# yukiteruono/pbsim3

Measured on AMD Instinct MI355X. Metric: simulated bases/sec, higher is better.
Workload: dtype u8

## Files before the change

pbsim3_amd/csrc/ctx.h:

```cpp
#pragma once
#include <hip/hip_runtime.h>
#include <limits.h>
#include <stdio.h>
#include <stdlib.h>
#include <stdint.h>

#include <algorithm>
#include <condition_variable>
#include <functional>
#include <memory>
#include <mutex>
#include <string>
#include <vector>

#include "../../include/pbsim3_amd.h"
#include "host_tables.h"
#include "kernels.h"

namespace pbsim {
extern thread_local std::string g_err;
int fail(const std::string &m);
}


#define NEED_DEVICE(c)                                                                      \
  do {                                                                                      \
    if ((c)->device < 0 || !(c)->stream)                                                    \
      return fail("this context has no HIP device: the gfx950 product path has no CPU fallback"); \
  } while (0)

#define HIP_OK(expr)                                                                        \
  do {                                                                                      \
    hipError_t e_ = (expr);                                                                 \
    if (e_ != hipSuccess)                                                                   \
      return fail(std::string("HIP error: ") + hipGetErrorString(e_) + " at " #expr);       \
  } while (0)

struct DevBuf {
  void *p = nullptr;
  size_t bytes = 0;
  ~DevBuf() { release(); }
  void release() {
    if (p) (void)hipFree(p);
    p = nullptr;
    bytes = 0;
  }
  hipError_t ensure(size_t n, bool exact = false) {
    if (n <= bytes) return hipSuccess;
    release();
    size_t want = exact ? n : std::max<size_t>(n + n / 8 + 256, 64u << 10);
    hipError_t e = hipMalloc(&p, want);
    if (e != hipSuccess) {
      p = nullptr;
      return e;
    }
    bytes = want;
    return hipSuccess;
  }
  template <class T>
  T *as() const {
    return reinterpret_cast<T *>(p);
  }
};

struct HostBuf {
  void *p = nullptr;
  size_t bytes = 0;
  ~HostBuf() {
    if (p) (void)hipHostFree(p);
  }
  hipError_t ensure(size_t n) {
    if (n <= bytes) return hipSuccess;
    if (p) (void)hipHostFree(p);
    p = nullptr;
    bytes = 0;
    size_t want = std::max<size_t>(n + n / 8 + 4096, 1u << 20);
    hipError_t e = hipHostMalloc(&p, want, hipHostMallocDefault);
    if (e != hipSuccess) {
      p = nullptr;
      return e;
    }
    bytes = want;
    return hipSuccess;
  }
};

using namespace pbsim;

constexpr int kMaxSlots = 6;
constexpr int kPipelineDepth = 2;
static_assert(kPipelineDepth >= 1 && kPipelineDepth <= kMaxSlots, "the pipeline's slots are the first of kMaxSlots");

constexpr size_t kScratchSlack = 64u << 10;
constexpr double kSinkBatchBases = 5.0e9;

constexpr int kDfBuffers = 5;
struct DfLane {
  DevBuf d_df_status, d_df_ctl;
  uint32_t epoch = 0;
  DevBuf d_df_dense[kDfBuffers];
  DevBuf d_df_code;
  HostBuf h_df_total, h_df_out[kDfBuffers];
  hipStream_t stream = nullptr;
  hipStream_t copy_stream = nullptr;
  bool own_streams = false;
  hipStream_t own[2] = {nullptr, nullptr};
  bool pre_valid = false, pre_own_staging = false, pre_elsewhere = false;
  const uint8_t *pre_text = nullptr;
  int64_t pre_n = 0;
  int pre_count = 0;
  hipStream_t lane_stream = nullptr;
  hipEvent_t ev_pre = nullptr;
  hipEvent_t ev_df[kDfBuffers] = {}, ev_cp[kDfBuffers] = {};
  hipEvent_t ev_k0[kDfBuffers] = {}, ev_k1[kDfBuffers] = {};
  std::vector<std::unique_ptr<HostBuf>> arena_blocks;
  std::vector<size_t> arena_fill;
  std::vector<char> arena_touched;
  std::vector<int> arena_idle;
  std::vector<std::pair<const char *, int64_t>> arena_segs;
  size_t arena_bytes() const {
    size_t n = 0;
    for (const auto &b : arena_blocks) n += b->bytes;
    return n;
  }
  void arena_reset() {
    std::fill(arena_fill.begin(), arena_fill.end(), 0);
    arena_segs.clear();
  }
  char *arena_reserve(int64_t n, size_t max_bytes) {
    static const size_t kBlock = getenv("PBSIM_PINNED_BLOCK_KB") && atoll(getenv("PBSIM_PINNED_BLOCK_KB")) > 0
                                     ? (size_t)atoll(getenv("PBSIM_PINNED_BLOCK_KB")) << 10 : (size_t)256u << 20;
    const size_t need = ((size_t)n + 63) & ~(size_t)63;
    for (size_t i = 0; i < arena_blocks.size(); i++) {
      HostBuf &b = *arena_blocks[i];
      if (arena_fill[i] + need <= b.bytes) {
        char *p = (char *)b.p + arena_fill[i];
        arena_fill[i] += need;
        arena_touched[i] = 1;
        arena_segs.emplace_back(p, n);
        return p;
      }
    }
    const size_t want = std::max(kBlock, need);
    if (max_bytes && arena_bytes() + want > max_bytes) return nullptr;
    if (getenv("PBSIM_TRACE")) fprintf(stderr, "[pbsim arena] new block of %zu MB (lane holds %zu MB in %zu blocks)\n", want >> 20, arena_bytes() >> 20, arena_blocks.size());
    arena_blocks.emplace_back(new HostBuf);
    arena_fill.push_back(0);
    arena_touched.push_back(1);
    arena_idle.push_back(0);
    if (arena_blocks.back()->ensure(want) != hipSuccess) {
      arena_blocks.pop_back();
      arena_fill.pop_back();
      arena_touched.pop_back();
      arena_idle.pop_back();
      return nullptr;
    }
    arena_fill.back() = need;
    arena_segs.emplace_back((char *)arena_blocks.back()->p, n);
    return (char *)arena_blocks.back()->p;
  }
  static constexpr int kArenaIdleJobs = 16;
  void arena_release() {
    arena_blocks.clear();
    arena_fill.clear();
    arena_touched.clear();
    arena_idle.clear();
    arena_segs.clear();
  }
  void arena_trim() {
    size_t k = 0;
    for (size_t i = 0; i < arena_blocks.size(); i++) arena_idle[i] = arena_touched[i] ? 0 : arena_idle[i] + 1;
    if (getenv("PBSIM_TRACE")) {
      size_t drop = 0;
      for (size_t i = 0; i < arena_blocks.size(); i++) drop += arena_idle[i] >= kArenaIdleJobs ? 1 : 0;
      if (drop) fprintf(stderr, "[pbsim arena] trim: %zu of %zu blocks go back\n", drop, arena_blocks.size());
    }
    for (size_t i = 0; i < arena_blocks.size(); i++)
      if (arena_idle[i] < kArenaIdleJobs) {
        if (k != i) {
          arena_blocks[k] = std::move(arena_blocks[i]);
          arena_idle[k] = arena_idle[i];
        }
        k++;
      }
    arena_blocks.resize(k);
    arena_idle.resize(k);
    arena_fill.assign(k, 0);
    arena_touched.assign(k, 0);
    arena_segs.clear();
  }
};

struct RefDesc {
  const uint8_t *seq = nullptr;
  const uint8_t *hp = nullptr;
  int64_t len = 0;
  int64_t unit = 0;
  bool hp_flag = false;
  bool hp11 = false;
};

struct StatsAcc {
  int64_t res_num = 0, res_len_total = 0, res_len_min = LONG_MAX, res_len_max = 0;
  int64_t res_sub = 0, res_ins = 0, res_del = 0;
  double accuracy_total = 0.0;
  std::vector<int64_t> freq_len, freq_acc;
  bool keep_values = false;
  struct Block {
    int64_t first_task;
    std::vector<double> values;
  };
  std::vector<Block> blocks;
  void reset() {
    res_num = res_len_total = res_len_max = 0;
    res_len_min = LONG_MAX;
    res_sub = res_ins = res_del = 0;
    accuracy_total = 0.0;
    std::fill(freq_len.begin(), freq_len.end(), 0);
    std::fill(freq_acc.begin(), freq_acc.end(), 0);
    blocks.clear();
  }
};

struct Slot {
  RefDesc ref;
  hipStream_t stream = nullptr;
  hipEvent_t ev0 = nullptr, ev1 = nullptr, ev2 = nullptr, ev3 = nullptr;
  DevBuf d_flags;
  DevBuf d_rawlen, d_len, d_off, d_acc;
  DevBuf d_hist, d_bin_start, d_bin_cursor, d_class_start;
  DevBuf d_task_of_slot, d_slot_of_task, d_wave_cap, d_wave_off, d_wg_tmp, d_wg_order;
  DevBuf d_out_len, d_maf_len, d_nsub, d_nins, d_ndel, d_qsum;
  DevBuf d_cum, d_scan_tmp, d_rt_len, d_mt_len, d_row_dst;
  DevBuf d_chain, d_chain_mask;
  DevBuf d_scratch, d_read_text, d_maf_text;
  HostBuf h_read_text, h_maf_text, h_stats, h_flags;
  DfLane df[2];
  hipStream_t walk_stream = nullptr;
  hipEvent_t ev_sq_walk = nullptr, ev_sq_done = nullptr;
  bool sq_pending = false;
  hipEvent_t ev_prep = nullptr;
  hipStream_t coop_stream = nullptr;
  hipEvent_t ev_coop = nullptr;
  bool stats_fetched = false;
  hipEvent_t ev_t0 = nullptr, ev_t1 = nullptr;
  bool text_timed = false;
  int64_t text_in = 0, text_out = 0;
  hipEvent_t ev_text = nullptr;
  int64_t b_first = 0, b_n = 0, b_slots_max = 0;
  bool b_truncated = false, b_enqueued = false, b_walked = false, b_finalized = false;
  bool b_chain = false;
  bool b_exported = false;
  int64_t b_trunc = -1;
  double b_factor = 2.0;
  int64_t b_pass0 = 0;
  int64_t b_max_raw = 0;
  pbsim_batch_info b_info;
};

struct JobRecord {
  DevBuf seq, hp, tiles, flags;
  int64_t len = 0;
  RefDesc ref;
  hipEvent_t ready = nullptr;
  DeviceFlags *h_flags = nullptr;
  ~JobRecord() {
    if (ready) (void)hipEventDestroy(ready);
    if (h_flags) (void)hipHostFree(h_flags);
  }
};

struct pbsim_ctx {
  pbsim_params p;
  int device = 0;
  hipStream_t stream = nullptr;
  Slot slots[kMaxSlots];
  int cur = 0;
  Slot &s() { return slots[cur]; }

  std::unique_ptr<ErrModel> err;
  std::unique_ptr<QsModel> qs;
  HeaderTables hdr;
  HpBias bias;
  ErrClassTables ect;
  QsClassTables qct;
  bool class_tables_dirty = true;
  int coop_wg_errhmm[2] = {0, 0};
  bool header_uploaded = false;

  DevBuf d_prob2len, d_prob2acc, d_cls;
  DevBuf d_qs_tabs_v[2];
  bool qs_tabs_ready[2] = {false, false};
  DevBuf d_seq_own, d_hp, d_tiles, d_ref_flags;
  DevBuf d_seq_next, d_hp_next, d_tiles_next, d_ref_flags_next;
  hipStream_t prefetch_stream = nullptr;
  DevBuf d_lines, d_lines_tmp;
  hipStream_t sq_stream = nullptr;
  const void *pf_src = nullptr;
  int64_t pf_len = 0;
  bool seq_hp_flag = false;
  const uint8_t *d_seq = nullptr;
  int64_t ref_len = 0;
  int64_t unit = 0;
  int64_t census[kHpSlots] = {0};
  bool census_done = false;
  bool census_from_job = false;
  bool hp11_explicit = false;
  bool hp11_before_job = false;
  int64_t n_units = 0, trans_reads = 0;
  DevBuf d_read_unit, d_read_minus, d_read_base, d_unit_len, d_unit_rank, d_unit_names, d_off_table, d_ssp, d_ssp_rv;
  DevBuf d_sq, d_sq_line_len, d_sq_line_qoff, d_sq_vbase;
  std::vector<int32_t> sq_len;
  std::vector<int64_t> sq_off;
  int64_t sq_total = 0;
  int64_t sp_chunk_bytes = 0;
  int64_t scratch_budget = 0;
  double scratch_factor = 2.0, need_seen = 0.0;
  bool scratch_factor_fixed = false;
  int64_t rewalked_batches = 0;
  bool scratch_auto = true;
  hipStream_t df_streams[2][2] = {{nullptr, nullptr}, {nullptr, nullptr}};
  bool defer_text_sync = false;
  bool defer_account = false;
  int walk_lds_kb = 27;
  bool bam_output = false;
  int deflate = 0;
  bool deflate_parallel = false;
  DevBuf d_df_tables;
  DevBuf d_df_prof;

  StatsAcc st;
  std::vector<std::unique_ptr<JobRecord>> job_records;
  std::mutex job_mu;
  std::condition_variable job_cv;
  std::vector<int64_t> job_expect_len;
  std::vector<std::unique_ptr<JobRecord>> job_spare;
  bool job_feed_failed = false;
  std::string job_feed_err;
  int64_t job_counters[8] = {0};
  int64_t job_progress[8] = {0};
  double job_breakdown[16] = {0};
  int job_interleave = 1;
  int64_t job_first_unit = 1;

  double prof_walk_ms = 0, prof_total_ms = 0, prof_tail_ms = 0;
  int64_t prof_walk_launches = 0, prof_tail_launches = 0;
  int64_t prof_wave_launches = 0;
  hipEvent_t ev_prof_base = nullptr;
  std::vector<std::pair<float, float>> prof_intervals;
  double prof_text_ms = 0, prof_deflate_ms = 0;
  int64_t prof_text_launches = 0, prof_text_in = 0, prof_text_out = 0;
  int64_t prof_deflate_launches = 0, prof_deflate_in = 0, prof_deflate_out = 0;
  std::mutex prof_mu;
};

namespace pbsim {
RefDesc current_ref(const pbsim_ctx *c);
int64_t quota_of(const pbsim_ctx *c, int64_t ref_len);
int walk_begin(pbsim_ctx *c, const RefDesc &ref, int64_t first_read, int64_t n_reads, int64_t truncate_remaining, bool chain = false,
               double factor = 0.0 );
double scratch_factor_of(const pbsim_ctx *c);
int chain_end_finalize(pbsim_ctx *c, int64_t len_total_before, pbsim_batch_info *out);
int chain_reads_for(const pbsim_ctx *c, int64_t ref_len, int64_t remaining);
constexpr int kChainReads = 6;
int64_t batch_capacity_for(const pbsim_ctx *c, int64_t ref_len);
int finalize_cut(pbsim_ctx *c, int64_t len_total_before, pbsim_batch_info *out);
int finalize_text(pbsim_ctx *c, pbsim_batch_info *info);
int finalize_uncut(pbsim_ctx *c, pbsim_batch_info *out);
std::string sam_header_text(const pbsim_ctx *c, int64_t unit);
int account_slot(pbsim_ctx *c, StatsAcc *st);
int account_of(pbsim_ctx *c, Slot &sl, StatsAcc *st);
void stats_add_task(StatsAcc *st, int64_t len_max, bool quality, long len, long nsub, long nins, long ndel, double qsum,
                    std::vector<double> *values);
void stats_finish(const StatsAcc &st, const pbsim_params &p, int64_t ref_len, pbsim_stats *o);
int stats_merge(StatsAcc *st, const pbsim_params &p, const pbsim_comm *comm, int64_t *extra, int n_extra);
int deflate_prelaunch(pbsim_ctx *c, Slot &sl, bool want_read, bool want_maf);
int deflate_pieces(pbsim_ctx *c, DfLane &lane, const uint8_t *d_text, int64_t n,
                   const std::function<int(const char *, int64_t)> &consume,
                   const std::function<char *(int64_t)> *place = nullptr);
int ensure_deflate_ready(pbsim_ctx *c);
int ensure_crc_tables(pbsim_ctx *c);
int prepare_enqueue(pbsim_ctx *c, uint8_t *d_seq, DevBuf &hp, DevBuf &tiles, DevBuf &flags, int64_t len, hipStream_t stream);
int ensure_tables(pbsim_ctx *c, bool hp11);
inline bool has_quality(const pbsim_ctx *c) { return c->p.method == PBSIM_METHOD_QS || c->p.method == PBSIM_METHOD_SAMPLE; }
}
```

pbsim3_amd/csrc/deflate.hip:

```cpp
#include <hip/hip_runtime.h>
#include <stdint.h>
#include <stdlib.h>

#include "kernels.h"

namespace pbsim {

namespace {

constexpr int kChunk = DF_CHUNK;
constexpr int kThreads = 256;
constexpr int kSeg = kChunk / kThreads;
constexpr int kSegDw = kSeg / 4;
constexpr int kInDw = kChunk / 4 + kChunk / 128;
constexpr int kOutBytes = 33024;
constexpr int kOutDw = kOutBytes / 4;
constexpr int kSyms = 288;
constexpr uint32_t kPoly = 0xEDB88320u;
constexpr int kHeadBits = 18 * 8;
constexpr int kPrefixBits = 3 + 5 + 5 + 4 + 19 * 3;

constexpr int kClLenTab[19] = {3, 5, 4, 4, 4, 5, 5, 5, 5, 5, 5, 5, 4, 5, 5, 5, 5, 3, 3};
constexpr int kClOrderTab[19] = {16, 17, 18, 0, 8, 7, 9, 6, 10, 5, 11, 4, 12, 3, 13, 2, 14, 1, 15};
constexpr uint64_t pack_cl_len() {
  uint64_t v = 0;
  for (int s = 0; s < 19; ++s) v |= (uint64_t)kClLenTab[s] << (3 * s);
  return v;
}
constexpr uint64_t kClLenPacked = pack_cl_len();
__device__ __forceinline__ uint32_t cl_len(uint32_t s) { return (uint32_t)(kClLenPacked >> (3 * s)) & 7u; }
constexpr unsigned __int128 pack_prefix() {
  unsigned __int128 v = 1u | (2u << 1) | ((unsigned __int128)15 << 13);
  for (int i = 0; i < 19; ++i) v |= (unsigned __int128)kClLenTab[kClOrderTab[i]] << (17 + 3 * i);
  return v;
}
constexpr uint64_t kPrefixLo = (uint64_t)pack_prefix();
constexpr uint32_t kPrefixHi = (uint32_t)(pack_prefix() >> 64);

__device__ __forceinline__ uint32_t rev_bits(uint32_t code, uint32_t len) { return __brev(code) >> (32 - len); }

__device__ __forceinline__ uint32_t cl_code(uint32_t s) {
  uint32_t c, l = cl_len(s);
  if (l == 3) c = s == 0 ? 0 : s - 16;
  else if (l == 4) c = s == 12 ? 9 : 4 + s;
  else c = s == 1 ? 20 : s <= 11 ? 16 + s : 15 + s;
  return rev_bits(c, l);
}

__device__ __forceinline__ uint32_t gf2_mul(uint32_t a, uint32_t b) {
  uint32_t p = 0;
#pragma unroll
  for (int i = 0; i < 32; ++i) {
    p ^= b & (0u - ((a >> (31 - i)) & 1u));
    b = (b >> 1) ^ (kPoly & (0u - (b & 1u)));
  }
  return p;
}

struct BitWriter {
  uint32_t *out;
  uint32_t word, nb;
  uint64_t acc;
  __device__ __forceinline__ void init(uint32_t *o, uint32_t bitpos) {
    out = o;
    word = bitpos >> 5;
    nb = bitpos & 31;
    acc = 0;
  }
  __device__ __forceinline__ void put(uint32_t v, uint32_t k) {
    acc |= (uint64_t)v << nb;
    nb += k;
    if (nb >= 32) {
      atomicOr(&out[word++], (uint32_t)acc);
      acc >>= 32;
      nb -= 32;
    }
  }
  __device__ __forceinline__ void put64(uint64_t v, uint32_t k) {
    if (k > 32) {
      put((uint32_t)v, 32);
      put((uint32_t)(v >> 32), k - 32);
    } else {
      put((uint32_t)v, k);
    }
  }
  __device__ __forceinline__ void flush() {
    if (nb) atomicOr(&out[word], (uint32_t)acc);
  }
};

__device__ __forceinline__ void length_symbol(uint32_t L, uint32_t *sym, uint32_t *eb, uint32_t *ev) {
  const uint32_t v = L - 3;
  if (v < 8) {
    *sym = 257 + v;
    *eb = 0;
    *ev = 0;
  } else if (L == 258) {
    *sym = 285;
    *eb = 0;
    *ev = 0;
  } else {
    const uint32_t e = (31 - __clz(v)) - 2;
    *sym = 261 + 4 * e + ((v >> e) & 3);
    *eb = e;
    *ev = v & ((1u << e) - 1);
  }
}

__device__ __forceinline__ uint32_t block_scan_excl(uint32_t v, uint32_t *s_wave, uint32_t *total) {
  const int lane = threadIdx.x & 63, wave = threadIdx.x >> 6;
  uint32_t inc = v;
#pragma unroll
  for (int d = 1; d < 64; d <<= 1) {
    const uint32_t o = __shfl_up(inc, d, 64);
    if (lane >= d) inc += o;
  }
  __syncthreads();
  if (lane == 63) s_wave[wave] = inc;
  __syncthreads();
  uint32_t base = 0, tot = 0;
#pragma unroll
  for (int w = 0; w < kThreads / 64; ++w) {
    const uint32_t x = s_wave[w];
    if (w < wave) base += x;
    tot += x;
  }
  *total = tot;
  return base + inc - v;
}

struct Mask128 {
  uint64_t lo, hi;
};
__device__ __forceinline__ Mask128 m_and(Mask128 a, Mask128 b) { return {a.lo & b.lo, a.hi & b.hi}; }
__device__ __forceinline__ Mask128 m_or(Mask128 a, Mask128 b) { return {a.lo | b.lo, a.hi | b.hi}; }
__device__ __forceinline__ Mask128 m_not(Mask128 a) { return {~a.lo, ~a.hi}; }
template <int K>
__device__ __forceinline__ Mask128 m_shl(Mask128 a) { return {a.lo << K, (a.hi << K) | (a.lo >> (64 - K))}; }
template <int K>
__device__ __forceinline__ Mask128 m_shr(Mask128 a) { return {(a.lo >> K) | (a.hi << (64 - K)), a.hi >> K}; }
__device__ __forceinline__ uint32_t m_nibble(Mask128 a, int j) {
  return (uint32_t)((j < 16 ? a.lo >> (4 * j) : a.hi >> (4 * j - 64)) & 15u);
}
__device__ __forceinline__ int m_first(Mask128 a) { return a.lo ? __builtin_ctzll(a.lo) : 64 + __builtin_ctzll(a.hi); }
__device__ __forceinline__ Mask128 m_clear(Mask128 a, int pos) {
  if (pos < 64) a.lo &= ~(1ull << pos);
  else a.hi &= ~(1ull << (pos - 64));
  return a;
}
__device__ __forceinline__ int m_run(Mask128 m, int pos) {
  uint64_t lo, hi;
  if (pos == 0) {
    lo = m.lo;
    hi = m.hi;
  } else if (pos < 64) {
    lo = (m.lo >> pos) | (m.hi << (64 - pos));
    hi = m.hi >> pos;
  } else {
    lo = m.hi >> (pos - 64);
    hi = 0;
  }
  if (~lo) return __builtin_ctzll(~lo);
  return ~hi ? 64 + __builtin_ctzll(~hi) : 128;
}

struct SegTokens {
  Mask128 lit;
  Mask128 start;
  Mask128 cover;
};

__device__ __forceinline__ SegTokens seg_tokens(const uint32_t (&seg)[kSegDw], int seg_n, uint32_t prev_dword,
                                                bool chunk_start) {
  uint64_t e[2] = {0, 0};
  uint32_t pw = prev_dword;
#pragma unroll
  for (int j = 0; j < kSegDw; ++j) {
    const uint32_t w = seg[j];
    const uint32_t d = w ^ ((w << 8) | (pw >> 24));
    const uint32_t z = ~(((d & 0x7F7F7F7Fu) + 0x7F7F7F7Fu) | d | 0x7F7F7F7Fu);
    const uint32_t nib = (((z >> 7) * 0x00204081u) >> 21) & 15u;
    e[j >> 4] |= (uint64_t)nib << (4 * (j & 15));
    pw = w;
  }
  Mask128 valid;
  valid.lo = seg_n >= 64 ? ~0ull : (1ull << seg_n) - 1;
  valid.hi = seg_n >= 128 ? ~0ull : seg_n > 64 ? (1ull << (seg_n - 64)) - 1 : 0ull;
  Mask128 eq = {e[0] & valid.lo, e[1] & valid.hi};
  if (chunk_start) eq.lo &= ~1ull;
  const Mask128 r3 = m_and(eq, m_and(m_shr<1>(eq), m_shr<2>(eq)));
  SegTokens t;
  t.cover = m_or(r3, m_or(m_shl<1>(r3), m_shl<2>(r3)));
  t.start = m_and(t.cover, m_not(m_shl<1>(t.cover)));
  t.lit = m_and(valid, m_not(t.cover));
  return t;
}

constexpr int kSampleChunks = DF_SAMPLE_CHUNKS;
constexpr int kHdrDw = DF_TABLE_HDR_DW;

struct DfTable {
  uint32_t code[kSyms];
  uint32_t hdr_end_bits;
  uint32_t pad[3];
  uint32_t hdr[kHdrDw];
};
static_assert(sizeof(DfTable) <= DF_TABLE_BYTES, "DF_TABLE_BYTES too small");

__device__ __forceinline__ void load_chunk(const uint8_t *__restrict__ text, int64_t n_bytes, int64_t chunk, uint32_t *s_in,
                                           uint32_t (&seg)[kSegDw], int *n_out, int *seg_n_out, uint32_t *prev_dw) {
  const int tid = threadIdx.x;
  const int64_t base = chunk * (int64_t)kChunk;
  const int n = (int)((n_bytes - base) < (int64_t)kChunk ? (n_bytes - base) : (int64_t)kChunk);
  const uint4 *src4 = reinterpret_cast<const uint4 *>(text + base);
  for (int q = tid; q < kChunk / 16; q += kThreads) {
    uint4 v = make_uint4(0, 0, 0, 0);
    if (q * 16 < n) v = src4[q];
    const int d = q * 4;
    uint32_t *dst = &s_in[d + (d >> 5)];
    dst[0] = v.x;
    dst[1] = v.y;
    dst[2] = v.z;
    dst[3] = v.w;
  }
  __syncthreads();
  const int beg = tid * kSeg;
  *n_out = n;
  *seg_n_out = n - beg < 0 ? 0 : (n - beg < kSeg ? n - beg : kSeg);
#pragma unroll
  for (int j = 0; j < kSegDw; ++j) seg[j] = s_in[tid * (kSegDw + 1) + j];
  *prev_dw = tid ? s_in[tid * (kSegDw + 1) - 2] : 0u;
  __syncthreads();
}

__global__ __launch_bounds__(kThreads) void k_deflate_hist(const uint8_t *__restrict__ text, int64_t n_bytes,
                                                            uint32_t *__restrict__ hist) {
  __shared__ uint32_t s_in[kInDw];
  __shared__ uint32_t s_hist[3 * kSyms + 64];
  const int tid = threadIdx.x, lane = tid & 63;
  for (int i = tid; i < 3 * kSyms + 64; i += kThreads) s_hist[i] = 0;
  uint32_t seg[kSegDw], prev_dw;
  int n, seg_n;
  load_chunk(text, n_bytes, blockIdx.x, s_in, seg, &n, &seg_n, &prev_dw);
  const SegTokens tk = seg_tokens(seg, seg_n, prev_dw, tid == 0);
  const uint32_t copy = (uint32_t)(lane % 3) * kSyms, dummy = 3 * kSyms + lane;
#pragma unroll
  for (int j = 0; j < kSegDw; ++j) {
    const uint32_t nl = m_nibble(tk.lit, j);
    if (nl == 0) continue;
    const uint32_t w = seg[j];
#pragma unroll
    for (int k = 0; k < 4; ++k) atomicAdd(&s_hist[((nl >> k) & 1u) ? copy + ((w >> (8 * k)) & 255u) : dummy], 1u);
  }
  Mask128 st = tk.start;
  while (st.lo | st.hi) {
    const int pos = m_first(st);
    st = m_clear(st, pos);
    uint32_t sy, eb, ev;
    length_symbol((uint32_t)m_run(tk.cover, pos), &sy, &eb, &ev);
    atomicAdd(&s_hist[copy + sy], 1u);
  }
  __syncthreads();
  for (int i = tid; i < 286; i += kThreads) {
    const uint32_t f = s_hist[i] + s_hist[kSyms + i] + s_hist[2 * kSyms + i] + (i == 256 ? 1u : 0u);
    if (f) atomicAdd(&hist[i], f);
  }
}

__global__ __launch_bounds__(kThreads) void k_deflate_build(const uint32_t *__restrict__ hist, DfTable *__restrict__ tbl) {
  __shared__ uint32_t s_freq[kSyms], s_sfreq[kSyms], s_w[kSyms], s_code[kSyms];
  __shared__ uint16_t s_sorted[kSyms], s_par[kSyms], s_leafpar[kSyms], s_dep[kSyms];
  __shared__ uint8_t s_len[kSyms];
  __shared__ uint32_t s_cnt[16], s_first[16];
  __shared__ uint32_t s_img[4 + kHdrDw];
  const int tid = threadIdx.x;
  constexpr int m = 286;
  for (int i = tid; i < kSyms; i += kThreads) {
    s_freq[i] = i < m ? hist[i] + 1u : 0u;
    s_code[i] = 0;
    s_len[i] = 0;
  }
  for (int i = tid; i < 4 + kHdrDw; i += kThreads) s_img[i] = 0;
  if (tid < 16) s_cnt[tid] = 0;
  __syncthreads();
  for (int i = tid; i < m; i += kThreads) {
    const uint32_t fi = s_freq[i];
    uint32_t rank = 0;
    for (int u = 0; u < m; ++u) {
      const uint32_t g = s_freq[u];
      rank += (g < fi) | ((g == fi) & (u < i));
    }
    s_sorted[rank] = (uint16_t)i;
    s_sfreq[rank] = fi;
  }
  __syncthreads();
  if (tid == 0) {
    int leaf = 0, root = 0;
    for (int nxt = 0; nxt < m - 1; ++nxt) {
      uint32_t tot = 0;
      for (int k = 0; k < 2; ++k) {
        const bool take_leaf = leaf < m && (root >= nxt || s_sfreq[leaf] <= s_w[root]);
        if (take_leaf) {
          tot += s_sfreq[leaf];
          s_leafpar[leaf] = (uint16_t)nxt;
          ++leaf;
        } else {
          tot += s_w[root];
          s_par[root] = (uint16_t)nxt;
          ++root;
        }
      }
      s_w[nxt] = tot;
    }
    s_dep[m - 2] = 0;
    for (int i = m - 3; i >= 0; --i) s_dep[i] = s_dep[s_par[i]] + 1;
    for (int i = 0; i < m; ++i) {
      int d = s_dep[s_leafpar[i]] + 1;
      if (d > 15) d = 15;
      s_cnt[d] += 1;
    }
    uint32_t total = 0;
    for (int l = 1; l <= 15; ++l) total += s_cnt[l] << (15 - l);
    while (total > (1u << 15)) {
      s_cnt[15] -= 1;
      for (int l = 14; l >= 1; --l)
        if (s_cnt[l]) {
          s_cnt[l] -= 1;
          s_cnt[l + 1] += 2;
          break;
        }
      total -= 1;
    }
    int i = 0;
    for (int l = 15; l >= 1; --l)
      for (uint32_t k = 0; k < s_cnt[l]; ++k) s_len[s_sorted[i++]] = (uint8_t)l;
    uint32_t code = 0;
    s_cnt[0] = 0;
    for (int l = 1; l <= 15; ++l) {
      code = (code + s_cnt[l - 1]) << 1;
      s_first[l] = code;
    }
  }
  __syncthreads();
  for (int i = tid; i < m; i += kThreads) {
    const uint32_t l = s_len[i];
    uint32_t idx = 0;
    for (int u = 0; u < i; ++u) idx += s_len[u] == l;
    s_code[i] = rev_bits(s_first[l] + idx, l) | (l << 16);
  }
  __syncthreads();
  if (tid == 0) {
    BitWriter bw;
    bw.init(s_img, kHeadBits);
    bw.put64(kPrefixLo | ((uint64_t)(m - 257) << 3), 64);
    bw.put(kPrefixHi, kPrefixBits - 64);
    uint32_t bits = kHeadBits + kPrefixBits;
    int p = 0;
    const int npos = m + 1;
    while (p < npos) {
      const uint32_t v = p < m ? s_len[p] : 1u;
      bw.put(cl_code(v), cl_len(v));
      bits += cl_len(v);
      ++p;
      int r = 0;
      while (p + r < npos && (p + r < m ? s_len[p + r] : 1u) == v) ++r;
      while (r >= 3) {
        const int t = r < 6 ? r : 6;
        bw.put(cl_code(16) | ((uint32_t)(t - 3) << cl_len(16)), cl_len(16) + 2);
        bits += cl_len(16) + 2;
        r -= t;
        p += t;
      }
    }
    bw.flush();
    tbl->hdr_end_bits = bits;
  }
  __syncthreads();
  for (int i = tid; i < kSyms; i += kThreads) tbl->code[i] = s_code[i];
  for (int i = tid; i < kHdrDw; i += kThreads) tbl->hdr[i] = s_img[4 + i];
}

struct DfCtl {
  uint32_t ticket;
  uint32_t error;
  int64_t total;
};
static_assert(sizeof(DfCtl) == DF_CTL_BYTES, "DF_CTL_BYTES");

constexpr uint64_t kStSize = 1ull << 32, kStPrefix = 2ull << 32;
__device__ __forceinline__ uint64_t st_word(uint32_t epoch, uint64_t flag, uint32_t v) { return ((uint64_t)epoch << 34) | flag | v; }

__device__ __forceinline__ uint32_t look_back(const uint64_t *status, int64_t c, uint32_t epoch, int lane, uint32_t *error) {
  uint32_t sum = 0;
  int64_t hi = c - 1;
  for (uint32_t spins = 0;; spins++) {
    if (spins > (1u << 24)) {
      if (lane == 0) atomicOr(error, 1u);
      return sum;
    }
    const int64_t i = hi - lane;
    uint64_t w = 0;
    if (i >= 0) w = __hip_atomic_load(&status[i], __ATOMIC_RELAXED, __HIP_MEMORY_SCOPE_AGENT);
    const bool mine = i >= 0 && (uint32_t)(w >> 34) == epoch && ((w >> 32) & 3u) != 0;
    const uint64_t ready = __ballot(mine || i < 0);
    const uint64_t pref = __ballot(mine && ((w >> 32) & 3u) == 2u);
    const int k = ~ready ? __builtin_ctzll(~ready) : 64;
    const uint64_t usable = k >= 64 ? ~0ull : ((1ull << k) - 1);
    const uint64_t stop = pref & usable;
    if (stop) {
      const int e = __builtin_ctzll(stop);
      uint32_t v = (lane <= e && i >= 0) ? (uint32_t)w : 0u;
#pragma unroll
      for (int d = 32; d >= 1; d >>= 1) v += __shfl_xor(v, d, 64);
      return sum + v;
    }
    if (k == 0) {
      __builtin_amdgcn_s_sleep(2);
      continue;
    }
    uint32_t v = (lane < k && i >= 0) ? (uint32_t)w : 0u;
#pragma unroll
    for (int d = 32; d >= 1; d >>= 1) v += __shfl_xor(v, d, 64);
    sum += v;
    hi -= k;
    if (hi < 0) return sum;
  }
}

typedef uint32_t u32x4 __attribute__((ext_vector_type(4)));
__device__ __forceinline__ void store_member(uint8_t *dst, const uint32_t *s_img, uint32_t bytes, int tid) {
  const uint32_t head = min((uint32_t)((16u - ((uintptr_t)dst & 15u)) & 15u), bytes);
  const uint8_t *s8 = reinterpret_cast<const uint8_t *>(s_img);
  if ((uint32_t)tid < head) dst[tid] = s8[tid];
  const uint32_t nvec = (bytes - head) >> 4;
  const uint32_t sh = head & 3u, dw0 = head >> 2;
  u32x4 *d4 = reinterpret_cast<u32x4 *>(dst + head);
  for (uint32_t v = tid; v < nvec; v += kThreads) {
    const uint32_t *p = s_img + dw0 + 4u * v;
    const uint32_t a = p[0], b = p[1], c = p[2], d = p[3], e = p[4];
    u32x4 o;
    o.x = __builtin_amdgcn_alignbyte(b, a, sh);
    o.y = __builtin_amdgcn_alignbyte(c, b, sh);
    o.z = __builtin_amdgcn_alignbyte(d, c, sh);
    o.w = __builtin_amdgcn_alignbyte(e, d, sh);
    __builtin_nontemporal_store(o, &d4[v]);
  }
  const uint32_t done = head + 16u * nvec;
  if ((uint32_t)tid < bytes - done) dst[done + tid] = s8[done + tid];
}

__global__ __launch_bounds__(kThreads) void k_deflate_chunks(const uint8_t *__restrict__ text, int64_t n_bytes,
                                                              uint8_t *__restrict__ dense, uint64_t *__restrict__ status,
                                                              DfCtl *__restrict__ ctl, uint32_t epoch,
                                                              const uint32_t *__restrict__ crc_table,
                                                              const uint32_t *__restrict__ pow128, uint32_t x8rem,
                                                              const DfTable *__restrict__ tbl,
                                                              unsigned long long *__restrict__ prof) {
  __shared__ uint32_t s_in[kInDw];
  static_assert(kOutDw <= kInDw, "the output image must fit the input image");
  uint32_t *const s_out = s_in;
  __shared__ uint32_t s_code[kSyms];
  uint32_t *const s_crc = s_in;
  __shared__ uint32_t s_wave[kThreads / 64];
  __shared__ uint32_t s_misc[4];

  const int tid = threadIdx.x, lane = tid & 63;
  unsigned long long t_prev = prof ? wall_clock64() : 0;
  int phase = 0;
  auto mark = [&]() {
    if (prof && tid == 0) {
      const unsigned long long t = wall_clock64();
      atomicAdd(&prof[phase], t - t_prev);
      t_prev = t;
    }
    ++phase;
  };
  for (int i = tid; i < kSyms; i += kThreads) s_code[i] = i < 286 ? tbl->code[i] : 0u;
  if (tid < 4) s_misc[tid] = tid == 0 ? atomicAdd(&ctl->ticket, 1u) : 0u;
  __syncthreads();
  const int64_t chunk = s_misc[0];
  const int64_t n_chunks = (n_bytes + kChunk - 1) / kChunk;
  uint32_t seg[kSegDw], prev_dw;
  int n, seg_n;
  load_chunk(text, n_bytes, chunk, s_in, seg, &n, &seg_n, &prev_dw);
  const int beg = tid * kSeg;
  mark();
  for (int i = tid; i < kInDw; i += kThreads) s_in[i] = (i < 1024) ? crc_table[i] : 0u;
  __syncthreads();
  const SegTokens tk = seg_tokens(seg, seg_n, prev_dw, tid == 0);

  uint32_t tok_bits = 0;
  {
    uint32_t c = tid == 0 ? 0xFFFFFFFFu : 0u;
    const int full = seg_n >> 2;
#pragma unroll
    for (int j = 0; j < kSegDw; ++j) {
      if (j < full) {
        const uint32_t x = c ^ seg[j];
        c = s_crc[768 + (x & 255u)] ^ s_crc[512 + ((x >> 8) & 255u)] ^ s_crc[256 + ((x >> 16) & 255u)] ^ s_crc[x >> 24];
      } else if (j == full) {
        for (int k = 0; k < (seg_n & 3); ++k) c = s_crc[(c ^ (seg[j] >> (8 * k))) & 255u] ^ (c >> 8);
      }
    }
    const int q = n >> 7, r = n & 127;
    if (seg_n == kSeg && tid < q) {
      c = gf2_mul(c, pow128[q - tid - 1]);
      if (r) c = gf2_mul(c, x8rem);
    }
    if (seg_n == 0) c = 0;
#pragma unroll
    for (int d = 32; d >= 1; d >>= 1) c ^= __shfl_xor(c, d, 64);
    if (lane == 0) atomicXor(&s_misc[3], c);
  }
  mark();
  {
#pragma unroll
    for (int j = 0; j < kSegDw; ++j) {
      const uint32_t nl = m_nibble(tk.lit, j);
      if (nl == 0) continue;
      const uint32_t w = seg[j];
#pragma unroll
      for (int k = 0; k < 4; ++k)
        tok_bits += s_code[((nl >> k) & 1u) ? (w >> (8 * k)) & 255u : 287u] >> 16;
    }
    Mask128 st = tk.start;
    while (st.lo | st.hi) {
      const int pos = m_first(st);
      st = m_clear(st, pos);
      uint32_t sy, eb, ev;
      length_symbol((uint32_t)m_run(tk.cover, pos), &sy, &eb, &ev);
      tok_bits += (s_code[sy] >> 16) + eb + 1;
    }
  }
  uint32_t tok_total;
  const uint32_t tok_off = block_scan_excl(tok_bits, s_wave, &tok_total);
  const uint32_t hdr_end = tbl->hdr_end_bits;
  const uint32_t eob_len = s_code[256] >> 16;
  const uint32_t payload_bits = hdr_end - kHeadBits + tok_total + eob_len;
  const uint32_t payload_bytes = (payload_bits + 7) >> 3;
  const bool huff = (18 + payload_bytes + 8 <= (uint32_t)kOutBytes) && (payload_bytes < (uint32_t)n + 5);
  const uint32_t crc = s_misc[3] ^ 0xFFFFFFFFu;
  const uint32_t member = huff ? 18 + payload_bytes + 8 : 18 + 5 + (uint32_t)n + 8;
  if (tid == 0)
    __hip_atomic_store(&status[chunk], st_word(epoch, chunk == 0 ? kStPrefix : kStSize, member), __ATOMIC_RELAXED, __HIP_MEMORY_SCOPE_AGENT);
  mark();

  if (huff) {
    __syncthreads();
    for (int i = tid; i < 1024; i += kThreads) s_in[i] = 0;
    __syncthreads();
    if (tid < kHdrDw) s_out[4 + tid] = tbl->hdr[tid];
    if (tid == 0) {
      s_out[0] = 0x04088b1fu;
      s_out[1] = 0;
      s_out[2] = 0x0006ff00u;
      s_out[3] = 0x00024342u;
    }
    __syncthreads();
    if (tid == 0) atomicOr(&s_out[4], member - 1);
    mark();
    {
      BitWriter bw;
      bw.init(s_out, hdr_end + tok_off);
#pragma unroll
      for (int j = 0; j < kSegDw; ++j) {
        const uint32_t nl = m_nibble(tk.lit, j), ns = m_nibble(tk.start, j);
        if ((nl | ns) == 0) continue;
        const uint32_t w = seg[j];
        uint32_t c[4];
#pragma unroll
        for (int k = 0; k < 4; ++k) c[k] = s_code[((nl >> k) & 1u) ? (w >> (8 * k)) & 255u : 287u];
        uint32_t mv = 0, ml = 0, ks = 4;
        if (ns) {
          ks = (uint32_t)__builtin_ctz(ns);
          uint32_t sy, eb, ev;
          length_symbol((uint32_t)m_run(tk.cover, 4 * j + (int)ks), &sy, &eb, &ev);
          const uint32_t cm = s_code[sy];
          mv = (cm & 0xFFFFu) | (ev << (cm >> 16));
          ml = (cm >> 16) + eb + 1;
        }
        bw.put(ks == 0 ? mv : 0u, ks == 0 ? ml : 0u);
        {
          const uint32_t l0 = c[0] >> 16;
          bw.put((c[0] & 0xFFFFu) | ((c[1] & 0xFFFFu) << l0), l0 + (c[1] >> 16));
        }
        const bool mid = ks == 1 || ks == 2;
        bw.put(mid ? mv : 0u, mid ? ml : 0u);
        {
          const uint32_t l2 = c[2] >> 16;
          bw.put((c[2] & 0xFFFFu) | ((c[3] & 0xFFFFu) << l2), l2 + (c[3] >> 16));
        }
        bw.put(ks == 3 ? mv : 0u, ks == 3 ? ml : 0u);
      }
      bw.flush();
    }
    mark();
    if (tid == 0) {
      BitWriter bw;
      bw.init(s_out, hdr_end + tok_total);
      bw.put(s_code[256] & 0xFFFFu, eob_len);
      bw.flush();
      bw.init(s_out, (18 + payload_bytes) * 8);
      bw.put(crc, 32);
      bw.put((uint32_t)n, 32);
      bw.flush();
    }
    if (tid < 64 && chunk > 0) {
      const uint32_t excl = look_back(status, chunk, epoch, tid, &ctl->error);
      if (tid == 0) {
        s_misc[1] = excl;
        __hip_atomic_store(&status[chunk], st_word(epoch, kStPrefix, excl + member), __ATOMIC_RELAXED, __HIP_MEMORY_SCOPE_AGENT);
      }
    }
    __syncthreads();
    mark();
    const uint32_t off = s_misc[1];
    store_member(dense + off, s_out, member, tid);
    if (tid == 0 && chunk == n_chunks - 1) ctl->total = (int64_t)off + member;
    mark();
  } else {
    if (tid < 64 && chunk > 0) {
      const uint32_t excl = look_back(status, chunk, epoch, tid, &ctl->error);
      if (tid == 0) {
        s_misc[1] = excl;
        __hip_atomic_store(&status[chunk], st_word(epoch, kStPrefix, excl + member), __ATOMIC_RELAXED, __HIP_MEMORY_SCOPE_AGENT);
      }
    }
    __syncthreads();
    uint8_t *slot = dense + s_misc[1];
    if (tid == 0 && chunk == n_chunks - 1) ctl->total = (int64_t)s_misc[1] + member;
    if (tid == 0) {
      const uint8_t head[23] = {0x1f, 0x8b, 8,   4,   0,   0,
                                0,    0,    0,   0xff, 6,  0,
                                'B',  'C',  2,   0,   (uint8_t)((member - 1) & 255), (uint8_t)((member - 1) >> 8),
                                1,    (uint8_t)(n & 255), (uint8_t)(n >> 8), (uint8_t)(~n & 255), (uint8_t)((~n >> 8) & 255)};
      for (int i = 0; i < 23; ++i) slot[i] = head[i];
      uint8_t *t = slot + 23 + n;
      for (int i = 0; i < 4; ++i) t[i] = (uint8_t)(crc >> (8 * i));
      for (int i = 0; i < 4; ++i) t[4 + i] = (uint8_t)((uint32_t)n >> (8 * i));
    }
#pragma unroll
    for (int j = 0; j < kSegDw; ++j)
#pragma unroll
      for (int k = 0; k < 4; ++k)
        if (4 * j + k < seg_n) slot[23 + beg + 4 * j + k] = (uint8_t)(seg[j] >> (8 * k));
  }
}

uint32_t host_gf2_mul(uint32_t a, uint32_t b) {
  uint32_t p = 0;
  for (int i = 0; i < 32; ++i) {
    if (a & (0x80000000u >> i)) p ^= b;
    b = (b >> 1) ^ ((b & 1u) ? kPoly : 0u);
  }
  return p;
}

uint32_t host_xpow8(uint64_t nbytes) {
  uint32_t r = 0x80000000u, b = 0x00800000u;
  while (nbytes) {
    if (nbytes & 1) r = host_gf2_mul(r, b);
    b = host_gf2_mul(b, b);
    nbytes >>= 1;
  }
  return r;
}

}

void deflate_host_tables(uint32_t *crc_table, uint32_t *pow128) {
  for (uint32_t i = 0; i < 256; ++i) {
    uint32_t c = i;
    for (int k = 0; k < 8; ++k) c = (c >> 1) ^ ((c & 1u) ? kPoly : 0u);
    crc_table[i] = c;
  }
  for (int t = 1; t < 4; ++t)
    for (uint32_t i = 0; i < 256; ++i) {
      const uint32_t c = crc_table[(t - 1) * 256 + i];
      crc_table[t * 256 + i] = (c >> 8) ^ crc_table[c & 255u];
    }
  const uint32_t step = host_xpow8(128);
  uint32_t v = 0x80000000u;
  for (int k = 0; k < 256; ++k) {
    pow128[k] = v;
    v = host_gf2_mul(v, step);
  }
}

void launch_deflate_table(const uint8_t *text, int64_t n_bytes, uint32_t *hist, void *table, hipStream_t s) {
  if (n_bytes <= 0) return;
  const int64_t nch = (n_bytes + DF_CHUNK - 1) / DF_CHUNK;
  const int64_t ns = nch < kSampleChunks ? nch : kSampleChunks;
  const int64_t sample_bytes = ns * (int64_t)DF_CHUNK < n_bytes ? ns * (int64_t)DF_CHUNK : n_bytes;
  (void)hipMemsetAsync(hist, 0, 288 * sizeof(uint32_t), s);
  hipLaunchKernelGGL(k_deflate_hist, dim3((unsigned)ns), dim3(kThreads), 0, s, text, sample_bytes, hist);
  hipLaunchKernelGGL(k_deflate_build, dim3(1), dim3(kThreads), 0, s, (const uint32_t *)hist, reinterpret_cast<DfTable *>(table));
}

void launch_deflate(const uint8_t *text, int64_t n_bytes, uint64_t *status, void *ctl, uint32_t epoch, uint8_t *dense,
                    const uint32_t *d_crc_table, const uint32_t *d_pow128, const void *table, hipStream_t s,
                    unsigned long long *d_prof, hipEvent_t ev_begin, hipEvent_t ev_chunks_done) {
  if (n_bytes <= 0) return;
  const int64_t nch = (n_bytes + DF_CHUNK - 1) / DF_CHUNK;
  const uint32_t x8rem = host_xpow8((uint64_t)(n_bytes % DF_CHUNK) & 127u);
  (void)hipMemsetAsync(ctl, 0, DF_CTL_BYTES, s);
  if (ev_begin) (void)hipEventRecord(ev_begin, s);
  hipLaunchKernelGGL(k_deflate_chunks, dim3((unsigned)nch), dim3(kThreads), 0, s, text, n_bytes, dense, status,
                     reinterpret_cast<DfCtl *>(ctl), epoch & 0x3fffffffu, d_crc_table, d_pow128, x8rem,
                     reinterpret_cast<const DfTable *>(table), d_prof);
  if (ev_chunks_done) (void)hipEventRecord(ev_chunks_done, s);
}

}
```

pbsim3_amd/csrc/deflate_host.cpp:

```cpp
#include <hip/hip_runtime.h>
#include <limits.h>
#include <math.h>
#include <stdio.h>
#include <stdlib.h>
#include <string.h>

#include <algorithm>
#include <chrono>
#include <functional>
#include <memory>
#include <string>
#include <thread>
#include <vector>

#include "ctx.h"
#include "engine_internal.h"
#include "unit_io.h"

extern "C" {

extern "C++" {
namespace {

int ensure_deflate_tables(pbsim_ctx *c) {
  if (c->d_df_tables.p) return PBSIM_SUCCEEDED;
  std::vector<uint32_t> t(1024 + 256);
  deflate_host_tables(t.data(), t.data() + 1024);
  if (!upload(c->d_df_tables, t.data(), t.size() * 4, c->stream)) return PBSIM_FAILED;
  HIP_OK(hipStreamSynchronize(c->stream));
  return PBSIM_SUCCEEDED;
}

struct DfGeom {
  int64_t piece, max_ch, n_pieces;
  int ahead, nbuf;
  int64_t off(int64_t j) const { return j * piece; }
  int64_t len(int64_t j, int64_t n) const { return std::min(piece, n - off(j)); }
};
DfGeom df_geom(int64_t n) {
  constexpr int64_t piece_chunks = DF_PIECE_CHUNKS;
  constexpr int kDfAhead = 4;
  static_assert(kDfAhead >= 1 && kDfAhead <= kDfBuffers - 1, "ahead + 1 dense buffers are in use");
  DfGeom g;
  g.piece = piece_chunks * DF_CHUNK;
  g.max_ch = std::min<int64_t>(piece_chunks, (n + DF_CHUNK - 1) / DF_CHUNK);
  g.n_pieces = (n + g.piece - 1) / g.piece;
  g.ahead = kDfAhead;
  g.nbuf = g.ahead + 1;
  return g;
}

int df_launch_piece(pbsim_ctx *c, DfLane &sl, const DfGeom &g, const uint8_t *d_text, int64_t n, int64_t j, bool wait_buffer,
                    bool own_staging, unsigned long long *d_prof) {
  const int b = (int)(j % g.nbuf);
  const int64_t off = g.off(j), len = g.len(j, n);
  const uint32_t *tab = c->d_df_tables.as<uint32_t>();
  int64_t *h_total = reinterpret_cast<int64_t *>(sl.h_df_total.p);
  HIP_OK(sl.d_df_dense[b].ensure((size_t)g.max_ch * DF_SLOT + 64, true));
  if (own_staging) HIP_OK(sl.h_df_out[b].ensure((size_t)g.max_ch * DF_SLOT + 64));
  if (wait_buffer) HIP_OK(hipStreamWaitEvent(sl.stream, sl.ev_cp[b], 0));
  uint8_t *dense = sl.d_df_dense[b].as<uint8_t>();
  if (((sl.epoch + 1) & 0x3fffffffu) == 0) {
    HIP_OK(hipMemsetAsync(sl.d_df_status.p, 0, sl.d_df_status.bytes, sl.stream));
    sl.epoch++;
  }
  launch_deflate(d_text + off, len, sl.d_df_status.as<uint64_t>(), sl.d_df_ctl.p, ++sl.epoch, dense, tab, tab + 1024,
                 sl.d_df_code.p, sl.stream, d_prof, sl.ev_k0[b], sl.ev_k1[b]);
  HIP_OK(hipGetLastError());
  HIP_OK(hipMemcpyAsync(&h_total[2 * b], sl.d_df_ctl.p, DF_CTL_BYTES, hipMemcpyDeviceToHost, sl.stream));
  HIP_OK(hipEventRecord(sl.ev_df[b], sl.stream));
  return PBSIM_SUCCEEDED;
}

int df_begin(pbsim_ctx *c, DfLane &sl, const uint8_t *d_text, int64_t n, bool own_staging, hipStream_t launch_stream) {
  if (!ensure_deflate_tables(c)) return PBSIM_FAILED;
  const DfGeom g = df_geom(n);
  const size_t status_bytes_was = sl.d_df_status.bytes;
  HIP_OK(sl.d_df_status.ensure((size_t)(g.piece / DF_CHUNK) * 8));
  HIP_OK(sl.d_df_ctl.ensure(DF_CTL_BYTES));
  HIP_OK(sl.h_df_total.ensure(DF_CTL_BYTES * kDfBuffers));
  HIP_OK(sl.d_df_code.ensure(DF_TABLE_BYTES + 288 * 4));
  int lane_index = 0;
  for (Slot &slot : c->slots)
    if (&slot.df[1] == &sl) lane_index = 1;
  hipStream_t lane_streams[2];
  if (sl.own_streams) {
    for (int i = 0; i < 2; i++)
      if (!sl.own[i]) HIP_OK(hipStreamCreateWithFlags(&sl.own[i], hipStreamNonBlocking));
    lane_streams[0] = sl.own[0];
    lane_streams[1] = sl.own[1];
  } else {
    for (int i = 0; i < 2; i++)
      if (!c->df_streams[lane_index][i]) HIP_OK(hipStreamCreateWithFlags(&c->df_streams[lane_index][i], hipStreamNonBlocking));
    lane_streams[0] = c->df_streams[lane_index][0];
    lane_streams[1] = c->df_streams[lane_index][1];
  }
  sl.lane_stream = lane_streams[0];
  sl.stream = launch_stream ? launch_stream : lane_streams[0];
  sl.copy_stream = lane_streams[1];
  if (sl.d_df_status.bytes != status_bytes_was) HIP_OK(hipMemsetAsync(sl.d_df_status.p, 0, sl.d_df_status.bytes, sl.stream));
  launch_deflate_table(d_text, n, reinterpret_cast<uint32_t *>(sl.d_df_code.as<uint8_t>() + DF_TABLE_BYTES), sl.d_df_code.p, sl.stream);
  if (!sl.ev_df[0]) {
    for (int i = 0; i < kDfBuffers; i++) {
      HIP_OK(hipEventCreateWithFlags(&sl.ev_df[i], hipEventDisableTiming));
      HIP_OK(hipEventCreateWithFlags(&sl.ev_cp[i], hipEventDisableTiming));
      HIP_OK(hipEventCreate(&sl.ev_k0[i]));
      HIP_OK(hipEventCreate(&sl.ev_k1[i]));
    }
  }
  unsigned long long *d_prof = nullptr;
  if (getenv("PBSIM_DEFLATE_PROF")) {
    HIP_OK(c->d_df_prof.ensure(128));
    HIP_OK(hipMemsetAsync(c->d_df_prof.p, 0, 128, sl.stream));
    d_prof = c->d_df_prof.as<unsigned long long>();
  }
  const int64_t first = std::min<int64_t>(launch_stream ? 1 : g.ahead, g.n_pieces);
  for (int64_t j = 0; j < first; j++)
    if (!df_launch_piece(c, sl, g, d_text, n, j, false, own_staging, d_prof)) return PBSIM_FAILED;
  sl.pre_count = (int)first;
  sl.pre_text = d_text;
  sl.pre_n = n;
  sl.pre_own_staging = own_staging;
  sl.pre_valid = true;
  sl.pre_elsewhere = launch_stream != nullptr;
  if (launch_stream) {
    if (!sl.ev_pre) HIP_OK(hipEventCreateWithFlags(&sl.ev_pre, hipEventDisableTiming));
    HIP_OK(hipEventRecord(sl.ev_pre, launch_stream));
  }
  return PBSIM_SUCCEEDED;
}

template <class F>
int deflate_stream(pbsim_ctx *c, DfLane &sl, const uint8_t *d_text, int64_t n, F &&consume,
                   const std::function<char *(int64_t)> *place = nullptr) {
  if (n <= 0) return PBSIM_SUCCEEDED;
  const bool prelaunched = sl.pre_valid && sl.pre_text == d_text && sl.pre_n == n && sl.pre_own_staging == (place == nullptr);
  sl.pre_valid = false;
  if (!prelaunched && !df_begin(c, sl, d_text, n, place == nullptr, nullptr)) return PBSIM_FAILED;
  sl.pre_valid = false;
  if (sl.pre_elsewhere) {
    sl.stream = sl.lane_stream;
    HIP_OK(hipStreamWaitEvent(sl.stream, sl.ev_pre, 0));
    sl.pre_elsewhere = false;
  }
  const DfGeom g = df_geom(n);
  const int64_t n_pieces = g.n_pieces;
  const int ahead = g.ahead, nbuf = g.nbuf;
  unsigned long long *d_prof = getenv("PBSIM_DEFLATE_PROF") ? c->d_df_prof.as<unsigned long long>() : nullptr;
  const bool trace = getenv("PBSIM_DEFLATE_TRACE") != nullptr;
  const auto now = []() { return std::chrono::duration<double, std::milli>(std::chrono::steady_clock::now().time_since_epoch()).count(); };
  double t_kernel = 0, t_copy = 0, t_consume = 0, t_begin = now();
  int64_t out_bytes = 0;
  std::vector<std::pair<hipEvent_t, hipEvent_t>> tev;
  bool used[kDfBuffers] = {false};
  int64_t *h_total = reinterpret_cast<int64_t *>(sl.h_df_total.p);
  auto launch = [&](int64_t j) -> int {
    return df_launch_piece(c, sl, g, d_text, n, j, used[(int)(j % nbuf)], place == nullptr, d_prof);
  };
  for (int64_t j = sl.pre_count; j < std::min<int64_t>(ahead, n_pieces); j++)
    if (!launch(j)) return PBSIM_FAILED;
  const char *prev_ptr = nullptr;
  int64_t prev_bytes = 0;
  int prev_buf = 0;
  for (int64_t k = 0; k < n_pieces; k++) {
    const int b = (int)(k % nbuf);
    const double t0 = now();
    HIP_OK(hipEventSynchronize(sl.ev_df[b]));
    t_kernel += now() - t0;
    const int64_t total = h_total[2 * b + 1];
    if ((uint64_t)h_total[2 * b] >> 32) return fail("deflate: a workgroup's look-back gave up waiting for its predecessors");
    out_bytes += total;
    {
      float ms = 0;
      if (hipEventElapsedTime(&ms, sl.ev_k0[b], sl.ev_k1[b]) == hipSuccess) {
        std::lock_guard<std::mutex> lk(c->prof_mu);
        c->prof_deflate_ms += ms;
        c->prof_deflate_launches++;
        c->prof_deflate_in += g.len(k, n);
        c->prof_deflate_out += total;
      }
    }
    char *dst = place ? (*place)(total) : (char *)sl.h_df_out[b].p;
    if (!dst) return fail("deflate: no room for a compressed piece");
    HIP_OK(hipStreamWaitEvent(sl.copy_stream, sl.ev_df[b], 0));
    if (trace) {
      hipEvent_t e0 = nullptr, e1 = nullptr;
      HIP_OK(hipEventCreate(&e0));
      HIP_OK(hipEventCreate(&e1));
      tev.emplace_back(e0, e1);
      HIP_OK(hipEventRecord(e0, sl.copy_stream));
    }
    HIP_OK(hipMemcpyAsync(dst, sl.d_df_dense[b].p, (size_t)total, hipMemcpyDeviceToHost, sl.copy_stream));
    if (trace) HIP_OK(hipEventRecord(tev.back().second, sl.copy_stream));
    HIP_OK(hipEventRecord(sl.ev_cp[b], sl.copy_stream));
    used[b] = true;
    if (prev_bytes) {
      const double t1 = now();
      HIP_OK(hipEventSynchronize(sl.ev_cp[prev_buf]));
      const double t2 = now();
      if (!consume(prev_ptr, prev_bytes)) return PBSIM_FAILED;
      t_copy += t2 - t1;
      t_consume += now() - t2;
    }
    prev_ptr = dst;
    prev_bytes = total;
    prev_buf = b;
    if (k + ahead < n_pieces && !launch(k + ahead)) return PBSIM_FAILED;
  }
  if (prev_bytes) {
    const double t1 = now();
    HIP_OK(hipEventSynchronize(sl.ev_cp[prev_buf]));
    const double t2 = now();
    if (!consume(prev_ptr, prev_bytes)) return PBSIM_FAILED;
    t_copy += t2 - t1;
    t_consume += now() - t2;
  }
  if (trace) {
    double t_link = 0, t_span = 0;
    float ms = 0;
    for (auto &e : tev) {
      if (hipEventElapsedTime(&ms, e.first, e.second) == hipSuccess) t_link += ms;
    }
    if (!tev.empty() && hipEventElapsedTime(&ms, tev.front().first, tev.back().second) == hipSuccess) t_span = ms;
    for (auto &e : tev) {
      (void)hipEventDestroy(e.first);
      (void)hipEventDestroy(e.second);
    }
    fprintf(stderr,
            "[deflate] %.1f MB -> %.1f MB in %.1f ms: waited %.1f ms for kernels, %.1f ms for copies, %.1f ms in the consumer; copies: "
            "%.1f ms on the engine within a span of %.1f ms (%.1f GB/s while copying)\n",
            n / 1e6, out_bytes / 1e6, now() - t_begin, t_kernel, t_copy, t_consume, t_link, t_span, t_link > 0 ? out_bytes / t_link / 1e6 : 0.0);
  }
  if (d_prof) {
    unsigned long long t[16];
    HIP_OK(hipMemcpy(t, d_prof, 128, hipMemcpyDeviceToHost));
    const double nch = (double)((n + DF_CHUNK - 1) / DF_CHUNK);
    static const char *names[7] = {"stage", "crc", "sizes+scan", "header", "tokens", "trailer", "store"};
    fprintf(stderr, "[deflate prof] %.0f chunks; us per chunk (lane 0):", nch);
    for (int i = 0; i < 7; ++i) fprintf(stderr, " %s %.1f", names[i], t[i] / nch / 100);
    fprintf(stderr, "\n");
  }
  return PBSIM_SUCCEEDED;
}

int deflate_to_host(pbsim_ctx *c, DfLane &sl, const uint8_t *d_text, int64_t n, char *host_dst, int64_t cap,
                    int64_t *out_bytes) {
  int64_t written = 0;
  const int ok = deflate_stream(c, sl, d_text, n, [&](const char *z, int64_t k) {
    if (written + k > cap) return fail("deflate: output buffer too small");
    memcpy(host_dst + written, z, (size_t)k);
    written += k;
    return PBSIM_SUCCEEDED;
  });
  *out_bytes = written;
  return ok;
}

}
}

extern "C++" int pbsim::deflate_pieces(pbsim_ctx *c, DfLane &lane, const uint8_t *d_text, int64_t n,
                                       const std::function<int(const char *, int64_t)> &consume,
                                       const std::function<char *(int64_t)> *place) {
  return deflate_stream(c, lane, d_text, n, consume, place);
}
extern "C++" int pbsim::ensure_deflate_ready(pbsim_ctx *c) {
  for (auto &lane : c->df_streams)
    for (hipStream_t &st : lane)
      if (!st) HIP_OK(hipStreamCreateWithFlags(&st, hipStreamNonBlocking));
  return ensure_deflate_tables(c);
}
extern "C++" int pbsim::ensure_crc_tables(pbsim_ctx *c) { return ensure_deflate_tables(c); }
extern "C++" int pbsim::deflate_prelaunch(pbsim_ctx *c, Slot &sl, bool want_read, bool want_maf) {
  const pbsim_batch_info &bi = sl.b_info;
  if (want_read && bi.read_text_bytes > 0 && !df_begin(c, sl.df[0], sl.d_read_text.as<uint8_t>(), bi.read_text_bytes, true, sl.stream))
    return PBSIM_FAILED;
  if (want_maf && bi.maf_text_bytes > 0 && !df_begin(c, sl.df[1], sl.d_maf_text.as<uint8_t>(), bi.maf_text_bytes, true, sl.stream))
    return PBSIM_FAILED;
  return PBSIM_SUCCEEDED;
}

int pbsim_set_deflate(pbsim_ctx *c, int on) {
  if (!c) return fail("bad argument");
  c->deflate = on & 3;
  c->deflate_parallel = (on & 4) != 0;
  return PBSIM_SUCCEEDED;
}

int64_t pbsim_deflate_bound(int64_t n) {
  if (n <= 0) return 0;
  return n + ((n + DF_CHUNK - 1) / DF_CHUNK) * 31;
}

int pbsim_batch_fetch_deflated(pbsim_ctx *c, char *read_gz, int64_t read_cap, char *maf_gz, int64_t maf_cap,
                               int64_t *read_gz_bytes, int64_t *maf_gz_bytes) {
  if (!c || !c->s().b_finalized) return fail("pbsim_batch_fetch_deflated: no finalized batch");
  NEED_DEVICE(c);
  HIP_OK(hipSetDevice(c->device));
  int64_t nr = 0, nm = 0;
  if (read_gz && !deflate_to_host(c, c->s().df[0], c->s().d_read_text.as<uint8_t>(), c->s().b_info.read_text_bytes, read_gz,
                                  read_cap, &nr))
    return PBSIM_FAILED;
  if (maf_gz && !deflate_to_host(c, c->s().df[0], c->s().d_maf_text.as<uint8_t>(), c->s().b_info.maf_text_bytes, maf_gz,
                                 maf_cap, &nm))
    return PBSIM_FAILED;
  if (read_gz_bytes) *read_gz_bytes = nr;
  if (maf_gz_bytes) *maf_gz_bytes = nm;
  return PBSIM_SUCCEEDED;
}

int pbsim_deflate_buffer(pbsim_ctx *c, const void *src, int64_t n, void *dst, int64_t cap, int64_t *out_bytes) {
  if (!c || !out_bytes || n < 0 || (n > 0 && (!src || !dst))) return fail("pbsim_deflate_buffer: bad argument");
  NEED_DEVICE(c);
  HIP_OK(hipSetDevice(c->device));
  *out_bytes = 0;
  if (n == 0) return PBSIM_SUCCEEDED;
  Slot &sl = c->slots[0];
  DevBuf d_in;
  HIP_OK(d_in.ensure((size_t)n + 16));
  HIP_OK(hipMemcpyAsync(d_in.p, src, (size_t)n, hipMemcpyHostToDevice, sl.stream));
  HIP_OK(hipStreamSynchronize(sl.stream));
  return deflate_to_host(c, sl.df[0], d_in.as<uint8_t>(), n, (char *)dst, cap, out_bytes);
}

extern "C++" int pbsim::deliver(pbsim_ctx *c, const pbsim_sink *sink) {
  const pbsim_batch_info &bi = c->s().b_info;
  if (sink && c->defer_text_sync) {
    NEED_DEVICE(c);
    HIP_OK(hipEventSynchronize(c->s().ev_text));
  }
  if (sink && c->deflate) {
    const bool zr = c->deflate & 1, zm = c->deflate & 2;
    NEED_DEVICE(c);
    HIP_OK(hipSetDevice(c->device));
    if (!zr) HIP_OK(c->s().h_read_text.ensure((size_t)bi.read_text_bytes + 16));
    if (!zm) HIP_OK(c->s().h_maf_text.ensure((size_t)bi.maf_text_bytes + 16));
    if ((!zr || !zm) &&
        !pbsim_batch_fetch(c, zr ? nullptr : (char *)c->s().h_read_text.p, zm ? nullptr : (char *)c->s().h_maf_text.p))
      return PBSIM_FAILED;
    Slot &sl = c->s();
    auto send_read = [&]() -> int {
      if (!(sink->on_read_text && bi.read_text_bytes)) return PBSIM_SUCCEEDED;
      if (!zr)
        return sink->on_read_text(sink->user, (const char *)sl.h_read_text.p, bi.read_text_bytes) ? PBSIM_SUCCEEDED
                                                                                                 : fail("sink aborted (read text)");
      return deflate_stream(c, sl.df[0], sl.d_read_text.as<uint8_t>(), bi.read_text_bytes, [&](const char *z, int64_t k) {
        return sink->on_read_text(sink->user, z, k) ? PBSIM_SUCCEEDED : fail("sink aborted (read text)");
      });
    };
    auto send_maf = [&]() -> int {
      if (!(sink->on_maf_text && bi.maf_text_bytes)) return PBSIM_SUCCEEDED;
      if (!zm)
        return sink->on_maf_text(sink->user, (const char *)sl.h_maf_text.p, bi.maf_text_bytes) ? PBSIM_SUCCEEDED
                                                                                              : fail("sink aborted (MAF text)");
      return deflate_stream(c, sl.df[1], sl.d_maf_text.as<uint8_t>(), bi.maf_text_bytes, [&](const char *z, int64_t k) {
        return sink->on_maf_text(sink->user, z, k) ? PBSIM_SUCCEEDED : fail("sink aborted (MAF text)");
      });
    };
    if (c->deflate_parallel && zr && zm && bi.read_text_bytes && bi.maf_text_bytes) {
      if (!ensure_deflate_tables(c)) return PBSIM_FAILED;
      int ok_read = PBSIM_SUCCEEDED;
      std::string err_read;
      std::thread t([&]() {
        (void)hipSetDevice(c->device);
        ok_read = send_read();
        if (!ok_read) err_read = g_err;
      });
      const int ok_maf = send_maf();
      t.join();
      if (!ok_read) return fail(err_read);
      if (!ok_maf) return PBSIM_FAILED;
    } else {
      if (!send_read()) return PBSIM_FAILED;
      if (!send_maf()) return PBSIM_FAILED;
    }
  } else if (sink) {
    HIP_OK(c->s().h_read_text.ensure((size_t)bi.read_text_bytes + 16));
    HIP_OK(c->s().h_maf_text.ensure((size_t)bi.maf_text_bytes + 16));
    if (!pbsim_batch_fetch(c, (char *)c->s().h_read_text.p, (char *)c->s().h_maf_text.p)) return PBSIM_FAILED;
    if (sink->on_read_text && bi.read_text_bytes &&
        !sink->on_read_text(sink->user, (const char *)c->s().h_read_text.p, bi.read_text_bytes))
      return fail("sink aborted (read text)");
    if (sink->on_maf_text && bi.maf_text_bytes &&
        !sink->on_maf_text(sink->user, (const char *)c->s().h_maf_text.p, bi.maf_text_bytes))
      return fail("sink aborted (MAF text)");
  }
  return c->defer_account ? PBSIM_SUCCEEDED : pbsim_batch_account(c);
}
}
```

pbsim3_amd/csrc/engine.cpp:

```cpp
#include <hip/hip_runtime.h>
#include <limits.h>
#include <math.h>
#include <stdio.h>
#include <stdlib.h>
#include <string.h>

#include <algorithm>
#include <chrono>
#include <functional>
#include <memory>
#include <string>
#include <thread>
#include <vector>

#include "ctx.h"
#include "engine_internal.h"
#include "unit_io.h"
#include "philox.h"

namespace pbsim {
thread_local std::string g_err;
int fail(const std::string &m) {
  g_err = m;
  return PBSIM_FAILED;
// ... 753 lines not shown
      hipStream_t cs = (ws == c->s().walk_stream && c->s().coop_stream) ? c->s().coop_stream : ws;
      if (cs != ws) HIP_OK(hipStreamWaitEvent(cs, c->s().ev_prep, 0));
      launch_walk_qshmm_coop(w, n_wg, c->qct.stride + 512 + 1024, cs);
      launch_qshmm_coop_qsum(w, slots_max, cs);
      c->prof_wave_launches++;
      if (cs != ws) HIP_OK(hipEventRecord(c->s().ev_coop, cs));
      lanes_idle = coop_len == 0 && s.coop_classes == (ncls >= 64 ? ~0ull : (1ull << ncls) - 1);
      if (!lanes_idle)
        launch_walk_qshmm(w, slots_max, c->qct.stride + 1536 + 96 * 8 + 94 * 48 + 94 * 8 + 94 * 32, c->qct.all_rv_100,
                          ref.hp_flag, ws, c->walk_lds_kb);
      if (cs != ws) HIP_OK(hipStreamWaitEvent(ws, c->s().ev_coop, 0));
    } else {
      launch_walk_qshmm(w, slots_max, c->qct.stride + 1536 + 96 * 8 + 94 * 48 + 94 * 8 + 94 * 32, c->qct.all_rv_100,
                        ref.hp_flag, ws, c->walk_lds_kb);
    }
    (void)lanes_idle;
  }
  if (chain) launch_chain_update(step, P, w.out_len, d_chain, ws);
  }
  HIP_OK(hipEventRecord(c->s().ev2, ws));
  HIP_OK(hipStreamWaitEvent(c->s().stream, c->s().ev2, 0));
  launch_gather_pass0_scan(w.out_len, n_reads, P, c->s().d_cum.as<int64_t>(), c->s().d_scan_tmp.as<int64_t>(),
                           &flags->sums[0], c->s().stream);
  HIP_OK(hipEventRecord(c->s().ev3, c->s().stream));
  HIP_OK(hipGetLastError());
  c->s().b_first = first_read;
  c->s().b_n = n_reads;
  c->s().b_slots_max = slots_max;
  c->s().b_chain = chain;
  c->s().b_trunc = truncate_remaining;
  c->s().b_factor = factor;
  c->s().b_truncated = truncate_remaining >= 0 || trans;
  c->s().b_enqueued = true;
  c->s().b_walked = false;
  c->s().b_finalized = false;
  c->s().stats_fetched = false;
  return PBSIM_SUCCEEDED;
}

int pbsim_batch_walk_end(pbsim_ctx *c, int64_t *pass0_bases) {
  if (!c) return fail("pbsim_batch_walk_end: bad argument");
  NEED_DEVICE(c);
  if (!c->s().b_enqueued) return fail("pbsim_batch_walk_end: no batch was begun on this slot");
  HIP_OK(hipSetDevice(c->device));
  c->s().b_enqueued = false;
  DeviceFlags f;
  if (!read_flags(c, &f)) return PBSIM_FAILED;
  float ms = 0;
  const bool bulk = c->s().b_n > 1 && !c->s().b_chain;
  if (hipEventElapsedTime(&ms, c->s().ev1, c->s().ev2) == hipSuccess) (bulk ? c->prof_walk_ms : c->prof_tail_ms) += ms;
  if (!bulk) c->prof_tail_launches++;
  if (bulk && c->ev_prof_base) {
    float a = 0, b = 0;
    if (hipEventElapsedTime(&a, c->ev_prof_base, c->s().ev1) == hipSuccess &&
        hipEventElapsedTime(&b, c->ev_prof_base, c->s().ev2) == hipSuccess)
      c->prof_intervals.emplace_back(a, b);
  }
  if (hipEventElapsedTime(&ms, c->s().ev0, c->s().ev3) == hipSuccess) c->prof_total_ms += ms;
  if (bulk) c->prof_walk_launches++;
  if (f.error & kErrScratchBudget) {
    char buf[160];
    snprintf(buf, sizeof buf, "scratch budget exceeded: batch needs %lld bytes, pool holds %lld",
             (long long)f.scratch_need, (long long)c->scratch_budget);
    return fail(buf);
  }
  if (f.need_q10) {
    c->need_seen = std::max(c->need_seen, (double)f.need_q10 / 1024.0);
    if (!c->scratch_factor_fixed) c->scratch_factor = std::min(2.0, std::max(1.0, c->need_seen + 0.08));
  }
  if (f.error & kErrScratchOverflow) {
    if (c->s().b_factor < 2.0) {
      c->rewalked_batches++;
      if (!c->scratch_factor_fixed) c->scratch_factor = std::min(2.0, c->scratch_factor + 0.25);
      Slot &sl = c->s();
      if (!walk_begin(c, sl.ref, sl.b_first, sl.b_n, sl.b_trunc, sl.b_chain, 2.0)) return PBSIM_FAILED;
      return pbsim_batch_walk_end(c, pass0_bases);
    }
    return fail("a read produced more MAF columns than 2*len+64 (the reference's buffers are 2*len_max+1)");
  }
  c->s().b_walked = true;
  c->s().b_pass0 = f.sums[0];
  c->s().b_max_raw = (int64_t)f.max_rawlen;
  if (pass0_bases) *pass0_bases = f.sums[0];
  return PBSIM_SUCCEEDED;
}

int pbsim_batch_fetch_lengths(pbsim_ctx *c, int32_t *rawlen, int32_t *len, int32_t *out_len_pass0) {
  if (!c || !c->s().b_walked) return fail("pbsim_batch_fetch_lengths: no walked batch on this slot");
  NEED_DEVICE(c);
  HIP_OK(hipSetDevice(c->device));
  Slot &sl = c->s();
  const size_t n = (size_t)sl.b_n;
  if (rawlen) HIP_OK(hipMemcpyAsync(rawlen, sl.d_rawlen.p, n * 4, hipMemcpyDeviceToHost, sl.stream));
  if (len) HIP_OK(hipMemcpyAsync(len, sl.d_len.p, n * 4, hipMemcpyDeviceToHost, sl.stream));
  if (out_len_pass0)
    HIP_OK(hipMemcpy2DAsync(out_len_pass0, 4, sl.d_out_len.p, (size_t)c->p.pass_num * 4, 4, n, hipMemcpyDeviceToHost, sl.stream));
  HIP_OK(hipStreamSynchronize(sl.stream));
  return PBSIM_SUCCEEDED;
}

extern "C++" int pbsim::chain_reads_for(const pbsim_ctx *c, int64_t ref_len, int64_t remaining) {
  const double lub = (double)std::min<int64_t>(std::min<int64_t>(c->p.len_max, std::max<int64_t>(ref_len, 1)),
                                               std::max<int64_t>(remaining, c->p.len_min));
  const double per_block = (double)regions_of(c) * 64.0 * (scratch_factor_of(c) * lub + kScratchPad + 64.0);
  const int64_t fit = (int64_t)((double)c->scratch_budget / (1.05 * per_block));
  return (int)std::max<int64_t>(1, std::min<int64_t>(kChainReads, fit));
}

extern "C++" int pbsim::chain_end_finalize(pbsim_ctx *c, int64_t len_total_before, pbsim_batch_info *out) {
  if (!c || !c->s().b_enqueued || !c->s().b_chain) return fail("internal: no chain of truncated reads on this slot");
  if (!pbsim_batch_walk_end(c, nullptr)) return PBSIM_FAILED;
  Slot &sl = c->s();
  ChainState *pin = reinterpret_cast<ChainState *>((char *)sl.h_flags.p + sizeof(DeviceFlags) + 16);
  HIP_OK(hipMemcpyAsync(pin, sl.d_chain.p, sizeof(ChainState), hipMemcpyDeviceToHost, sl.stream));
  HIP_OK(hipStreamSynchronize(sl.stream));
  const ChainState cs = *pin;
  pbsim_batch_info bi;
  memset(&bi, 0, sizeof bi);
  bi.first_read = sl.b_first;
  bi.n_reads = sl.b_n;
  bi.n_final = cs.made;
  bi.len_total_after = len_total_before + cs.total;
  bi.quota_reached = cs.done != 0;
  bi.need_truncated_read = !cs.done;
  sl.b_info = bi;
  if (!finalize_text(c, &bi)) return PBSIM_FAILED;
  *out = bi;
  return PBSIM_SUCCEEDED;
}

static void fill_text_args(pbsim_ctx *c, TextArgs *t, int64_t n_emit) {
  memset(t, 0, sizeof *t);
  t->first_read = c->s().b_first;
  t->n_reads = n_emit;
  t->pass_num = c->p.pass_num;
  t->is_wgs = c->p.strategy == PBSIM_STRATEGY_WGS;
  t->is_qs = has_quality_row(c);
  t->unit = (uint32_t)c->s().ref.unit;
  t->ref_len = c->s().ref.len;
  t->len = c->s().d_len.as<int32_t>();
  t->off = c->s().d_off.as<int32_t>();
  t->out_len = c->s().d_out_len.as<int32_t>();
  t->maf_len = c->s().d_maf_len.as<int32_t>();
  t->slot_of_task = c->s().d_slot_of_task.as<int32_t>();
  t->task_of_slot = c->s().d_task_of_slot.as<int32_t>();
  t->row_dst = c->s().d_row_dst.as<int64_t>();
  t->wave_cap = c->s().d_wave_cap.as<int32_t>();
  t->wave_off = c->s().d_wave_off.as<int64_t>();
  t->scratch = c->s().d_scratch.as<uint8_t>();
  t->read_text_len = c->s().d_rt_len.as<int64_t>();
  t->maf_text_len = c->s().d_mt_len.as<int64_t>();
  t->read_text_off = t->read_text_len;
  t->maf_text_off = t->maf_text_len;
  t->id_prefix_len = (int)strlen(c->p.id_prefix);
  memcpy(t->id_prefix, c->p.id_prefix, sizeof t->id_prefix);
  t->rq_len = snprintf(t->rq_text, sizeof t->rq_text, "%f", c->p.accuracy_mean);
  t->bam = c->bam_output && c->p.pass_num > 1;
  {
    const float f = strtof(t->rq_text, nullptr);
    memcpy(&t->rq_bits, &f, 4);
  }
  if (c->p.strategy != PBSIM_STRATEGY_WGS) {
    t->name_pad3 = c->p.strategy == PBSIM_STRATEGY_TEMPL;
    t->read_unit = c->d_read_unit.as<int32_t>() + (c->s().b_first - 1);
    t->read_minus = c->d_read_minus.as<uint8_t>() + (c->s().b_first - 1);
    t->unit_len = c->d_unit_len.as<int64_t>();
    t->unit_names = c->d_unit_names.as<char>();
  }
}

extern "C++" int pbsim::finalize_cut(pbsim_ctx *c, int64_t len_total_before, pbsim_batch_info *out) {
  if (!c || !c->s().b_walked) return fail("pbsim_batch_finalize: no walked batch");
  NEED_DEVICE(c);
  HIP_OK(hipSetDevice(c->device));
  DeviceFlags *flags = c->s().d_flags.as<DeviceFlags>();
  const int64_t quota = quota_of(c, c->s().ref.len);
  launch_quota_cut(c->s().d_cum.as<int64_t>(),
                   c->p.method == PBSIM_METHOD_SAMPLE ? nullptr : c->s().d_rawlen.as<int32_t>(), c->s().b_n, len_total_before, quota,
                   c->s().b_truncated ? 1 : 0, flags, c->s().stream);
  DeviceFlags f;
  if (!read_flags(c, &f)) return PBSIM_FAILED;
  const int64_t n_final = f.n_final;
  int64_t cum_final = c->s().b_pass0;
  if (n_final < c->s().b_n) {
    int64_t *pin = reinterpret_cast<int64_t *>((char *)c->s().h_flags.p + sizeof(DeviceFlags));
    HIP_OK(hipMemcpyAsync(pin, c->s().d_cum.as<int64_t>() + n_final, 8, hipMemcpyDeviceToHost, c->s().stream));
    HIP_OK(hipStreamSynchronize(c->s().stream));
    cum_final = *pin;
  }
  pbsim_batch_info bi;
  memset(&bi, 0, sizeof bi);
  bi.first_read = c->s().b_first;
  bi.n_reads = c->s().b_n;
  bi.n_final = n_final;
  bi.len_total_after = len_total_before + cum_final;
  if (c->p.strategy != PBSIM_STRATEGY_WGS) {
    bi.quota_reached = 0;
    bi.need_truncated_read = 0;
  } else if (c->s().b_truncated) {
    bi.quota_reached = bi.len_total_after >= quota;
    bi.need_truncated_read = !bi.quota_reached;
  } else {
    bi.quota_reached = (n_final < c->s().b_n) || (bi.len_total_after >= quota);
    bi.need_truncated_read = (n_final < c->s().b_n) && (bi.len_total_after < quota);
  }
  c->s().b_info = bi;
  *out = bi;
  return PBSIM_SUCCEEDED;
}

extern "C++" int pbsim::finalize_uncut(pbsim_ctx *c, pbsim_batch_info *out) {
  if (!c || !c->s().b_walked) return fail("pbsim_batch_finalize: no walked batch");
  NEED_DEVICE(c);
  pbsim_batch_info bi;
  memset(&bi, 0, sizeof bi);
  bi.first_read = c->s().b_first;
  bi.n_reads = c->s().b_n;
  bi.n_final = c->s().b_n;
  bi.len_total_after = c->s().b_pass0;
  c->s().b_info = bi;
  *out = bi;
  return PBSIM_SUCCEEDED;
}

static int fetch_stats(pbsim_ctx *c, Slot &sl, int64_t n_tasks);
static void collect_text_timing(pbsim_ctx *c, Slot &sl) {
  if (!sl.text_timed || hipEventQuery(sl.ev_t1) != hipSuccess) return;
  float ms = 0;
  if (hipEventElapsedTime(&ms, sl.ev_t0, sl.ev_t1) == hipSuccess) {
    std::lock_guard<std::mutex> lk(c->prof_mu);
    c->prof_text_ms += ms;
    c->prof_text_launches++;
    c->prof_text_in += sl.text_in;
    c->prof_text_out += sl.text_out;
  }
  sl.text_timed = false;
}
extern "C++" int pbsim::finalize_text(pbsim_ctx *c, pbsim_batch_info *info) {
  DeviceFlags *flags = c->s().d_flags.as<DeviceFlags>();
  DeviceFlags f;
  pbsim_batch_info bi = c->s().b_info;
  const int P = c->p.pass_num;
  const int64_t n_final = bi.n_final;
  const int64_t n_tasks = n_final * P;
  for (DfLane &L : c->s().df) L.pre_valid = false;
  if (n_tasks > 0) {
    HIP_OK(c->s().d_rt_len.ensure(n_tasks * 8));
    HIP_OK(c->s().d_mt_len.ensure(n_tasks * 8));
    HIP_OK(c->s().d_row_dst.ensure(n_tasks * 6 * 8));
    c->s().stats_fetched = c->defer_text_sync;
    if (c->defer_text_sync && !fetch_stats(c, c->s(), n_tasks)) return PBSIM_FAILED;
    HIP_OK(hipMemsetAsync(&flags->sums[1], 0, 5 * sizeof(int64_t), c->s().stream));
    TextArgs t;
    fill_text_args(c, &t, n_final);
    launch_text_sizes(t, flags, c->s().stream);
    launch_exclusive_scan_i64(t.read_text_len, t.read_text_len, n_tasks, c->s().d_scan_tmp.as<int64_t>(), &flags->sums[1],
                              c->s().stream);
    launch_exclusive_scan_i64(t.maf_text_len, t.maf_text_len, n_tasks, c->s().d_scan_tmp.as<int64_t>(), &flags->sums[2],
                              c->s().stream);
    if (!read_flags(c, &f)) return PBSIM_FAILED;
    bi.read_text_bytes = f.sums[1];
    bi.maf_text_bytes = f.sums[2];
    bi.bases = f.sums[3];
    bi.ref_bases = f.sums[4];
    bi.maf_columns = f.sums[5];
    HIP_OK(c->s().d_read_text.ensure(std::max<size_t>((size_t)bi.read_text_bytes + 16, 8u << 20)));
    HIP_OK(c->s().d_maf_text.ensure(std::max<size_t>((size_t)bi.maf_text_bytes + 16, 8u << 20)));
    t.read_text = c->s().d_read_text.as<char>();
    t.maf_text = c->s().d_maf_text.as<char>();
    collect_text_timing(c, c->s());
    HIP_OK(hipEventRecord(c->s().ev_t0, c->s().stream));
    launch_text_emit(t, c->s().b_slots_max, flags, c->s().stream);
    HIP_OK(hipEventRecord(c->s().ev_t1, c->s().stream));
    c->s().text_timed = true;
    c->s().text_in = (int64_t)regions_of(c) * bi.maf_columns;
    c->s().text_out = bi.read_text_bytes + bi.maf_text_bytes;
    HIP_OK(hipGetLastError());
    HIP_OK(hipEventRecord(c->s().ev_text, c->s().stream));
    if (!c->defer_text_sync) HIP_OK(hipStreamSynchronize(c->s().stream));
  }
  c->s().b_info = bi;
  c->s().b_finalized = true;
  if (info) *info = bi;
  return PBSIM_SUCCEEDED;
}

extern "C++" int pbsim::emit_batch(pbsim_ctx *c, const BatchOutput &o, pbsim_batch_info *info) {
  return o.arrays ? export_batch(c, o.arrays, info) : finalize_text(c, info);
}
extern "C++" int pbsim::deliver_batch(pbsim_ctx *c, const BatchOutput &o) {
  return o.arrays ? deliver_arrays(c, o.arrays) : deliver(c, o.sink);
}

int pbsim_batch_finalize(pbsim_ctx *c, int64_t len_total_before, pbsim_batch_info *info) {
  pbsim_batch_info bi;
  if (!finalize_cut(c, len_total_before, &bi)) return PBSIM_FAILED;
  return finalize_text(c, info);
}

int pbsim_batch_fetch(pbsim_ctx *c, char *read_text, char *maf_text) {
  if (!c || !c->s().b_finalized) return fail("pbsim_batch_fetch: no finalized batch");
  NEED_DEVICE(c);
  HIP_OK(hipSetDevice(c->device));
  if (read_text && c->s().b_info.read_text_bytes)
    HIP_OK(hipMemcpyAsync(read_text, c->s().d_read_text.p, (size_t)c->s().b_info.read_text_bytes, hipMemcpyDeviceToHost,
                          c->s().stream));
  if (maf_text && c->s().b_info.maf_text_bytes)
    HIP_OK(hipMemcpyAsync(maf_text, c->s().d_maf_text.p, (size_t)c->s().b_info.maf_text_bytes, hipMemcpyDeviceToHost,
                          c->s().stream));
  HIP_OK(hipStreamSynchronize(c->s().stream));
  return PBSIM_SUCCEEDED;
}

static int fetch_stats(pbsim_ctx *c, Slot &sl, int64_t n_tasks) {
  HIP_OK(sl.h_stats.ensure((size_t)n_tasks * 24));
  int32_t *ol = reinterpret_cast<int32_t *>(sl.h_stats.p);
  int32_t *ns = ol + n_tasks, *ni = ns + n_tasks, *nd = ni + n_tasks;
  double *qs = reinterpret_cast<double *>(nd + n_tasks);
  if (sl.sq_pending) {
    HIP_OK(hipStreamWaitEvent(sl.stream, sl.ev_sq_done, 0));
    sl.sq_pending = false;
  }
  HIP_OK(hipMemcpyAsync(ol, sl.d_out_len.p, n_tasks * 4, hipMemcpyDeviceToHost, sl.stream));
  HIP_OK(hipMemcpyAsync(ns, sl.d_nsub.p, n_tasks * 4, hipMemcpyDeviceToHost, sl.stream));
  HIP_OK(hipMemcpyAsync(ni, sl.d_nins.p, n_tasks * 4, hipMemcpyDeviceToHost, sl.stream));
  HIP_OK(hipMemcpyAsync(nd, sl.d_ndel.p, n_tasks * 4, hipMemcpyDeviceToHost, sl.stream));
  if (has_quality_row(c)) HIP_OK(hipMemcpyAsync(qs, sl.d_qsum.p, n_tasks * 8, hipMemcpyDeviceToHost, sl.stream));
  return PBSIM_SUCCEEDED;
}

extern "C++" int pbsim::account_of(pbsim_ctx *c, Slot &sl, StatsAcc *st) {
  if (!c || !sl.b_finalized) return fail("pbsim_batch_account: no finalized batch");
  NEED_DEVICE(c);
  HIP_OK(hipSetDevice(c->device));
  const int P = c->p.pass_num;
  const int64_t n_tasks = sl.b_info.n_final * P;
  if (n_tasks == 0) return PBSIM_SUCCEEDED;
  if (!sl.stats_fetched) {
    if (!fetch_stats(c, sl, n_tasks)) return PBSIM_FAILED;
    HIP_OK(hipStreamSynchronize(sl.stream));
  }
  const int32_t *ol = reinterpret_cast<const int32_t *>(sl.h_stats.p);
  const int32_t *ns = ol + n_tasks, *ni = ns + n_tasks, *nd = ni + n_tasks;
  const double *qs = reinterpret_cast<const double *>(nd + n_tasks);
  const bool quality = has_quality_row(c);
  st->res_num += sl.b_info.n_final;
  std::vector<double> *values = nullptr;
  if (st->keep_values) {
    st->blocks.emplace_back();
    st->blocks.back().first_task = (sl.b_first - 1) * P;
    values = &st->blocks.back().values;
    values->reserve((size_t)n_tasks);
  }
  for (int64_t t = 0; t < n_tasks; t++) stats_add_task(st, c->p.len_max, quality, ol[t], ns[t], ni[t], nd[t], quality ? qs[t] : 0.0, values);
  return PBSIM_SUCCEEDED;
}

extern "C++" int pbsim::account_slot(pbsim_ctx *c, StatsAcc *st) {
  if (!c) return fail("pbsim_batch_account: bad argument");
  return account_of(c, c->s(), st);
}

int pbsim_batch_account(pbsim_ctx *c) { return c ? account_slot(c, &c->st) : fail("pbsim_batch_account: bad argument"); }

int pbsim_get_stats(pbsim_ctx *c, pbsim_stats *o) {
  if (!c || !o) return fail("pbsim_get_stats: bad argument");
  stats_finish(c->st, c->p, c->p.strategy == PBSIM_STRATEGY_WGS ? c->ref_len : 0, o);
  return PBSIM_SUCCEEDED;
}

extern "C++" std::string pbsim::sam_header_text(const pbsim_ctx *c, int64_t unit) {
  std::string h = "@HD\tVN:1.5\tSO:unknown\tpb:3.0.7\n";
  h += "@RG\tID:ffffffff\tPL:PACBIO\tDS:READTYPE=SUBREAD;Ipd:CodecV1=ip;PulseWidth:CodecV1=pw;"
       "BINDINGKIT=101-789-500;SEQUENCINGKIT=101-826-100;BASECALLERVERSION=5.0.0;FRAMERATEHZ=100.000000\tPU:";
  h += c->p.id_prefix;
  if (c->p.strategy == PBSIM_STRATEGY_WGS) h += std::to_string((long)unit);
  h += "\tPM:SEQUELII\n";
  return h;
}
int64_t pbsim_sam_header(pbsim_ctx *c, char *buf, int64_t cap) {
  if (!c) return -1;
  const std::string h = sam_header_text(c, c->unit);
  if (buf && cap > (int64_t)h.size()) memcpy(buf, h.c_str(), h.size() + 1);
  return (int64_t)h.size();
}

int pbsim_set_bam_output(pbsim_ctx *c, int on) {
  if (!c) return fail("bad argument");
  if (on && c->p.pass_num < 2) return fail("BAM output applies to --pass-num >= 2 (single pass writes FASTQ, pbsim.cpp:707)");
  c->bam_output = on != 0;
  return PBSIM_SUCCEEDED;
}

int64_t pbsim_bam_header(pbsim_ctx *c, char *buf, int64_t cap) {
  if (!c) return -1;
  const int64_t lt = pbsim_sam_header(c, nullptr, 0);
  const int64_t n = 4 + 4 + lt + 4;
  if (buf && cap >= n) {
    std::vector<char> text((size_t)lt + 1);
    pbsim_sam_header(c, text.data(), lt + 1);
    memcpy(buf, "BAM\1", 4);
    const uint32_t l = (uint32_t)lt, zero = 0;
    memcpy(buf + 4, &l, 4);
    memcpy(buf + 8, text.data(), (size_t)lt);
    memcpy(buf + 8 + lt, &zero, 4);
  }
  return n;
}

extern "C++" int pbsim::prepare_enqueue(pbsim_ctx *c, uint8_t *d_seq, DevBuf &hp, DevBuf &tiles, DevBuf &flags, int64_t len,
                                        hipStream_t stream) {
  return enqueue_prepare(c, d_seq, hp, tiles, flags, len, 0, stream);
}
extern "C++" int pbsim::ensure_tables(pbsim_ctx *c, bool hp11) {
  if (!ensure_header_tables(c) || !ensure_class_tables(c)) return PBSIM_FAILED;
  if (c->p.method == PBSIM_METHOD_QS && !ensure_qs_tabs(c, hp11)) return PBSIM_FAILED;
  return PBSIM_SUCCEEDED;
}


int pbsim_simulate_wgs(pbsim_ctx *c, const pbsim_sink *sink) {
  if (!c) return fail("bad argument");
  return simulate_wgs(c, BatchOutput{sink, nullptr});
}
extern "C++" int pbsim::simulate_wgs(pbsim_ctx *c, const BatchOutput &out) {
  NEED_DEVICE(c);
  if (c->p.strategy != PBSIM_STRATEGY_WGS) return fail("pbsim_simulate_wgs: strategy is not wgs");
  if (!c->d_seq) return fail("no reference set (pbsim_set_reference)");
  pbsim_reset_stats(c);
  const int64_t quota = pbsim_unit_quota(c);
  double mean = 0.97 * std::min<double>(c->hdr.mean_len, (double)c->ref_len);
  constexpr int n_slots = kPipelineDepth;
  if (c->scratch_auto) {
    size_t free_b = 0, total_b = 0;
// ... 260 lines not shown
```

pbsim3_amd/csrc/job.cpp:

```cpp
#include <math.h>
#include <stdio.h>
#include <stdlib.h>
#include <string.h>

#include <algorithm>
#include <atomic>
#include <chrono>
#include <condition_variable>
#include <deque>
#include <future>
#include <mutex>
#include <thread>

#include "ctx.h"

using namespace pbsim;

namespace {

double now_us() {
  return std::chrono::duration<double, std::micro>(std::chrono::steady_clock::now().time_since_epoch()).count();
}

constexpr double kMinBatchBases = 2.0e9;
// ... 241 lines not shown
    return fail(werr);
  }

  void progress(int phase, int rec, int64_t first = 0, int64_t n_per = 0) {
    int64_t *g = c->job_progress;
    g[0] = phase;
    g[1] = rec;
    g[2] = first;
    g[3] = n_per;
    g[4] = W;
    g[5] = rec >= 0 ? recs[(size_t)rec].len_total : 0;
    g[6] = rec >= 0 ? recs[(size_t)rec].quota : 0;
    g[7] = rec >= 0 ? recs[(size_t)rec].next_read : 0;
  }
  int gather(const int64_t *send, int64_t n, std::vector<int64_t> *recv) {
    recv->assign((size_t)W * n, 0);
    if (!multi) {
      memcpy(recv->data(), send, (size_t)n * 8);
      return PBSIM_SUCCEEDED;
    }
    const double t0 = now_us();
    const int ok = comm->all_gather_i64(comm->user, send, n, recv->data());
    comm_us += now_us() - t0;
    n_exchanges++;
    return ok ? PBSIM_SUCCEEDED : fail("pbsim_comm.all_gather_i64 failed");
  }

  bool slot_busy(int s) const {
    if (delivering[s]) return true;
    for (const Round &r : fifo)
      if (r.slot == s) return true;
    for (const Rec &r : recs)
      if (r.tail_slot == s) return true;
    return false;
  }
  static constexpr int kTailSlot = kMaxSlots - 2;
  int free_slot() const {
    for (int s = 0; s < kTailSlot; s++)
      if (!slot_busy(s)) return s;
    return -1;
  }
  int free_tail_slot() const {
    for (int s = kTailSlot; s < kMaxSlots; s++)
      if (!slot_busy(s)) return s;
    return -1;
  }
  int bulk_in_flight() const { return (int)fifo.size(); }
  int acquire_slot() {
    const double t0 = now_us();
    for (;;) {
      const int s = free_slot();
      if (s >= 0) {
        bd_slot_wait += now_us() - t0;
        return s;
      }
      std::unique_lock<std::mutex> lk(worker.mu);
      worker.cv_idle.wait_for(lk, std::chrono::milliseconds(2));
    }
  }

  void drop_round(const Round &r) {
    c->cur = r.slot;
    (void)hipStreamSynchronize(c->s().stream);
    c->s().b_enqueued = false;
  }
  void drop_rounds_of(int rec) {
    for (auto it = fifo.begin(); it != fifo.end();) {
      if (it->rec == rec) {
        drop_round(*it);
        it = fifo.erase(it);
      } else {
        ++it;
      }
    }
  }
  void drop_everything(bool failing = true) {
    if (failing) {
      giving_up = true;
      { std::lock_guard<std::mutex> lk(out_mu); }
      out_cv.notify_all();
    }
    worker.drain();
    tail_worker.drain();
    for (const Round &r : fifo) drop_round(r);
    fifo.clear();
    for (Rec &r : recs)
      if (r.tail_slot >= 0) {
        c->cur = r.tail_slot;
        (void)hipStreamSynchronize(c->s().stream);
        c->s().b_enqueued = false;
        r.tail_slot = -1;
      }
  }

  size_t arena_max = 0;
  bool wants_text() const { return sink && (sink->on_read_text || sink->on_maf_text); }
  bool deflated() const { return wants_text() && c->deflate == 3; }

  int fetch_plain(Slot &sl) {
    const pbsim_batch_info &bi = sl.b_info;
    const bool want_r = sink->on_read_text && bi.read_text_bytes, want_m = sink->on_maf_text && bi.maf_text_bytes;
    if (want_r) {
      HIP_OK(sl.h_read_text.ensure((size_t)bi.read_text_bytes + 16));
      HIP_OK(hipMemcpyAsync(sl.h_read_text.p, sl.d_read_text.p, (size_t)bi.read_text_bytes, hipMemcpyDeviceToHost, sl.stream));
    }
    if (want_m) {
      HIP_OK(sl.h_maf_text.ensure((size_t)bi.maf_text_bytes + 16));
      HIP_OK(hipMemcpyAsync(sl.h_maf_text.p, sl.d_maf_text.p, (size_t)bi.maf_text_bytes, hipMemcpyDeviceToHost, sl.stream));
    }
    HIP_OK(hipStreamSynchronize(sl.stream));
    return PBSIM_SUCCEEDED;
  }
  int call_sink(int which, int64_t unit, const char *text, int64_t bytes, int64_t at) {
    std::lock_guard<std::mutex> lk(sink_mu[which]);
    return (which == 0 ? sink->on_read_text : sink->on_maf_text)(sink->user, unit, text, bytes, at);
  }
  int sink_plain(Slot &sl, int64_t unit, int64_t read_at, int64_t maf_at) {
    const pbsim_batch_info &bi = sl.b_info;
    if (sink->on_read_text && bi.read_text_bytes && !call_sink(0, unit, (const char *)sl.h_read_text.p, bi.read_text_bytes, read_at))
      return fail("sink aborted (read text)");
    if (sink->on_maf_text && bi.maf_text_bytes && !call_sink(1, unit, (const char *)sl.h_maf_text.p, bi.maf_text_bytes, maf_at))
      return fail("sink aborted (MAF text)");
    return PBSIM_SUCCEEDED;
  }
  template <class F>
  int both_lanes(Slot &sl, F &&lane) {
    const pbsim_batch_info &bi = sl.b_info;
    if (c->deflate_parallel && bi.read_text_bytes && bi.maf_text_bytes && sink->on_read_text && sink->on_maf_text) {
      int ok_read = PBSIM_SUCCEEDED;
      std::string err_read;
      std::thread t([&]() {
        (void)hipSetDevice(c->device);
        ok_read = lane(0);
        if (!ok_read) err_read = g_err;
      });
      const int ok_maf = lane(1);
      t.join();
      if (!ok_read) return fail(err_read);
      return ok_maf;
    }
    return lane(0) && lane(1);
  }
  int stream_deflated(Slot &sl, int64_t unit, int64_t read_at, int64_t maf_at, int64_t *read_gz, int64_t *maf_gz) {
    const pbsim_batch_info &bi = sl.b_info;
    *read_gz = *maf_gz = 0;
    return both_lanes(sl, [&](int which) -> int {
      const bool is_read = which == 0;
      const int64_t n = is_read ? bi.read_text_bytes : bi.maf_text_bytes;
      auto cb = is_read ? sink->on_read_text : sink->on_maf_text;
      int64_t *sent = is_read ? read_gz : maf_gz;
      const int64_t base = is_read ? read_at : maf_at;
      const uint8_t *d = is_read ? sl.d_read_text.as<uint8_t>() : sl.d_maf_text.as<uint8_t>();
      if (!cb || n == 0) return PBSIM_SUCCEEDED;
      return deflate_pieces(c, sl.df[which], d, n, [&](const char *z, int64_t k) {
        if (!call_sink(which, unit, z, k, base + *sent)) return fail(is_read ? "sink aborted (read text)" : "sink aborted (MAF text)");
        *sent += k;
        return PBSIM_SUCCEEDED;
      });
    });
  }
  int arena_fill(Slot &sl, int64_t *read_gz, int64_t *maf_gz) {
    const pbsim_batch_info &bi = sl.b_info;
    *read_gz = *maf_gz = 0;
    return both_lanes(sl, [&](int which) -> int {
      DfLane &L = sl.df[which];
      L.arena_reset();
      const int64_t n = which == 0 ? bi.read_text_bytes : bi.maf_text_bytes;
      auto cb = which == 0 ? sink->on_read_text : sink->on_maf_text;
      if (!cb || n == 0) return PBSIM_SUCCEEDED;
      const uint8_t *d = which == 0 ? sl.d_read_text.as<uint8_t>() : sl.d_maf_text.as<uint8_t>();
      bool oom = false;
      const std::function<char *(int64_t)> place = [&](int64_t k) -> char * {
        char *p = L.arena_reserve(k, arena_max);
        if (!p) oom = true;
        return p;
      };
      if (!deflate_pieces(c, L, d, n, [](const char *, int64_t) { return PBSIM_SUCCEEDED; }, &place))
        return oom ? fail("out of pinned host memory for a compressed batch (PBSIM_PINNED_ARENA_MB bounds a lane's arena)") : PBSIM_FAILED;
      int64_t tot = 0;
      for (const auto &sg : L.arena_segs) tot += sg.second;
      (which == 0 ? *read_gz : *maf_gz) = tot;
      return PBSIM_SUCCEEDED;
    });
  }
  int arena_flush(Slot &sl, int64_t unit, int64_t read_at, int64_t maf_at) {
    return both_lanes(sl, [&](int which) -> int {
      int64_t at = which == 0 ? read_at : maf_at;
      for (const auto &sg : sl.df[which].arena_segs) {
        if (!call_sink(which, unit, sg.first, sg.second, at)) return fail(which == 0 ? "sink aborted (read text)" : "sink aborted (MAF text)");
        at += sg.second;
      }
      sl.df[which].arena_segs.clear();
      return PBSIM_SUCCEEDED;
    });
  }

  void submit_stage1(Delivery *d) {
    d->stage1 = std::make_shared<std::promise<int>>();
    d->stage1_done = d->stage1->get_future();
    if (!d->mine) {
      d->stage1->set_value(PBSIM_SUCCEEDED);
      return;
    }
    delivering[d->slot] = true;
    Slot *sl = &c->slots[d->slot];
    Rec *R = &recs[(size_t)d->rec];
    auto prom = d->stage1;
    int64_t *sizes = d->sizes;
    const int64_t read_at = R->read_off, maf_at = R->maf_off;
    std::atomic<int> *out = &rec_out[(size_t)d->rec], *bulk = &rec_bulk[(size_t)d->rec];
    ++*out;
    ++*bulk;
    worker.post([this, sl, R, prom, sizes, read_at, maf_at, out, bulk]() {
      const double w0 = now_us();
      int ok = PBSIM_SUCCEEDED;
      if (wants_text() && hipEventSynchronize(sl->ev_text) != hipSuccess) ok = fail("hipEventSynchronize failed (text emission)");
      if (!ok) {
      } else if (!wants_text()) {
        sizes[0] = sizes[1] = 0;
      } else if (!deflated()) {
        ok = fetch_plain(*sl);
        sizes[0] = sink->on_read_text ? sl->b_info.read_text_bytes : 0;
        sizes[1] = sink->on_maf_text ? sl->b_info.maf_text_bytes : 0;
      } else if (!multi) {
        ok = stream_deflated(*sl, R->ref.unit, read_at, maf_at, &sizes[0], &sizes[1]);
      } else {
        ok = arena_fill(*sl, &sizes[0], &sizes[1]);
      }
      if (!ok) worker_fail();
      bd_worker_busy += now_us() - w0;
      if (trace)
        fprintf(stderr, "[pbsim job r%d] t=%.1f ms   worker: bytes of rec %lld on their way for %.1f ms (%lld + %lld)\n", rank,
                (w0 - t_start) / 1e3, (long long)R->ref.unit, (now_us() - w0) / 1e3, (long long)sizes[0], (long long)sizes[1]);
      delivered_one(out, bulk);
      prom->set_value(ok);
    });
  }
  Slot *acct_slot = nullptr;
  Rec *acct_rec = nullptr;
  int account_deferred() {
    if (!acct_slot) return PBSIM_SUCCEEDED;
    Slot *sl = acct_slot;
    acct_slot = nullptr;
    const double t0 = now_us();
    const int ok = account_of(c, *sl, &acct_rec->st);
    bd_account += now_us() - t0;
    round_closed((int)(acct_rec - recs.data()));
    return ok;
  }
  int wait_pending(int64_t c3[3]) {
    c3[0] = c3[1] = c3[2] = 0;
    if (!pending) return PBSIM_SUCCEEDED;
    const double t0 = now_us();
    const int ok1 = pending->stage1_done.get();
    pending->ok1 = ok1;
    pending->t_wait0 = t0;
    pending->t_wait1 = now_us();
    bd_wait_bytes += pending->t_wait1 - t0;
    c3[0] = pending->mine ? pending->sizes[0] : 0;
    c3[1] = pending->mine ? pending->sizes[1] : 0;
    c3[2] = ok1 ? 0 : 1;
    return PBSIM_SUCCEEDED;
  }
  int apply_pending(const std::vector<int64_t> &S, int stride, int at, bool defer_account) {
    if (!pending) return PBSIM_SUCCEEDED;
    std::unique_ptr<Delivery> d = std::move(pending);
    Rec &R = recs[(size_t)d->rec];
    const int ok1 = d->ok1;
    int64_t read_at = R.read_off, maf_at = R.maf_off, read_all = 0, maf_all = 0, bad = 0;
    for (int q = 0; q < W; q++) {
      const int64_t *v = &S[(size_t)q * stride + at];
      if (q < rank) {
        read_at += v[0];
        maf_at += v[1];
      }
      read_all += v[0];
      maf_all += v[1];
      bad += v[2];
    }
    if (bad) {
      if (ok1) peer_failed = true;
      return ok1 ? fail("another rank of the job failed") : check_worker();
    }
    R.read_off += read_all;
    R.maf_off += maf_all;
    if (d->mine) {
      Slot *sl = &c->slots[d->slot];
      Rec *Rp = &R;
      const int slot = d->slot;
      const bool flush = deflated() && multi, plain = wants_text() && !deflated();
      acct_slot = sl;
      acct_rec = &R;
      std::atomic<int> *out = &rec_out[(size_t)d->rec], *bulk = &rec_bulk[(size_t)d->rec];
      if (flush || plain) {
        ++*out;
        ++*bulk;
      }
      if (!defer_account && !account_deferred()) return PBSIM_FAILED;
      if (flush || plain) {
        worker.post([this, sl, Rp, slot, flush, read_at, maf_at, out, bulk]() {
          const int ok = flush ? arena_flush(*sl, Rp->ref.unit, read_at, maf_at) : sink_plain(*sl, Rp->ref.unit, read_at, maf_at);
          if (!ok) worker_fail();
          delivering[slot] = false;
          delivered_one(out, bulk);
        });
      } else {
        delivering[slot] = false;
      }
    } else {
      round_closed(d->rec);
    }
    if (trace)
      fprintf(stderr, "[pbsim job r%d] t=%.1f ms rec %d delivery: waited %.1f ms for the bytes (%lld + %lld)\n", rank,
              (d->t_wait0 - t_start) / 1e3, d->rec + 1, (d->t_wait1 - d->t_wait0) / 1e3, (long long)d->sizes[0], (long long)d->sizes[1]);
    return check_worker();
  }
  int complete_pending(bool defer_account = false) {
    if (!account_deferred()) return PBSIM_FAILED;
    if (!pending) return PBSIM_SUCCEEDED;
    int64_t mine2[3];
    if (!wait_pending(mine2)) return PBSIM_FAILED;
    std::vector<int64_t> S;
    progress(3, pending->rec, 0, pending->n_per);
    if (!gather(mine2, 3, &S)) return PBSIM_FAILED;
    return apply_pending(S, 3, 0, defer_account);
  }

  int tail_begin(Rec &R) {
    const int s = free_tail_slot();
    if (s < 0) {
      R.tail_waiting = true;
      return PBSIM_SUCCEEDED;
    }
    R.tail_waiting = false;
    c->cur = s;
    const int64_t remaining = R.quota - R.len_total;
    if (!walk_begin(c, R.ref, R.next_read, chain_reads_for(c, R.ref.len, remaining), remaining, true)) return PBSIM_FAILED;
    R.tail_slot = s;
    return PBSIM_SUCCEEDED;
  }
  int tail_poll(int rec, bool block) {
    Rec &R = recs[(size_t)rec];
    for (;;) {
      if (R.tail_waiting) {
        if (block) {
          for (size_t o = 0; o < recs.size(); o++)
            if ((int)o != rec && recs[o].tail_slot >= 0 && !tail_poll((int)o, true)) return PBSIM_FAILED;
          const double t_wait = now_us();
          while (free_tail_slot() < 0 && !wfailed && !giving_up) {
            std::unique_lock<std::mutex> lk(tail_worker.mu);
            tail_worker.cv_idle.wait_for(lk, std::chrono::milliseconds(1));
            if (now_us() - t_wait > 120e6) return fail("internal: the chains of truncated reads hold both slots and none comes back (120 s)");
          }
        }
        if (!tail_begin(R)) return PBSIM_FAILED;
        if (R.tail_waiting) return block ? fail("internal: no slot for the truncated reads") : PBSIM_SUCCEEDED;
      }
      if (R.tail_slot < 0) return PBSIM_SUCCEEDED;
      c->cur = R.tail_slot;
      if (!block && hipEventQuery(c->s().ev3) != hipSuccess) return PBSIM_SUCCEEDED;
      const double t0 = now_us();
      pbsim_batch_info bi;
      if (!chain_end_finalize(c, R.len_total, &bi)) return PBSIM_FAILED;
      n_tail_reads += bi.n_final;
      const int slot = R.tail_slot;
      Slot *sl = &c->slots[slot];
      Rec *Rp = &R;
      delivering[slot] = true;
      std::atomic<int> *out = &rec_out[(size_t)rec];
      ++*out;
      tail_worker.post([this, sl, Rp, slot, out, rec]() {
        int ok = PBSIM_SUCCEEDED;
        std::string zr, zm;
        const pbsim_batch_info &bi2 = sl->b_info;
        if (wants_text() && hipEventSynchronize(sl->ev_text) != hipSuccess) ok = fail("hipEventSynchronize failed (text emission)");
        if (!ok) {
        } else if (deflated()) {
          ok = both_lanes(*sl, [&](int which) -> int {
            const int64_t n = which == 0 ? bi2.read_text_bytes : bi2.maf_text_bytes;
            if (!(which == 0 ? sink->on_read_text : sink->on_maf_text) || n == 0) return PBSIM_SUCCEEDED;
            std::string *z = which == 0 ? &zr : &zm;
            const uint8_t *d = which == 0 ? sl->d_read_text.as<uint8_t>() : sl->d_maf_text.as<uint8_t>();
            return deflate_pieces(c, sl->df[which], d, n, [z](const char *p, int64_t k) {
              z->append(p, (size_t)k);
              return PBSIM_SUCCEEDED;
            });
          });
        } else if (wants_text()) {
          ok = fetch_plain(*sl);
        }
        if (!ok) worker_fail();
        const std::string err1 = ok ? std::string() : g_err;
        auto members = std::make_shared<std::pair<std::string, std::string>>(std::move(zr), std::move(zm));
        tail_worker.defer(
            rec,
            [this, rec]() {
              return wfailed.load() || giving_up.load() ||
                     (rec_rounds_open[(size_t)rec].load() == 0 && (!wants_text() || rec_bulk[(size_t)rec].load() == 0));
            },
            [this, sl, Rp, slot, out, ok, members]() {
              int ok2 = ok && !giving_up && !wfailed;
              const int64_t read_at = Rp->read_off + Rp->tail_read, maf_at = Rp->maf_off + Rp->tail_maf;
              int64_t nr = 0, nm = 0;
              if (!ok2) {
              } else if (deflated()) {
                nr = (int64_t)members->first.size();
                nm = (int64_t)members->second.size();
                if (nr && !call_sink(0, Rp->ref.unit, members->first.data(), nr, read_at)) ok2 = fail("sink aborted (read text)");
                if (ok2 && nm && !call_sink(1, Rp->ref.unit, members->second.data(), nm, maf_at)) ok2 = fail("sink aborted (MAF text)");
              } else if (wants_text()) {
                ok2 = sink_plain(*sl, Rp->ref.unit, read_at, maf_at);
                nr = sink->on_read_text ? sl->b_info.read_text_bytes : 0;
                nm = sink->on_maf_text ? sl->b_info.maf_text_bytes : 0;
              }
              if (ok2) ok2 = account_of(c, *sl, &Rp->st);
              Rp->tail_read += nr;
              Rp->tail_maf += nm;
              if (ok && !ok2 && !giving_up && !wfailed) worker_fail();
              delivering[slot] = false;
              delivered_one(out);
            });
      });
      reads_walked += bi.n_final;
      reads_delivered += bi.n_final;
      bases += bi.bases;
      ref_bases += bi.ref_bases;
      maf_columns += bi.maf_columns;
      if (trace)
        fprintf(stderr, "[pbsim job r%d] t=%.1f ms rec %d tail chain from read %lld: %lld reads, %.2f ms to collect\n", rank,
                (t0 - t_start) / 1e3, rec + 1, (long long)R.next_read, (long long)bi.n_final, (now_us() - t0) / 1e3);
      R.next_read += bi.n_final;
      R.len_total = bi.len_total_after;
      R.tail_slot = -1;
      if (!block) bd_tail_steps += now_us() - t0;
      if (R.len_total < R.quota) {
        if (!tail_begin(R)) return PBSIM_FAILED;
      } else {
        R.done = true;
        return PBSIM_SUCCEEDED;
      }
    }
  }

  int finish_record(int rec) {
    Rec &R = recs[(size_t)rec];
    if (pending && pending->rec == rec && !complete_pending()) return PBSIM_FAILED;
    if (!account_deferred()) return PBSIM_FAILED;
    const double tt = now_us();
    int tail_ok = PBSIM_SUCCEEDED;
    std::string tail_err;
    if (rank == R.owner && !tail_poll(rec, true)) {
      tail_ok = PBSIM_FAILED;
      tail_err = g_err;
    }
    const double td = now_us();
    bd_tail_block += td - tt;
    wait_record(rec);
    bd_drain += now_us() - td;
    int64_t extra[3] = {R.tail_read, R.tail_maf, (tail_ok && !wfailed) ? 0 : 1};
    const double t0 = now_us();
    progress(4, rec);
    if (!stats_merge(&R.st, c->p, multi ? comm : nullptr, extra, 3)) return PBSIM_FAILED;
    bd_merge += now_us() - t0;
    if (!tail_ok) return fail(tail_err);
    if (!check_worker()) return PBSIM_FAILED;
    if (extra[2]) {
      peer_failed = true;
      return fail("another rank of the job failed");
    }
    R.merged = R.done = true;
    pbsim_stats st;
    stats_finish(R.st, c->p, R.ref.len, &st);
    c->st = R.st;
    c->st.blocks.clear();
    R.st = StatsAcc();
    if (sink && sink->on_record_done &&
        !sink->on_record_done(sink->user, recs[(size_t)rec].ref.unit, &st, R.read_off + extra[0], R.maf_off + extra[1]))
      return fail("sink aborted (record done)");
    return PBSIM_SUCCEEDED;
  }

  int begin_round(int rec) {
    Rec &R = recs[(size_t)rec];
    const double remaining = (double)R.quota - R.spec_total;
    int64_t n_total = (int64_t)(1.005 * remaining / mean) + 64;
    if (remaining <= 0) n_total = 64;
    int64_t n_per = std::min<int64_t>((n_total + W - 1) / W, R.cap);
    if (rounds < 2) n_per = std::min<int64_t>(n_per, std::max<int64_t>(64, (int64_t)((double)R.cap * (rounds == 0 ? 0.2 : 0.5))));
    n_per = std::max<int64_t>(n_per, 1);
    if (!collect(rec)) return PBSIM_FAILED;
    const int s = acquire_slot();
    c->cur = s;
    const double tb = now_us();
    if (trace) fprintf(stderr, "[pbsim job r%d] begin rec %d first=%lld n_per=%lld\n", rank, rec + 1, (long long)R.spec_read, (long long)n_per);
    if (!walk_begin(c, R.ref, R.spec_read + (int64_t)rank * n_per, n_per, -1)) return PBSIM_FAILED;
    bd_begin += now_us() - tb;
    const double after = R.spec_total + (double)W * (double)n_per * mean;
    static const char *force_clear = getenv("PBSIM_JOB_CLEAR");
    const bool clear = force_clear ? atoi(force_clear) != 0
                                   : (double)R.quota - after > 0.04 * (double)W * (double)n_per * mean + 2.0 * (double)std::min<int64_t>(c->p.len_max, R.ref.len);
    fifo.push_back(Round{rec, s, R.spec_read, n_per, mean, clear});
    R.spec_read += (int64_t)W * n_per;
    R.spec_total += (double)W * (double)n_per * mean;
    reads_walked += n_per;
    rounds++;
    return PBSIM_SUCCEEDED;
  }

  static constexpr int kMsg = 8;
  int process_round() {
    const Round rd = fifo.front();
    fifo.pop_front();
    Rec &R = recs[(size_t)rd.rec];
    c->cur = rd.slot;
    const double t0 = now_us();
    int64_t pass0 = 0, code = 0;
    std::string my_err;
    if (!pbsim_batch_walk_end(c, &pass0)) {
      my_err = g_err;
      code = (my_err.rfind("scratch budget exceeded", 0) == 0 && rd.n_per > 1) ? 1 : 2;
    }
    if (wfailed) code = 2;
    const double t1 = now_us();
    bd_wait_walk += t1 - t0;
    for (size_t r = 0; r < recs.size(); r++)
      if ((recs[r].tail_slot >= 0 || recs[r].tail_waiting) && !tail_poll((int)r, false)) return PBSIM_FAILED;
    c->cur = rd.slot;
    const int64_t max_raw = c->s().b_max_raw;
    pbsim_batch_info bi;
    memset(&bi, 0, sizeof bi);
    int fin_ok = PBSIM_SUCCEEDED;
    double t_fin = 0;
    std::vector<int64_t> A, B;
    int64_t msg[kMsg] = {pass0, code, max_raw, 0, 0, 0, 0, 0};
    bool c_applied = false;
    if (rd.clear) {
      if (code == 0) {
        const double tf = now_us();
        fin_ok = finalize_uncut(c, &bi) && finalize_text(c, &bi);
// ... 724 lines not shown
```

pbsim3_amd/csrc/kernels.h:

```cpp
#pragma once
#include <hip/hip_runtime.h>
#include <stdint.h>

#include "modes.h"

namespace pbsim {

constexpr int kWG = 256;
constexpr int kLenBuckets = 4096;
constexpr int kBinPad = 16;
constexpr int kLenShift = 8;
constexpr int kScratchPad = 64;
constexpr int kMaxClasses = 64;
constexpr int32_t kWaveTransposed = 1 << 30;
constexpr int kHpTile = 4096;

enum : uint32_t {
  kErrScratchOverflow = 1u,
  kErrScratchBudget = 2u,
};

struct DeviceFlags {
  uint32_t error;
  uint32_t high_bytes;
  int64_t n_final;
  int64_t total_slots;
  int64_t scratch_need;
  int64_t sums[8];
  unsigned long long hpfreq[12];
  uint32_t need_q10;
  uint32_t max_rawlen;
};

struct RefView {
  const uint8_t *seq;
  const uint8_t *hp;
  int64_t len;
};


struct HeaderArgs {
  uint32_t seed, unit;
  int64_t first_read;
  int64_t n_reads;
  const int32_t *prob2len;
  int64_t len_rv;
  const uint8_t *prob2acc;
  int64_t acc_rv;
  int64_t ref_len;
  int64_t len_min;
  int64_t truncate_remaining;
  int32_t *rawlen, *len, *off;
  uint8_t *acc;
  uint32_t *max_rawlen;
  int32_t is_templ;
  const int32_t *read_unit;
  const int64_t *unit_len;
  const int32_t *unit_rank;
  const int32_t *off_table;
  const uint8_t *ssp;
  const int32_t *ssp_rv;
};

struct ChainState {
  int64_t remaining;
  int64_t total;
  int32_t made;
  int32_t done;
};

struct SortArgs {
  int64_t n_reads;
  int32_t pass_num;
  int32_t acc_lo, ncls;
  const int32_t *len;
  const uint8_t *acc;
  int32_t *hist;
  int32_t *bin_start;
  int32_t *bin_cursor;
  int32_t *class_start;
  int32_t coop_bucket;
  int32_t *coop_end;
  uint64_t coop_classes;
  int32_t *task_of_slot;
  int32_t *slot_of_task;
  int32_t *wave_cap;
  int64_t *wave_off;
  int64_t n_slots_max;
  int32_t *wg_hist, *wg_start;
  int32_t *wg_order;
  int32_t regions;
  int32_t cap_q8;
  int64_t scratch_bytes;
  DeviceFlags *flags;
};

struct WalkArgs {
  uint32_t seed, unit;
  int64_t first_read;
  int32_t pass_num;
  int32_t ncls;
  RefView ref;
  const int32_t *len, *off;
  const int64_t *read_base;
  const uint8_t *read_minus;
  const uint8_t *cls_blob;
  uint32_t stride, rows_off, init_off, tran_off, emis_off, freq_off, rv_off;
  const int32_t *class_start;
  const int32_t *task_of_slot;
  const int32_t *wg_order;
  int32_t mean_len;
  int32_t coop_min_len;
  int32_t coop_dynamic;
  int32_t cap_q8;
  const int32_t *coop_end;
  const int32_t *wave_cap;
  const int64_t *wave_off;
  uint8_t *scratch;
  int32_t *out_len, *maf_len, *nsub, *nins, *ndel;
  double *qsum;
  const uint32_t *sub_thre, *ins_thre, *del_thr;
  const double *qprob;
  DeviceFlags *flags;
};

struct SampleArgs {
  uint32_t seed, unit;
  int64_t first_read;
  int32_t n_lines;
  int32_t n_line_waves;
  int32_t n_coop_waves;
  int32_t n_coop_blocks;
  int64_t n_coop_slots;
  RefView ref;
  const uint8_t *quals;
  const int64_t *line_qoff;
  const int32_t *line_len;
  const int32_t *vbase;
  const int32_t *task_of_slot;
  const int32_t *wave_cap;
  const int64_t *wave_off;
  uint8_t *scratch;
  int32_t *span, *off;
  int32_t *out_len, *maf_len, *nsub, *nins, *ndel;
  double *qsum;
  const uint32_t *sub_thre, *ins_thre, *del_thr;
  const double *qprob;
  DeviceFlags *flags;
};

struct TextArgs {
  int64_t first_read;
  int64_t n_reads;
  int32_t pass_num;
  int32_t is_wgs;
  int32_t is_qs;
  uint32_t unit;
  int64_t ref_len;
  const int32_t *len, *off;
  const int32_t *out_len, *maf_len;
  const int32_t *slot_of_task;
  const int32_t *task_of_slot;
  int64_t *row_dst;
  const int32_t *wave_cap;
  const int64_t *wave_off;
  const uint8_t *scratch;
  const int64_t *read_text_off, *maf_text_off;
  int64_t *read_text_len, *maf_text_len;
  char *read_text, *maf_text;
  char id_prefix[64];
  int32_t id_prefix_len;
  char rq_text[32];
  int32_t rq_len;
  int32_t bam;
  uint32_t rq_bits;
  const int32_t *read_unit;
  const int64_t *unit_len;
  const char *unit_names;
  int32_t name_pad3;
  const uint8_t *read_minus;
};

struct ReadArrays {
  uint8_t *seq, *qual;
  int32_t *ref_pos;
  int64_t *offsets;
  int64_t *read_number;
  int32_t *pass_index, *unit;
  uint8_t *strand;
  int64_t *ref_start;
  int32_t *ref_span, *n_sub, *n_ins, *n_del;
};

struct ExportArgs {
  int64_t first_read;
  int64_t n_reads;
  int64_t bases;
  int32_t pass_num;
  int32_t is_qs;
  uint32_t unit;
  const int32_t *len, *off;
  const int32_t *out_len, *maf_len, *nsub, *nins, *ndel;
  const int32_t *task_of_slot;
  const int32_t *wave_cap;
  const int64_t *wave_off;
  const uint8_t *scratch;
  const int32_t *read_unit;
  const uint8_t *read_minus;
  int64_t *task_off;
  ReadArrays out;
};

void launch_prepare_reference(uint8_t *seq, uint8_t *hp, int flag_hp11, int64_t len, int64_t *tile_first, int64_t *tile_last,
                              int64_t *carry_start, int64_t *carry_next, int keep_first_case, DeviceFlags *flags,
                              hipStream_t s);
void launch_squeeze_lines(const uint8_t *lines, int64_t bytes, uint8_t *dst, int64_t *tile_tmp, int64_t *scan_tmp, int64_t *total,
                          hipStream_t s);
void launch_header_wgs(const HeaderArgs &a, hipStream_t s);
void launch_header_trans(const HeaderArgs &a, hipStream_t s);
void launch_task_sort(const SortArgs &a, hipStream_t s);
void launch_chain_prepare(const HeaderArgs &a, int k, int32_t pass_num, const int32_t *task_of_slot, int32_t *masked,
                          int64_t n_slots_max, ChainState *chain, hipStream_t s);
void launch_chain_update(int k, int32_t pass_num, const int32_t *out_len, ChainState *chain, hipStream_t s);
void launch_chain_init(ChainState *chain, int64_t remaining, hipStream_t s);
void launch_walk_errhmm(const WalkArgs &a, int64_t n_slots_max, uint32_t lds_bytes, bool fast_rv, bool hp_bits,
                        hipStream_t s, int min_lds_kb);
constexpr int kCoopMaxStates = 31;
constexpr int kCoopWaves = 8;
void launch_walk_errhmm_coop(const WalkArgs &a, int n_wg, uint32_t lds_bytes, bool hp_bits, hipStream_t s);
int walk_errhmm_coop_resident(uint32_t lds_bytes, bool hp_bits);
constexpr int kQCoopMaxStates = 63;
void launch_walk_qshmm_coop(const WalkArgs &a, int n_wg, uint32_t lds_bytes, hipStream_t s);
void launch_qshmm_coop_qsum(const WalkArgs &a, int64_t n_slots_max, hipStream_t s);
void launch_walk_qshmm(const WalkArgs &a, int64_t n_slots_max, uint32_t lds_bytes, bool fast_rv, bool hp_bits,
                       hipStream_t s, int min_lds_kb);
void launch_walk_sample(const SampleArgs &a, bool hp_bits, hipStream_t s);
void launch_sample_qsum(const SampleArgs &a, hipStream_t s);
void launch_exclusive_scan_i64(const int64_t *in, int64_t *out, int64_t n, int64_t *tmp, int64_t *total, hipStream_t s);
void launch_gather_pass0_scan(const int32_t *out_len, int64_t n_reads, int32_t pass_num, int64_t *cum, int64_t *tmp,
                              int64_t *total, hipStream_t s);
void launch_quota_cut(const int64_t *cum, const int32_t *rawlen, int64_t n_reads, int64_t len_total_before,
                      int64_t quota, int force_all, DeviceFlags *flags, hipStream_t s);
void launch_text_sizes(const TextArgs &a, DeviceFlags *flags, hipStream_t s);
void launch_text_emit(const TextArgs &a, int64_t n_slots_max, const DeviceFlags *flags, hipStream_t s);
void launch_export_sizes(const ExportArgs &a, DeviceFlags *flags, int64_t *scan_tmp, hipStream_t s);
void launch_export(const ExportArgs &a, int64_t n_slots_max, const DeviceFlags *flags, hipStream_t s);

#define DF_CHUNK 32768
#define DF_SLOT (DF_CHUNK + 64)
#define DF_PIECE_CHUNKS 8192
#define DF_SAMPLE_CHUNKS 64
#define DF_TABLE_HDR_DW 96
#define DF_TABLE_BYTES 2048
void deflate_host_tables(uint32_t *crc_table , uint32_t *pow128 );
void launch_deflate_table(const uint8_t *text, int64_t n_bytes, uint32_t *hist, void *table, hipStream_t s);
#define DF_CTL_BYTES 16
void launch_deflate(const uint8_t *text, int64_t n_bytes, uint64_t *status, void *ctl, uint32_t epoch, uint8_t *dense,
                    const uint32_t *d_crc_table, const uint32_t *d_pow128, const void *table, hipStream_t s,
                    unsigned long long *d_prof = nullptr ,
                    hipEvent_t ev_begin = nullptr, hipEvent_t ev_chunks_done = nullptr );

struct InflateMember {
  int64_t in_off, out_off;
  int32_t in_len, out_len;
  uint32_t crc, pad;
};
enum InflateStatus : int32_t {
  kInfOk = 0,
  kInfBlockType,
  kInfStoredLen,
  kInfTooMany,
  kInfClSet,
  kInfRepeat,
  kInfNoEob,
  kInfLitSet,
  kInfDistSet,
  kInfLitCode,
  kInfDistCode,
  kInfTooFar,
  kInfTruncated,
  kInfTrailing,
  kInfCrc,
  kInfLength,
  kInfCount
};
const char *inflate_reason(int32_t status);
void launch_inflate(const uint8_t *in, const InflateMember *members, int64_t n_members, uint8_t *out, int32_t *status,
                    const uint32_t *d_crc_table, const uint32_t *d_pow128, hipStream_t s);

constexpr int kSpTile = 1024;
inline int64_t sp_tiles(int64_t b0, int64_t b1) { return b1 > b0 ? (b1 - (b0 & ~(int64_t)(kSpTile - 1)) + kSpTile - 1) / kSpTile : 0; }
void launch_sp_count(const uint8_t *buf, int64_t b0, int64_t b1, int64_t *tile_count, int32_t *nul, hipStream_t s);
void launch_sp_lines(const uint8_t *buf, int64_t b0, int64_t b1, int phase, const int64_t *tile_base, uint32_t *rec_start,
                     uint32_t *rec_end, hipStream_t s);
void launch_sp_sums(const uint8_t *buf, const uint32_t *rec_start, const uint32_t *rec_end, int64_t n_rec, int32_t len_min,
                    int32_t len_max, double acc_min, double acc_max, const double *qprob , int32_t *rec_len,
                    double *accuracy, int64_t *padded, hipStream_t s);
void launch_sp_pool(const uint8_t *buf, const uint32_t *rec_start, const int32_t *rec_len, const int64_t *padded, const int64_t *off,
                    int64_t n_rec, uint8_t *pool, hipStream_t s);

}
```

pbsim3_amd/csrc/kernels.hip:

```cpp
#include <hip/hip_runtime.h>
#include <type_traits>

#include "kernels.h"
#include "philox.h"

namespace pbsim {

namespace {

constexpr int kScanBlock = 256;

__device__ __forceinline__ void short_kernel_priority() { __builtin_amdgcn_s_setprio(3); }
constexpr uint32_t kATGC = 0x43475441u;

__device__ __forceinline__ uint32_t to_upper(uint32_t c) { return (c >= 'a' && c <= 'z') ? c - 32u : c; }

__device__ __forceinline__ void scratch_store(uint32_t *p, uint32_t v) { __builtin_nontemporal_store(v, p); }
__device__ __forceinline__ uint32_t scratch_load(const uint32_t *p) { return *p; }

__device__ __forceinline__ uint32_t complement(uint32_t c) {
  uint32_t r = c;
  r = (c == 'A') ? 'T' : r;
  r = (c == 'T') ? 'A' : r;
  r = (c == 'G') ? 'C' : r;
// ... 2355 lines not shown
                       + (8 + (int64_t)q)
                       + 4
                       + 3 + bam_int_size((int64_t)q - 1)
                       + 7
                       + 24
                       + 3 + bam_int_size(readnum)
                       + 12;
  return 4 + 32 + (idl + 1) + (q + 1) / 2 + q + tags;
}

__global__ __launch_bounds__(256) void k_text_sizes(TextArgs a, DeviceFlags *flags) {
  short_kernel_priority();
  __shared__ unsigned long long s_sum[3];
  if (threadIdx.x < 3) s_sum[threadIdx.x] = 0;
  __syncthreads();
  const int64_t t = (int64_t)blockIdx.x * 256 + threadIdx.x;
  const int64_t n_tasks = a.n_reads * a.pass_num;
  if (t < n_tasks) {
    const int64_t r = t / a.pass_num;
    const int pass = (int)(t - r * a.pass_num);
    const int q = a.out_len[t], m = a.maf_len[t];
    TaskText x;
    task_text(a, r, pass, q, &x);
    int64_t rt;
    if (a.bam) {
      rt = bam_record_size(x.idl, q, x.readnum);
    } else if (a.pass_num == 1) {
      rt = 2LL * x.idl + 2LL * q + 6;
    } else {
      rt = (int64_t)x.idl + PB_LEN(PB_SAM_MID) + q + 1 + q + PB_LEN(PB_SAM_IP) + 2LL * q + PB_LEN(PB_SAM_PW) + 2LL * q +
           PB_LEN(PB_SAM_T1) + dec_len((int64_t)q - 1) + PB_LEN(PB_SAM_T2) + a.rq_len + PB_LEN(PB_SAM_T3) +
           count_digit(x.readnum) + PB_LEN(PB_SAM_T4);
    }
    const int64_t mt = (11LL + (x.name_len - x.r0) + x.w0 + x.w1 + x.w2 + x.w3 + m) +
                       (10LL + x.idl + (x.w0 - x.q0) + x.w1 + x.w2 + x.w3 + m);
    a.read_text_len[t] = rt;
    a.maf_text_len[t] = mt;
    atomicAdd(&s_sum[0], (unsigned long long)q);
    atomicAdd(&s_sum[1], (unsigned long long)a.len[r]);
    atomicAdd(&s_sum[2], (unsigned long long)m);
  }
  __syncthreads();
  if (threadIdx.x < 3) atomicAdd((unsigned long long *)&flags->sums[3 + threadIdx.x], s_sum[threadIdx.x]);
}

__device__ __forceinline__ char *g_lit(char *o, const char *lit, int n) {
  for (int i = 0; i < n; i++) o[i] = lit[i];
  return o + n;
}
__device__ __forceinline__ char *g_pad(char *o, int n) {
  for (int i = 0; i < n; i++) o[i] = ' ';
  return o + (n > 0 ? n : 0);
}

__global__ __launch_bounds__(256) void k_text_headers(TextArgs a) {
  short_kernel_priority();
  const int64_t t = (int64_t)blockIdx.x * 256 + threadIdx.x;
  const int64_t n_tasks = a.n_reads * a.pass_num;
  if (t >= n_tasks) return;
  const int64_t r = t / a.pass_num;
  const int pass = (int)(t - r * a.pass_num);
  const int q = a.out_len[t], m = a.maf_len[t];
  const int64_t readnum = a.first_read + r;
  const bool minus = a.read_minus ? (a.read_minus[r] != 0) : ((readnum & 1) == 0);
  int64_t *rd = a.row_dst + t * 6;
  char idbuf[160];
  const int idl = put_id(idbuf, a, readnum, pass);

  char *base = a.read_text + a.read_text_off[t];
  char *o = base;
  if (a.bam) {
    const int64_t size = bam_record_size(idl, q, readnum);
    o = bam_put_u32(o, (uint32_t)(size - 4));
    o = bam_put_u32(o, 0xffffffffu);
    o = bam_put_u32(o, 0xffffffffu);
    *o++ = (char)(idl + 1);
    *o++ = (char)255;
    *o++ = (char)(4680 & 0xff);
    *o++ = (char)(4680 >> 8);
    *o++ = 0;
    *o++ = 0;
    *o++ = 4;
    *o++ = 0;
    o = bam_put_u32(o, (uint32_t)q);
    o = bam_put_u32(o, 0xffffffffu);
    o = bam_put_u32(o, 0xffffffffu);
    o = bam_put_u32(o, 0);
    o = g_lit(o, idbuf, idl);
    *o++ = 0;
    rd[0] = o - a.read_text;
    o += (q + 1) / 2;
    rd[1] = o - a.read_text;
    o += q;
    o = bam_put_int_tag(o, 'c', 'x', 3);
    *o++ = 'i'; *o++ = 'p'; *o++ = 'B'; *o++ = 'C';
    o = bam_put_u32(o, (uint32_t)q);
    rd[4] = o - a.read_text;
    o += q;
    o = bam_put_int_tag(o, 'n', 'p', 1);
    *o++ = 'p'; *o++ = 'w'; *o++ = 'B'; *o++ = 'C';
    o = bam_put_u32(o, (uint32_t)q);
    rd[5] = o - a.read_text;
    o += q;
    o = bam_put_int_tag(o, 'q', 's', 0);
    o = bam_put_int_tag(o, 'q', 'e', (int64_t)q - 1);
    *o++ = 'r'; *o++ = 'q'; *o++ = 'f';
    o = bam_put_u32(o, a.rq_bits);
    *o++ = 's'; *o++ = 'n'; *o++ = 'B'; *o++ = 'f';
    o = bam_put_u32(o, 4);
    for (int i = 0; i < 4; i++) o = bam_put_u32(o, 0x41200000u);
    o = bam_put_int_tag(o, 'z', 'm', readnum);
    *o++ = 'R'; *o++ = 'G'; *o++ = 'Z';
    o = g_lit(o, "ffffffff", 8);
    *o++ = 0;
  } else if (a.pass_num == 1) {
    *o++ = '@';
    o = g_lit(o, idbuf, idl);
    *o++ = '\n';
    rd[0] = o - a.read_text;
    o += q;
    *o++ = '\n';
    *o++ = '+';
    o = g_lit(o, idbuf, idl);
    *o++ = '\n';
    rd[1] = o - a.read_text;
    o += q;
    *o++ = '\n';
    rd[4] = rd[5] = 0;
  } else {
    o = g_lit(o, idbuf, idl);
    o = g_lit(o, PB_SAM_MID, PB_LEN(PB_SAM_MID));
    rd[0] = o - a.read_text;
    o += q;
    *o++ = '\t';
    rd[1] = o - a.read_text;
    o += q;
    o = g_lit(o, PB_SAM_IP, PB_LEN(PB_SAM_IP));
    rd[4] = o - a.read_text;
    o += 2 * q;
    o = g_lit(o, PB_SAM_PW, PB_LEN(PB_SAM_PW));
    rd[5] = o - a.read_text;
    o += 2 * q;
    o = g_lit(o, PB_SAM_T1, PB_LEN(PB_SAM_T1));
    o += put_dec(o, (int64_t)q - 1);
    o = g_lit(o, PB_SAM_T2, PB_LEN(PB_SAM_T2));
    o = g_lit(o, a.rq_text, a.rq_len);
    o = g_lit(o, PB_SAM_T3, PB_LEN(PB_SAM_T3));
    o += put_dec(o, readnum);
    o = g_lit(o, PB_SAM_T4, PB_LEN(PB_SAM_T4));
  }

  TaskText x;
  task_text(a, r, pass, q, &x);
  o = a.maf_text + a.maf_text_off[t];
  *o++ = 'a';
  *o++ = '\n';
  *o++ = 's';
  *o++ = ' ';
  if (a.read_unit) {
    o = g_lit(o, a.unit_names + (size_t)a.read_unit[r] * 132, x.name_len);
  } else {
    *o++ = 'r';
    *o++ = 'e';
    *o++ = 'f';
  }
  o = g_pad(o, x.w0 - x.r0);
  o = g_pad(o, x.w1 - x.r1);
  *o++ = ' ';
  o += put_dec(o, x.start0);
  o = g_pad(o, x.w2 - x.r2);
  *o++ = ' ';
  o += put_dec(o, x.span);
  *o++ = ' ';
  *o++ = '+';
  o = g_pad(o, x.w3 - x.r3);
  *o++ = ' ';
  o += put_dec(o, x.reflen);
  *o++ = ' ';
  rd[2] = o - a.maf_text;
  o += m;
  *o++ = '\n';
  *o++ = 's';
  *o++ = ' ';
  o = g_lit(o, idbuf, idl);
  o = g_pad(o, x.w0 - x.q0);
  o = g_pad(o, x.w1 - 1);
  *o++ = ' ';
  *o++ = '0';
  o = g_pad(o, x.w2 - x.q2);
  *o++ = ' ';
  o += put_dec(o, q);
  *o++ = ' ';
  *o++ = minus ? '-' : '+';
  o = g_pad(o, x.w3 - x.q2);
  *o++ = ' ';
  o += put_dec(o, q);
  *o++ = ' ';
  rd[3] = o - a.maf_text;
  o += m;
  *o++ = '\n';
  *o++ = '\n';
}

constexpr int kTileStride = 69;
constexpr int kOutStride = 76;

__device__ __forceinline__ uint32_t dash_zero_bytes(uint32_t w) { return w | ((eq_bytes(w, 0u) >> 7) * 0x2Du); }

__device__ __forceinline__ void wave_lds_sync() {
  __builtin_amdgcn_fence(__ATOMIC_ACQ_REL, "wavefront");
  __builtin_amdgcn_wave_barrier();
}

__device__ __forceinline__ int row16_scan(int x) {
  x += __builtin_amdgcn_update_dpp(0, x, 0x111, 0xf, 0xf, false);
  x += __builtin_amdgcn_update_dpp(0, x, 0x112, 0xf, 0xf, false);
  x += __builtin_amdgcn_update_dpp(0, x, 0x114, 0xf, 0xf, false);
  x += __builtin_amdgcn_update_dpp(0, x, 0x118, 0xf, 0xf, false);
  return x;
}

__device__ __forceinline__ void write_maf_tile(char *text, long long D, int m, int t, const uint32_t *row, int minus,
                                               bool dash_zero, int sub) {
  int h = minus ? (int)((D + m) & 15) : (int)((16 - (D & 15)) & 15);
  h = h < m ? h : m;
  const int cons = (t == 0) ? h : 256 * t - ((16 - h) & 15);
  const int avail = (m < 256 * (t + 1)) ? m : 256 * (t + 1);
  const uint8_t *row8 = reinterpret_cast<const uint8_t *>(row);
  if (t == 0 && sub < h) {
    uint32_t v = row8[16 + sub];
    if (minus) v = complement(v);
    if (dash_zero && v == 0) v = '-';
    text[minus ? D + m - 1 - sub : D + sub] = (char)v;
  }
  const int n_ch = (avail - cons) >> 4;
  if (sub < n_ch) {
    const int b = 16 + cons - 256 * t + 16 * sub;
    const uint32_t *src = row + (b >> 2);
    const uint32_t sh = (uint32_t)(b & 3);
    const uint32_t d0 = src[0], d1 = src[1], d2 = src[2], d3 = src[3], d4 = src[4];
    const uint32_t a0 = __builtin_amdgcn_alignbyte(d1, d0, sh), a1 = __builtin_amdgcn_alignbyte(d2, d1, sh),
                   a2 = __builtin_amdgcn_alignbyte(d3, d2, sh), a3 = __builtin_amdgcn_alignbyte(d4, d3, sh);
    const uint32_t rev = minus ? 0x00010203u : 0x03020100u;
    const uint32_t x0 = __builtin_amdgcn_perm(0u, minus ? a3 : a0, rev), x1 = __builtin_amdgcn_perm(0u, minus ? a2 : a1, rev),
                   x2 = __builtin_amdgcn_perm(0u, minus ? a1 : a2, rev), x3 = __builtin_amdgcn_perm(0u, minus ? a0 : a3, rev);
    const long long dst = minus ? D + m - cons - 16 * sub - 16 : D + cons + 16 * sub;
    const uint32_t f_lo = (minus ? 0x47025400u : 0x43024100u) | (dash_zero ? 0x2Du : 0u);
    const uint32_t f_hi = minus ? 0x434E2D41u : 0x474E2D54u;
    const uint32_t b_lo = minus ? 0x47025400u : 0x43024100u;
    const uint32_t b_hi = (minus ? 0x434E0041u : 0x474E0054u) | (dash_zero ? 0u : 0x2D00u);
    uint32_t w0 = __builtin_amdgcn_perm(f_hi, f_lo, x0 & 0x07070707u), w1 = __builtin_amdgcn_perm(f_hi, f_lo, x1 & 0x07070707u),
             w2 = __builtin_amdgcn_perm(f_hi, f_lo, x2 & 0x07070707u), w3 = __builtin_amdgcn_perm(f_hi, f_lo, x3 & 0x07070707u);
    const uint32_t bad = (__builtin_amdgcn_perm(b_hi, b_lo, w0 & 0x07070707u) ^ x0) |
                         (__builtin_amdgcn_perm(b_hi, b_lo, w1 & 0x07070707u) ^ x1) |
                         (__builtin_amdgcn_perm(b_hi, b_lo, w2 & 0x07070707u) ^ x2) |
                         (__builtin_amdgcn_perm(b_hi, b_lo, w3 & 0x07070707u) ^ x3);
    if (__builtin_expect(bad != 0, 0)) {
      w0 = minus ? complement4(x0) : x0;
      w1 = minus ? complement4(x1) : x1;
      w2 = minus ? complement4(x2) : x2;
      w3 = minus ? complement4(x3) : x3;
      if (dash_zero) {
        w0 = dash_zero_bytes(w0);
        w1 = dash_zero_bytes(w1);
        w2 = dash_zero_bytes(w2);
        w3 = dash_zero_bytes(w3);
      }
    }
    *reinterpret_cast<uint4 *>(text + dst) = make_uint4(w0, w1, w2, w3);
  }
  if (avail == m) {
    const int r = (m - cons) & 15, c0 = m - r;
    if (sub < r) {
      uint32_t v = row8[16 + (c0 - 256 * t) + sub];
      if (minus) v = complement(v);
      if (dash_zero && v == 0) v = '-';
      text[minus ? D + m - 1 - (c0 + sub) : D + c0 + sub] = (char)v;
    }
  }
}

struct RowLane {
  const uint32_t *src;
  size_t step;
};
__device__ __forceinline__ RowLane row_lane(const uint32_t *region, bool transposed, int cap_dw, int wv, int lt, int lc) {
  RowLane r;
  r.src = transposed ? region + (size_t)(wv * 16 + lt) * cap_dw + 16 * lc : region + wv * 16 + lt + (size_t)(16 * lc) * 64;
  r.step = transposed ? 1 : 64;
  return r;
}
__device__ __forceinline__ void tile_fetch(uint32_t pre[16], const RowLane &r, int c1) {
#pragma unroll
  for (int c = 0; c < 16; ++c) pre[c] = scratch_load(r.src + (size_t)(c1 + c) * r.step);
}
__device__ __forceinline__ void tile_park(uint32_t *tile, const uint32_t pre[16], int lt, int lc) {
#pragma unroll
  for (int c = 0; c < 16; ++c) tile[lt * kTileStride + 4 + c + 16 * lc] = pre[c];
}

struct SqueezeStep {
  uint32_t keep;
  int excl;
  int total;
};
template <bool kPhred>
__device__ __forceinline__ SqueezeStep squeeze_window(char *dst_base, long long D, const uint32_t *trow, int ncol, bool act,
                                                      bool last, int sub, int lane, uint32_t *outb, const uint32_t *s_sel,
                                                      uint32_t *pend, int *done) {
  const uint8_t *orow = reinterpret_cast<const uint8_t *>(outb);
  const int dn = *done;
  const int p = (int)((D + dn) & 15);
  uint32_t w[4];
  uint32_t keep = 0;
#pragma unroll
  for (int k = 0; k < 4; k++) {
    w[k] = trow[4 + 4 * sub + k];
    const uint32_t nz = ~eq_bytes(w[k], 0u) & 0x80808080u;
    keep |= ((((nz >> 7) * 0x00204081u) >> 21) & 15u) << (4 * k);
  }
  const int nv = ncol - 16 * sub;
  keep &= (nv >= 16) ? 0xffffu : (nv > 0 ? (1u << nv) - 1u : 0u);
  const int cnt = __popc(keep);
  const int incl = row16_scan(cnt);
  const int total = __shfl(incl, (lane & 48) | 15, 64);
  reinterpret_cast<uint4 *>(outb)[1 + sub] = make_uint4(0u, 0u, 0u, 0u);
  if (sub < 2) reinterpret_cast<uint4 *>(outb)[17 + sub] = make_uint4(0u, 0u, 0u, 0u);
  if (sub < 4) outb[sub] = pend[sub];
  wave_lds_sync();
  {
    const int o = p + incl - cnt;
#pragma unroll
    for (int k = 0; k < 4; k++) {
      const uint32_t nib = (keep >> (4 * k)) & 15u;
      uint32_t v = __builtin_amdgcn_perm(0u, w[k], s_sel[nib]);
      if (kPhred) v -= 0x21212121u & (uint32_t)((1ull << (8 * __popc(nib))) - 1u);
      const int off = o + __popc(keep & ((1u << (4 * k)) - 1u));
      const unsigned long long sv = (unsigned long long)v << (8 * (off & 3));
      atomicOr(&outb[off >> 2], (uint32_t)sv);
      atomicOr(&outb[(off >> 2) + 1], (uint32_t)(sv >> 32));
    }
  }
  wave_lds_sync();
  const int have = p + total;
  const int n_ch = have >> 4;
  char *dst = dst_base + (D + dn - p);
  const int foreign = (p > dn) ? p - dn : 0;
  if (act && sub < n_ch) {
    const uint32_t *src = outb + 4 * sub;
    if (sub == 0 && foreign) {
#pragma unroll
// ... 622 lines not shown
```

Measured before the change: 55.49 billion.

## Add long-distance row matches to GPU deflate of MAF text using known alignment layout

The MAF text writer now records, per block, where the read alignment row starts and how far back the matching reference row lies. The deflate histogram and encode kernels use that layout to emit long back-references (minimum eleven bytes) from the read row to the reference row, plus a real distance Huffman alphabet. A per-chunk row summary kernel avoids a binary search per segment. The aim is to shrink the compressed MAF output and so cut encode, copy and sink cost. In exchange it adds extra kernels, per-segment comparison work and a more complex Huffman table build.

Measured after the change: 54.99 billion (median of 5 runs). No clear change (-0.9%).

```diff
diff --git a/pbsim3_amd/csrc/ctx.h b/pbsim3_amd/csrc/ctx.h
--- a/pbsim3_amd/csrc/ctx.h
+++ b/pbsim3_amd/csrc/ctx.h
@@ -100,6 +100,7 @@
   uint32_t epoch = 0;
   DevBuf d_df_dense[kDfBuffers];
   DevBuf d_df_code;
+  DevBuf d_df_rows;
   HostBuf h_df_total, h_df_out[kDfBuffers];
   hipStream_t stream = nullptr;
   hipStream_t copy_stream = nullptr;
@@ -109,6 +110,7 @@
   const uint8_t *pre_text = nullptr;
   int64_t pre_n = 0;
   int pre_count = 0;
+  DfMafLayout maf;
   hipStream_t lane_stream = nullptr;
   hipEvent_t ev_pre = nullptr;
   hipEvent_t ev_df[kDfBuffers] = {}, ev_cp[kDfBuffers] = {};
@@ -232,6 +234,8 @@
   DevBuf d_task_of_slot, d_slot_of_task, d_wave_cap, d_wave_off, d_wg_tmp, d_wg_order;
   DevBuf d_out_len, d_maf_len, d_nsub, d_nins, d_ndel, d_qsum;
   DevBuf d_cum, d_scan_tmp, d_rt_len, d_mt_len, d_row_dst;
+  DevBuf d_maf_row, d_maf_dist;
+  int64_t maf_blocks = 0;
   DevBuf d_chain, d_chain_mask;
   DevBuf d_scratch, d_read_text, d_maf_text;
   HostBuf h_read_text, h_maf_text, h_stats, h_flags;
@@ -377,7 +381,16 @@
 int deflate_prelaunch(pbsim_ctx *c, Slot &sl, bool want_read, bool want_maf);
 int deflate_pieces(pbsim_ctx *c, DfLane &lane, const uint8_t *d_text, int64_t n,
                    const std::function<int(const char *, int64_t)> &consume,
-                   const std::function<char *(int64_t)> *place = nullptr);
+                   const std::function<char *(int64_t)> *place = nullptr, const DfMafLayout *maf = nullptr);
+inline DfMafLayout maf_layout_of(const Slot &sl) {
+  DfMafLayout m;
+  m.block_off = sl.d_mt_len.as<int64_t>();
+  m.row = sl.d_maf_row.as<int32_t>();
+  m.dist = sl.d_maf_dist.as<int32_t>();
+  m.n_blocks = sl.maf_blocks;
+  m.text_bytes = sl.b_info.maf_text_bytes;
+  return m;
+}
 int ensure_deflate_ready(pbsim_ctx *c);
 int ensure_crc_tables(pbsim_ctx *c);
 int prepare_enqueue(pbsim_ctx *c, uint8_t *d_seq, DevBuf &hp, DevBuf &tiles, DevBuf &flags, int64_t len, hipStream_t stream);
diff --git a/pbsim3_amd/csrc/deflate.hip b/pbsim3_amd/csrc/deflate.hip
--- a/pbsim3_amd/csrc/deflate.hip
+++ b/pbsim3_amd/csrc/deflate.hip
@@ -168,10 +168,11 @@
   Mask128 lit;
   Mask128 start;
   Mask128 cover;
+  Mask128 row;
 };
 
 __device__ __forceinline__ SegTokens seg_tokens(const uint32_t (&seg)[kSegDw], int seg_n, uint32_t prev_dword,
-                                                bool chunk_start) {
+                                                bool chunk_start, Mask128 row = Mask128{0, 0}) {
   uint64_t e[2] = {0, 0};
   uint32_t pw = prev_dword;
 #pragma unroll
@@ -188,12 +189,154 @@
   valid.hi = seg_n >= 128 ? ~0ull : seg_n > 64 ? (1ull << (seg_n - 64)) - 1 : 0ull;
   Mask128 eq = {e[0] & valid.lo, e[1] & valid.hi};
   if (chunk_start) eq.lo &= ~1ull;
+  eq = m_and(eq, m_not(row));
   const Mask128 r3 = m_and(eq, m_and(m_shr<1>(eq), m_shr<2>(eq)));
   SegTokens t;
-  t.cover = m_or(r3, m_or(m_shl<1>(r3), m_shl<2>(r3)));
-  t.start = m_and(t.cover, m_not(m_shl<1>(t.cover)));
+  const Mask128 run = m_or(r3, m_or(m_shl<1>(r3), m_shl<2>(r3)));
+  t.row = row;
+  t.cover = m_or(run, row);
+  t.start = m_or(m_and(run, m_not(m_shl<1>(run))), m_and(row, m_not(m_shl<1>(row))));
   t.lit = m_and(valid, m_not(t.cover));
   return t;
+}
+__device__ __forceinline__ bool m_bit(Mask128 a, int pos) { return ((pos < 64 ? a.lo >> pos : a.hi >> (pos - 64)) & 1ull) != 0; }
+__device__ __forceinline__ int match_len(const SegTokens &t, int pos, bool *is_row) {
+  *is_row = m_bit(t.row, pos);
+  const uint64_t k = *is_row ? ~0ull : 0ull;
+  return m_run(Mask128{(t.row.lo & k) | (t.cover.lo & ~t.row.lo & ~k), (t.row.hi & k) | (t.cover.hi & ~t.row.hi & ~k)}, pos);
+}
+
+constexpr int kRowMin = 11;
+constexpr int kDistSyms = 30;
+constexpr int kDistBase = 288;
+
+struct ChunkRows {
+  int32_t n, more, first, pad;
+  int32_t beg[4], end[4], d[4];
+};
+static_assert(sizeof(ChunkRows) == DF_CHUNK_ROWS_BYTES, "DF_CHUNK_ROWS_BYTES");
+
+struct MafArgs {
+  const int64_t *block_off;
+  const int32_t *row, *dist;
+  const ChunkRows *chunk_rows;
+  int64_t n_blocks, text_bytes, base;
+};
+
+__device__ __forceinline__ int64_t block_of(const int64_t *__restrict__ off, int64_t lo, int64_t hi, int64_t g) {
+  while (hi - lo > 1) {
+    const int64_t mid = (lo + hi) >> 1;
+    if (off[mid] <= g) lo = mid;
+    else hi = mid;
+  }
+  return lo;
+}
+
+struct SegRows {
+  int lo0, hi0, lo1, hi1;
+  int split;
+  int32_t d0, d1;
+  __device__ __forceinline__ int32_t dist_at(int pos) const { return pos >= split ? d1 : d0; }
+};
+
+__device__ __forceinline__ SegRows seg_rows(const MafArgs &m, int64_t cbase, int n, int beg) {
+  SegRows r;
+  r.lo0 = r.lo1 = r.hi0 = r.hi1 = 0;
+  r.d0 = r.d1 = 1;
+  r.split = kSeg;
+  const ChunkRows cr = m.chunk_rows[cbase / kChunk];
+  if (beg >= n) return r;
+  auto take = [&](int k, int a, int b, int32_t d) {
+    const bool ok = d >= 1 && d <= 32768;
+    const int first = d - beg;
+    const int lo_k = ok ? (a > first ? a : first) : 0, hi_k = ok ? b : 0;
+    if (k == 0) {
+      r.lo0 = lo_k;
+      r.hi0 = hi_k;
+      r.d0 = ok ? d : 1;
+    } else {
+      r.lo1 = lo_k;
+      r.hi1 = hi_k;
+      r.d1 = ok ? d : 1;
+      r.split = a;
+    }
+  };
+  if (!cr.more) {
+    int k = 0;
+#pragma unroll
+    for (int i = 0; i < 4; ++i) {
+      const int a0 = cr.beg[i] - beg, b0 = cr.end[i] - beg;
+      const int a = a0 > 0 ? a0 : 0, b = b0 < kSeg ? b0 : kSeg;
+      if (i < cr.n && a < b && k < 2) {
+        take(k, a, b, cr.d[i]);
+        ++k;
+      }
+    }
+    return r;
+  }
+  const int64_t g = cbase + beg;
+  int64_t lo = cr.first, step = 1;
+  while (lo + step < m.n_blocks && m.block_off[lo + step] <= g) {
+    lo += step;
+    step <<= 1;
+  }
+  int k = 0;
+  for (int64_t t = block_of(m.block_off, lo, lo + step < m.n_blocks ? lo + step : m.n_blocks, g); t < m.n_blocks && k < 2; ++t) {
+    const int64_t o = m.block_off[t];
+    if (o >= g + kSeg) break;
+    const int64_t row_beg = o + m.row[t];
+    const int64_t row_end = (t + 1 < m.n_blocks ? m.block_off[t + 1] : m.text_bytes) - 2;
+    const int64_t a = row_beg > g ? row_beg - g : 0, b = row_end - g < kSeg ? row_end - g : kSeg;
+    if (a >= b) continue;
+    take(k, (int)a, (int)b, m.dist[t]);
+    ++k;
+  }
+  return r;
+}
+
+__device__ __forceinline__ Mask128 row_cover(const SegRows &r, const uint32_t (&seg)[kSegDw], const uint32_t *s_in, int beg) {
+  uint64_t e[2] = {0, 0};
+  {
+#pragma unroll
+    for (int j = 0; j < kSegDw; ++j) {
+      const bool second = 4 * j + 3 >= r.split;
+      const int lo = second ? r.lo1 : r.lo0, hi = second ? r.hi1 : r.hi0;
+      if (4 * j + 4 <= lo || 4 * j >= hi) continue;
+      const int s = beg + 4 * j - (second ? r.d1 : r.d0);
+      const int sa = s >> 2;
+      const uint32_t w0 = sa >= 0 ? s_in[sa + (sa >> 5)] : 0u, w1 = s_in[sa + 1 + ((sa + 1) >> 5)];
+      const uint32_t d = seg[j] ^ __builtin_amdgcn_alignbyte(w1, w0, (uint32_t)(s & 3));
+      const uint32_t z = ~(((d & 0x7F7F7F7Fu) + 0x7F7F7F7Fu) | d | 0x7F7F7F7Fu);
+      uint32_t nib = (((z >> 7) * 0x00204081u) >> 21) & 15u;
+      if (lo > 4 * j) nib &= 15u << (lo - 4 * j);
+      if (hi < 4 * j + 4) nib &= 15u >> (4 * j + 4 - hi);
+      e[j >> 4] |= (uint64_t)nib << (4 * (j & 15));
+    }
+  }
+  const Mask128 x = {e[0], e[1]};
+  static_assert(kRowMin == 11, "the shifts below spell eleven");
+  const Mask128 r2 = m_and(x, m_shr<1>(x));
+  const Mask128 r4 = m_and(r2, m_shr<2>(r2));
+  const Mask128 r8 = m_and(r4, m_shr<4>(r4));
+  const Mask128 r11 = m_and(r8, m_and(m_shr<8>(r2), m_shr<10>(x)));
+  Mask128 c = m_or(r11, m_shl<1>(r11));
+  c = m_or(c, m_shl<2>(c));
+  c = m_or(c, m_shl<4>(c));
+  return m_or(c, m_shl<3>(c));
+}
+
+__device__ __forceinline__ void dist_symbol(uint32_t D, uint32_t *sym, uint32_t *eb, uint32_t *ev) {
+  const uint32_t v = D - 1;
+  if (v < 4) {
+    *sym = v;
+    *eb = 0;
+    *ev = 0;
+  } else {
+    const uint32_t e = (31 - __clz(v)) - 1;
+    *sym = 2 * e + 2 + ((v >> e) & 1u);
+    *eb = e;
+    *ev = v & ((1u << e) - 1);
+  }
 }
 
 constexpr int kSampleChunks = DF_SAMPLE_CHUNKS;
@@ -204,6 +347,7 @@
   uint32_t hdr_end_bits;
   uint32_t pad[3];
   uint32_t hdr[kHdrDw];
+  uint32_t dcode[32];
 };
 static_assert(sizeof(DfTable) <= DF_TABLE_BYTES, "DF_TABLE_BYTES too small");
 
@@ -230,19 +374,54 @@
 #pragma unroll
   for (int j = 0; j < kSegDw; ++j) seg[j] = s_in[tid * (kSegDw + 1) + j];
   *prev_dw = tid ? s_in[tid * (kSegDw + 1) - 2] : 0u;
-  __syncthreads();
-}
-
+}
+
+__global__ __launch_bounds__(kThreads) void k_deflate_chunk_rows(MafArgs m, int64_t n_chunks, ChunkRows *__restrict__ out) {
+  const int64_t c = (int64_t)blockIdx.x * kThreads + threadIdx.x;
+  if (c >= n_chunks) return;
+  const int64_t cbase = c * (int64_t)kChunk;
+  const int64_t cend = cbase + kChunk < m.text_bytes ? cbase + kChunk : m.text_bytes;
+  const int64_t t0 = block_of(m.block_off, 0, m.n_blocks, cbase);
+  ChunkRows cr;
+  cr.n = 0;
+  cr.first = (int32_t)t0;
+  cr.pad = 0;
+  for (int i = 0; i < 4; ++i) {
+    const int64_t t = t0 + i;
+    cr.beg[i] = cr.end[i] = 0;
+    cr.d[i] = 1;
+    if (t < m.n_blocks && m.block_off[t] < cend) {
+      cr.beg[i] = (int32_t)(m.block_off[t] + m.row[t] - cbase);
+      cr.end[i] = (int32_t)((t + 1 < m.n_blocks ? m.block_off[t + 1] : m.text_bytes) - 2 - cbase);
+      cr.d[i] = m.dist[t];
+      cr.n = i + 1;
+    }
+  }
+  cr.more = (t0 + 4 < m.n_blocks && m.block_off[t0 + 4] < cend) ? 1 : 0;
+  out[c] = cr;
+}
+
+template <bool kMaf>
 __global__ __launch_bounds__(kThreads) void k_deflate_hist(const uint8_t *__restrict__ text, int64_t n_bytes,
-                                                            uint32_t *__restrict__ hist) {
+                                                            uint32_t *__restrict__ hist, MafArgs maf) {
   __shared__ uint32_t s_in[kInDw];
   __shared__ uint32_t s_hist[3 * kSyms + 64];
+  __shared__ uint32_t s_dhist[32];
   const int tid = threadIdx.x, lane = tid & 63;
   for (int i = tid; i < 3 * kSyms + 64; i += kThreads) s_hist[i] = 0;
+  if (tid < 32) s_dhist[tid] = 0;
   uint32_t seg[kSegDw], prev_dw;
   int n, seg_n;
+  SegRows rows;
+  if constexpr (kMaf) {
+    const int64_t left = n_bytes - (int64_t)blockIdx.x * kChunk;
+    rows = seg_rows(maf, maf.base + (int64_t)blockIdx.x * kChunk, left < kChunk ? (int)left : kChunk, tid * kSeg);
+  }
   load_chunk(text, n_bytes, blockIdx.x, s_in, seg, &n, &seg_n, &prev_dw);
-  const SegTokens tk = seg_tokens(seg, seg_n, prev_dw, tid == 0);
+  Mask128 row = {0, 0};
+  if constexpr (kMaf) row = row_cover(rows, seg, s_in, tid * kSeg);
+  __syncthreads();
+  const SegTokens tk = seg_tokens(seg, seg_n, prev_dw, tid == 0, row);
   const uint32_t copy = (uint32_t)(lane % 3) * kSyms, dummy = 3 * kSyms + lane;
 #pragma unroll
   for (int j = 0; j < kSegDw; ++j) {
@@ -257,113 +436,125 @@
     const int pos = m_first(st);
     st = m_clear(st, pos);
     uint32_t sy, eb, ev;
-    length_symbol((uint32_t)m_run(tk.cover, pos), &sy, &eb, &ev);
+    bool is_row;
+    length_symbol((uint32_t)match_len(tk, pos, &is_row), &sy, &eb, &ev);
     atomicAdd(&s_hist[copy + sy], 1u);
+    if constexpr (kMaf) {
+      dist_symbol(is_row ? (uint32_t)rows.dist_at(pos) : 1u, &sy, &eb, &ev);
+      atomicAdd(&s_dhist[sy], 1u);
+    }
   }
   __syncthreads();
   for (int i = tid; i < 286; i += kThreads) {
     const uint32_t f = s_hist[i] + s_hist[kSyms + i] + s_hist[2 * kSyms + i] + (i == 256 ? 1u : 0u);
     if (f) atomicAdd(&hist[i], f);
   }
-}
-
-__global__ __launch_bounds__(kThreads) void k_deflate_build(const uint32_t *__restrict__ hist, DfTable *__restrict__ tbl) {
-  __shared__ uint32_t s_freq[kSyms], s_sfreq[kSyms], s_w[kSyms], s_code[kSyms];
+  if (kMaf && tid < kDistSyms && s_dhist[tid]) atomicAdd(&hist[kDistBase + tid], s_dhist[tid]);
+}
+
+__global__ __launch_bounds__(kThreads) void k_deflate_build(const uint32_t *__restrict__ hist, DfTable *__restrict__ tbl, int n_dist) {
+  constexpr int kAll = kDistBase + 32;
+  __shared__ uint32_t s_freq[kSyms], s_sfreq[kSyms], s_w[kSyms], s_code[kAll];
   __shared__ uint16_t s_sorted[kSyms], s_par[kSyms], s_leafpar[kSyms], s_dep[kSyms];
-  __shared__ uint8_t s_len[kSyms];
+  __shared__ uint8_t s_len[kAll];
   __shared__ uint32_t s_cnt[16], s_first[16];
   __shared__ uint32_t s_img[4 + kHdrDw];
   const int tid = threadIdx.x;
-  constexpr int m = 286;
-  for (int i = tid; i < kSyms; i += kThreads) {
-    s_freq[i] = i < m ? hist[i] + 1u : 0u;
+  constexpr int kLit = 286;
+  for (int i = tid; i < kAll; i += kThreads) {
     s_code[i] = 0;
     s_len[i] = 0;
   }
   for (int i = tid; i < 4 + kHdrDw; i += kThreads) s_img[i] = 0;
-  if (tid < 16) s_cnt[tid] = 0;
-  __syncthreads();
-  for (int i = tid; i < m; i += kThreads) {
-    const uint32_t fi = s_freq[i];
-    uint32_t rank = 0;
-    for (int u = 0; u < m; ++u) {
-      const uint32_t g = s_freq[u];
-      rank += (g < fi) | ((g == fi) & (u < i));
-    }
-    s_sorted[rank] = (uint16_t)i;
-    s_sfreq[rank] = fi;
-  }
-  __syncthreads();
-  if (tid == 0) {
-    int leaf = 0, root = 0;
-    for (int nxt = 0; nxt < m - 1; ++nxt) {
-      uint32_t tot = 0;
-      for (int k = 0; k < 2; ++k) {
-        const bool take_leaf = leaf < m && (root >= nxt || s_sfreq[leaf] <= s_w[root]);
-        if (take_leaf) {
-          tot += s_sfreq[leaf];
-          s_leafpar[leaf] = (uint16_t)nxt;
-          ++leaf;
-        } else {
-          tot += s_w[root];
-          s_par[root] = (uint16_t)nxt;
-          ++root;
+  for (int alpha = 0; alpha < (n_dist > 1 ? 2 : 1); ++alpha) {
+    const int m = alpha ? n_dist : kLit, o = alpha ? kDistBase : 0;
+    __syncthreads();
+    for (int i = tid; i < kSyms; i += kThreads) s_freq[i] = i < m ? hist[o + i] + 1u : 0u;
+    if (tid < 16) s_cnt[tid] = 0;
+    __syncthreads();
+    for (int i = tid; i < m; i += kThreads) {
+      const uint32_t fi = s_freq[i];
+      uint32_t rank = 0;
+      for (int u = 0; u < m; ++u) {
+        const uint32_t g = s_freq[u];
+        rank += (g < fi) | ((g == fi) & (u < i));
+      }
+      s_sorted[rank] = (uint16_t)i;
+      s_sfreq[rank] = fi;
+    }
+    __syncthreads();
+    if (tid == 0) {
+      int leaf = 0, root = 0;
+      for (int nxt = 0; nxt < m - 1; ++nxt) {
+        uint32_t tot = 0;
+        for (int k = 0; k < 2; ++k) {
+          const bool take_leaf = leaf < m && (root >= nxt || s_sfreq[leaf] <= s_w[root]);
+          if (take_leaf) {
+            tot += s_sfreq[leaf];
+            s_leafpar[leaf] = (uint16_t)nxt;
+            ++leaf;
+          } else {
+            tot += s_w[root];
+            s_par[root] = (uint16_t)nxt;
+            ++root;
+          }
         }
-      }
-      s_w[nxt] = tot;
-    }
-    s_dep[m - 2] = 0;
-    for (int i = m - 3; i >= 0; --i) s_dep[i] = s_dep[s_par[i]] + 1;
-    for (int i = 0; i < m; ++i) {
-      int d = s_dep[s_leafpar[i]] + 1;
-      if (d > 15) d = 15;
-      s_cnt[d] += 1;
-    }
-    uint32_t total = 0;
-    for (int l = 1; l <= 15; ++l) total += s_cnt[l] << (15 - l);
-    while (total > (1u << 15)) {
-      s_cnt[15] -= 1;
-      for (int l = 14; l >= 1; --l)
-        if (s_cnt[l]) {
-          s_cnt[l] -= 1;
-          s_cnt[l + 1] += 2;
-          break;
-        }
-      total -= 1;
-    }
-    int i = 0;
-    for (int l = 15; l >= 1; --l)
-      for (uint32_t k = 0; k < s_cnt[l]; ++k) s_len[s_sorted[i++]] = (uint8_t)l;
-    uint32_t code = 0;
-    s_cnt[0] = 0;
-    for (int l = 1; l <= 15; ++l) {
-      code = (code + s_cnt[l - 1]) << 1;
-      s_first[l] = code;
-    }
-  }
-  __syncthreads();
-  for (int i = tid; i < m; i += kThreads) {
-    const uint32_t l = s_len[i];
-    uint32_t idx = 0;
-    for (int u = 0; u < i; ++u) idx += s_len[u] == l;
-    s_code[i] = rev_bits(s_first[l] + idx, l) | (l << 16);
+        s_w[nxt] = tot;
+      }
+      s_dep[m - 2] = 0;
+      for (int i = m - 3; i >= 0; --i) s_dep[i] = s_dep[s_par[i]] + 1;
+      for (int i = 0; i < m; ++i) {
+        int d = s_dep[s_leafpar[i]] + 1;
+        if (d > 15) d = 15;
+        s_cnt[d] += 1;
+      }
+      uint32_t total = 0;
+      for (int l = 1; l <= 15; ++l) total += s_cnt[l] << (15 - l);
+      while (total > (1u << 15)) {
+        s_cnt[15] -= 1;
+        for (int l = 14; l >= 1; --l)
+          if (s_cnt[l]) {
+            s_cnt[l] -= 1;
+            s_cnt[l + 1] += 2;
+            break;
+          }
+        total -= 1;
+      }
+      int i = 0;
+      for (int l = 15; l >= 1; --l)
+        for (uint32_t k = 0; k < s_cnt[l]; ++k) s_len[o + s_sorted[i++]] = (uint8_t)l;
+      uint32_t code = 0;
+      s_cnt[0] = 0;
+      for (int l = 1; l <= 15; ++l) {
+        code = (code + s_cnt[l - 1]) << 1;
+        s_first[l] = code;
+      }
+    }
+    __syncthreads();
+    for (int i = tid; i < m; i += kThreads) {
+      const uint32_t l = s_len[o + i];
+      uint32_t idx = 0;
+      for (int u = 0; u < i; ++u) idx += s_len[o + u] == l;
+      s_code[o + i] = rev_bits(s_first[l] + idx, l) | (l << 16);
+    }
   }
   __syncthreads();
   if (tid == 0) {
     BitWriter bw;
     bw.init(s_img, kHeadBits);
-    bw.put64(kPrefixLo | ((uint64_t)(m - 257) << 3), 64);
+    bw.put64(kPrefixLo | ((uint64_t)(kLit - 257) << 3) | ((uint64_t)(n_dist - 1) << 8), 64);
     bw.put(kPrefixHi, kPrefixBits - 64);
     uint32_t bits = kHeadBits + kPrefixBits;
     int p = 0;
-    const int npos = m + 1;
+    const int npos = kLit + n_dist;
+    auto len_at = [&](int q) -> uint32_t { return q < kLit ? s_len[q] : n_dist > 1 ? s_len[kDistBase + q - kLit] : 1u; };
     while (p < npos) {
-      const uint32_t v = p < m ? s_len[p] : 1u;
+      const uint32_t v = len_at(p);
       bw.put(cl_code(v), cl_len(v));
       bits += cl_len(v);
       ++p;
       int r = 0;
-      while (p + r < npos && (p + r < m ? s_len[p + r] : 1u) == v) ++r;
+      while (p + r < npos && len_at(p + r) == v) ++r;
       while (r >= 3) {
         const int t = r < 6 ? r : 6;
         bw.put(cl_code(16) | ((uint32_t)(t - 3) << cl_len(16)), cl_len(16) + 2);
@@ -378,6 +569,7 @@
   __syncthreads();
   for (int i = tid; i < kSyms; i += kThreads) tbl->code[i] = s_code[i];
   for (int i = tid; i < kHdrDw; i += kThreads) tbl->hdr[i] = s_img[4 + i];
+  if (tid < 32) tbl->dcode[tid] = s_code[kDistBase + tid];
 }
 
 struct DfCtl {
@@ -449,18 +641,21 @@
   if ((uint32_t)tid < bytes - done) dst[done + tid] = s8[done + tid];
 }
 
+template <bool kMaf>
 __global__ __launch_bounds__(kThreads) void k_deflate_chunks(const uint8_t *__restrict__ text, int64_t n_bytes,
                                                               uint8_t *__restrict__ dense, uint64_t *__restrict__ status,
                                                               DfCtl *__restrict__ ctl, uint32_t epoch,
                                                               const uint32_t *__restrict__ crc_table,
                                                               const uint32_t *__restrict__ pow128, uint32_t x8rem,
                                                               const DfTable *__restrict__ tbl,
-                                                              unsigned long long *__restrict__ prof) {
+                                                              unsigned long long *__restrict__ prof, MafArgs maf) {
   __shared__ uint32_t s_in[kInDw];
   static_assert(kOutDw <= kInDw, "the output image must fit the input image");
   uint32_t *const s_out = s_in;
   __shared__ uint32_t s_code[kSyms];
   uint32_t *const s_crc = s_in;
+  static_assert(kOutDw + 4 + 32 <= kInDw, "no room behind the member for the distance codes");
+  uint32_t *const s_dist = s_in + kInDw - 32;
   __shared__ uint32_t s_wave[kThreads / 64];
   __shared__ uint32_t s_misc[4];
 
@@ -482,12 +677,45 @@
   const int64_t n_chunks = (n_bytes + kChunk - 1) / kChunk;
   uint32_t seg[kSegDw], prev_dw;
   int n, seg_n;
+  const int beg = tid * kSeg;
+  SegRows rows;
+  if constexpr (kMaf) {
+    const int64_t left = n_bytes - chunk * (int64_t)kChunk;
+    rows = seg_rows(maf, maf.base + chunk * (int64_t)kChunk, left < kChunk ? (int)left : kChunk, beg);
+  }
   load_chunk(text, n_bytes, chunk, s_in, seg, &n, &seg_n, &prev_dw);
-  const int beg = tid * kSeg;
+  Mask128 row = {0, 0};
+  if constexpr (kMaf) row = row_cover(rows, seg, s_in, beg);
+  __syncthreads();
   mark();
-  for (int i = tid; i < kInDw; i += kThreads) s_in[i] = (i < 1024) ? crc_table[i] : 0u;
+  for (int i = tid; i < kInDw; i += kThreads)
+    s_in[i] = (i < 1024) ? crc_table[i] : (kMaf && i >= kInDw - 32) ? tbl->dcode[i - (kInDw - 32)] : 0u;
   __syncthreads();
-  const SegTokens tk = seg_tokens(seg, seg_n, prev_dw, tid == 0);
+  const SegTokens tk = seg_tokens(seg, seg_n, prev_dw, tid == 0, row);
+  uint32_t dv0 = 0, dl0 = 0, dv1 = 0, dl1 = 0, dv2 = 0, dl2 = 0;
+  if constexpr (kMaf) {
+    auto dist_bits = [&](uint32_t D, uint32_t *v, uint32_t *l) {
+      uint32_t sy, eb, ev;
+      dist_symbol(D, &sy, &eb, &ev);
+      const uint32_t cd = s_dist[sy];
+      *v = (cd & 0xFFFFu) | (ev << (cd >> 16));
+      *l = (cd >> 16) + eb;
+    };
+    dist_bits(1u, &dv0, &dl0);
+    dist_bits((uint32_t)rows.d0, &dv1, &dl1);
+    dist_bits((uint32_t)rows.d1, &dv2, &dl2);
+  }
+  auto match_bits = [&](int pos, uint32_t *av, uint32_t *al, uint32_t *bv, uint32_t *bl) {
+    uint32_t sy, eb, ev;
+    bool is_row;
+    length_symbol((uint32_t)match_len(tk, pos, &is_row), &sy, &eb, &ev);
+    const uint32_t cm = s_code[sy];
+    *av = (cm & 0xFFFFu) | (ev << (cm >> 16));
+    *al = (cm >> 16) + eb;
+    const uint32_t mr = is_row ? ~0u : 0u, m2 = pos >= rows.split ? ~0u : 0u;
+    *bv = (dv0 & ~mr) | (mr & ((dv1 & ~m2) | (dv2 & m2)));
+    *bl = (dl0 & ~mr) | (mr & ((dl1 & ~m2) | (dl2 & m2)));
+  };
 
   uint32_t tok_bits = 0;
   {
@@ -527,9 +755,15 @@
     while (st.lo | st.hi) {
       const int pos = m_first(st);
       st = m_clear(st, pos);
-      uint32_t sy, eb, ev;
-      length_symbol((uint32_t)m_run(tk.cover, pos), &sy, &eb, &ev);
-      tok_bits += (s_code[sy] >> 16) + eb + 1;
+      if constexpr (kMaf) {
+        uint32_t av, al, bv, bl;
+        match_bits(pos, &av, &al, &bv, &bl);
+        tok_bits += al + bl;
+      } else {
+        uint32_t sy, eb, ev;
+        length_symbol((uint32_t)m_run(tk.cover, pos), &sy, &eb, &ev);
+        tok_bits += (s_code[sy] >> 16) + eb + 1;
+      }
     }
   }
   uint32_t tok_total;
@@ -570,6 +804,24 @@
         uint32_t c[4];
 #pragma unroll
         for (int k = 0; k < 4; ++k) c[k] = s_code[((nl >> k) & 1u) ? (w >> (8 * k)) & 255u : 287u];
+        if constexpr (kMaf) {
+          uint32_t av = 0, al = 0, bv = 0, bl = 0, a3v = 0, a3l = 0, b3v = 0, b3l = 0, ks = 4;
+          if (ns & 7u) {
+            ks = (uint32_t)__builtin_ctz(ns);
+            match_bits(4 * j + (int)ks, &av, &al, &bv, &bl);
+          }
+          if (ns & 8u) match_bits(4 * j + 3, &a3v, &a3l, &b3v, &b3l);
+          const uint32_t l0 = c[0] >> 16, l2 = c[2] >> 16;
+          const uint32_t v01 = (c[0] & 0xFFFFu) | ((c[1] & 0xFFFFu) << l0), n01 = l0 + (c[1] >> 16);
+          const uint32_t v23 = (c[2] & 0xFFFFu) | ((c[3] & 0xFFFFu) << l2), n23 = l2 + (c[3] >> 16);
+          const bool first = ks == 0, mid = ks == 1 || ks == 2;
+          bw.put(first ? av : v01, first ? al : n01);
+          bw.put(first ? bv : mid ? av : 0u, first ? bl : mid ? al : 0u);
+          bw.put(mid ? bv : v23, mid ? bl : n23);
+          bw.put(a3v, a3l);
+          bw.put(b3v, b3l);
+          continue;
+        }
         uint32_t mv = 0, ml = 0, ks = 4;
         if (ns) {
           ks = (uint32_t)__builtin_ctz(ns);
@@ -687,27 +939,48 @@
   }
 }
 
-void launch_deflate_table(const uint8_t *text, int64_t n_bytes, uint32_t *hist, void *table, hipStream_t s) {
+static MafArgs maf_args(const DfMafLayout *maf) {
+  MafArgs m = {nullptr, nullptr, nullptr, nullptr, 0, 0, 0};
+  if (maf)
+    m = {maf->block_off, maf->row, maf->dist, reinterpret_cast<const ChunkRows *>(maf->chunk_rows), maf->n_blocks, maf->text_bytes, maf->base};
+  return m;
+}
+
+void launch_deflate_table(const uint8_t *text, int64_t n_bytes, uint32_t *hist, void *table, hipStream_t s,
+                          const DfMafLayout *maf) {
   if (n_bytes <= 0) return;
   const int64_t nch = (n_bytes + DF_CHUNK - 1) / DF_CHUNK;
   const int64_t ns = nch < kSampleChunks ? nch : kSampleChunks;
   const int64_t sample_bytes = ns * (int64_t)DF_CHUNK < n_bytes ? ns * (int64_t)DF_CHUNK : n_bytes;
-  (void)hipMemsetAsync(hist, 0, 288 * sizeof(uint32_t), s);
-  hipLaunchKernelGGL(k_deflate_hist, dim3((unsigned)ns), dim3(kThreads), 0, s, text, sample_bytes, hist);
-  hipLaunchKernelGGL(k_deflate_build, dim3(1), dim3(kThreads), 0, s, (const uint32_t *)hist, reinterpret_cast<DfTable *>(table));
+  const bool rows = maf && maf->n_blocks > 0;
+  (void)hipMemsetAsync(hist, 0, DF_HIST_WORDS * sizeof(uint32_t), s);
+  if (rows)
+    hipLaunchKernelGGL(k_deflate_chunk_rows, dim3((unsigned)((nch + kThreads - 1) / kThreads)), dim3(kThreads), 0, s, maf_args(maf), nch,
+                       reinterpret_cast<ChunkRows *>(maf->chunk_rows));
+  if (rows)
+    hipLaunchKernelGGL(k_deflate_hist<true>, dim3((unsigned)ns), dim3(kThreads), 0, s, text, sample_bytes, hist, maf_args(maf));
+  else
+    hipLaunchKernelGGL(k_deflate_hist<false>, dim3((unsigned)ns), dim3(kThreads), 0, s, text, sample_bytes, hist, maf_args(nullptr));
+  hipLaunchKernelGGL(k_deflate_build, dim3(1), dim3(kThreads), 0, s, (const uint32_t *)hist, reinterpret_cast<DfTable *>(table),
+                     rows ? kDistSyms : 1);
 }
 
 void launch_deflate(const uint8_t *text, int64_t n_bytes, uint64_t *status, void *ctl, uint32_t epoch, uint8_t *dense,
                     const uint32_t *d_crc_table, const uint32_t *d_pow128, const void *table, hipStream_t s,
-                    unsigned long long *d_prof, hipEvent_t ev_begin, hipEvent_t ev_chunks_done) {
+                    unsigned long long *d_prof, hipEvent_t ev_begin, hipEvent_t ev_chunks_done, const DfMafLayout *maf) {
   if (n_bytes <= 0) return;
   const int64_t nch = (n_bytes + DF_CHUNK - 1) / DF_CHUNK;
   const uint32_t x8rem = host_xpow8((uint64_t)(n_bytes % DF_CHUNK) & 127u);
   (void)hipMemsetAsync(ctl, 0, DF_CTL_BYTES, s);
   if (ev_begin) (void)hipEventRecord(ev_begin, s);
-  hipLaunchKernelGGL(k_deflate_chunks, dim3((unsigned)nch), dim3(kThreads), 0, s, text, n_bytes, dense, status,
-                     reinterpret_cast<DfCtl *>(ctl), epoch & 0x3fffffffu, d_crc_table, d_pow128, x8rem,
-                     reinterpret_cast<const DfTable *>(table), d_prof);
+  if (maf && maf->n_blocks > 0)
+    hipLaunchKernelGGL(k_deflate_chunks<true>, dim3((unsigned)nch), dim3(kThreads), 0, s, text, n_bytes, dense, status,
+                       reinterpret_cast<DfCtl *>(ctl), epoch & 0x3fffffffu, d_crc_table, d_pow128, x8rem,
+                       reinterpret_cast<const DfTable *>(table), d_prof, maf_args(maf));
+  else
+    hipLaunchKernelGGL(k_deflate_chunks<false>, dim3((unsigned)nch), dim3(kThreads), 0, s, text, n_bytes, dense, status,
+                       reinterpret_cast<DfCtl *>(ctl), epoch & 0x3fffffffu, d_crc_table, d_pow128, x8rem,
+                       reinterpret_cast<const DfTable *>(table), d_prof, maf_args(nullptr));
   if (ev_chunks_done) (void)hipEventRecord(ev_chunks_done, s);
 }
 
diff --git a/pbsim3_amd/csrc/deflate_host.cpp b/pbsim3_amd/csrc/deflate_host.cpp
--- a/pbsim3_amd/csrc/deflate_host.cpp
+++ b/pbsim3_amd/csrc/deflate_host.cpp
@@ -64,22 +64,30 @@
     HIP_OK(hipMemsetAsync(sl.d_df_status.p, 0, sl.d_df_status.bytes, sl.stream));
     sl.epoch++;
   }
+  DfMafLayout maf = sl.maf;
+  maf.base = off;
   launch_deflate(d_text + off, len, sl.d_df_status.as<uint64_t>(), sl.d_df_ctl.p, ++sl.epoch, dense, tab, tab + 1024,
-                 sl.d_df_code.p, sl.stream, d_prof, sl.ev_k0[b], sl.ev_k1[b]);
+                 sl.d_df_code.p, sl.stream, d_prof, sl.ev_k0[b], sl.ev_k1[b], maf.n_blocks ? &maf : nullptr);
   HIP_OK(hipGetLastError());
   HIP_OK(hipMemcpyAsync(&h_total[2 * b], sl.d_df_ctl.p, DF_CTL_BYTES, hipMemcpyDeviceToHost, sl.stream));
   HIP_OK(hipEventRecord(sl.ev_df[b], sl.stream));
   return PBSIM_SUCCEEDED;
 }
 
-int df_begin(pbsim_ctx *c, DfLane &sl, const uint8_t *d_text, int64_t n, bool own_staging, hipStream_t launch_stream) {
+int df_begin(pbsim_ctx *c, DfLane &sl, const uint8_t *d_text, int64_t n, bool own_staging, hipStream_t launch_stream,
+             const DfMafLayout *maf) {
   if (!ensure_deflate_tables(c)) return PBSIM_FAILED;
+  sl.maf = maf ? *maf : DfMafLayout();
   const DfGeom g = df_geom(n);
   const size_t status_bytes_was = sl.d_df_status.bytes;
   HIP_OK(sl.d_df_status.ensure((size_t)(g.piece / DF_CHUNK) * 8));
   HIP_OK(sl.d_df_ctl.ensure(DF_CTL_BYTES));
   HIP_OK(sl.h_df_total.ensure(DF_CTL_BYTES * kDfBuffers));
-  HIP_OK(sl.d_df_code.ensure(DF_TABLE_BYTES + 288 * 4));
+  HIP_OK(sl.d_df_code.ensure(DF_TABLE_BYTES + DF_HIST_WORDS * 4));
+  if (sl.maf.n_blocks) {
+    HIP_OK(sl.d_df_rows.ensure((size_t)((n + DF_CHUNK - 1) / DF_CHUNK) * DF_CHUNK_ROWS_BYTES));
+    sl.maf.chunk_rows = sl.d_df_rows.p;
+  }
   int lane_index = 0;
   for (Slot &slot : c->slots)
     if (&slot.df[1] == &sl) lane_index = 1;
@@ -99,7 +107,8 @@
   sl.stream = launch_stream ? launch_stream : lane_streams[0];
   sl.copy_stream = lane_streams[1];
   if (sl.d_df_status.bytes != status_bytes_was) HIP_OK(hipMemsetAsync(sl.d_df_status.p, 0, sl.d_df_status.bytes, sl.stream));
-  launch_deflate_table(d_text, n, reinterpret_cast<uint32_t *>(sl.d_df_code.as<uint8_t>() + DF_TABLE_BYTES), sl.d_df_code.p, sl.stream);
+  launch_deflate_table(d_text, n, reinterpret_cast<uint32_t *>(sl.d_df_code.as<uint8_t>() + DF_TABLE_BYTES), sl.d_df_code.p, sl.stream,
+                       sl.maf.n_blocks ? &sl.maf : nullptr);
   if (!sl.ev_df[0]) {
     for (int i = 0; i < kDfBuffers; i++) {
       HIP_OK(hipEventCreateWithFlags(&sl.ev_df[i], hipEventDisableTiming));
@@ -132,11 +141,12 @@
 
 template <class F>
 int deflate_stream(pbsim_ctx *c, DfLane &sl, const uint8_t *d_text, int64_t n, F &&consume,
-                   const std::function<char *(int64_t)> *place = nullptr) {
+                   const std::function<char *(int64_t)> *place = nullptr, const DfMafLayout *maf = nullptr) {
   if (n <= 0) return PBSIM_SUCCEEDED;
-  const bool prelaunched = sl.pre_valid && sl.pre_text == d_text && sl.pre_n == n && sl.pre_own_staging == (place == nullptr);
+  const bool prelaunched = sl.pre_valid && sl.pre_text == d_text && sl.pre_n == n && sl.pre_own_staging == (place == nullptr) &&
+                           (sl.maf.n_blocks != 0) == (maf && maf->n_blocks != 0);
   sl.pre_valid = false;
-  if (!prelaunched && !df_begin(c, sl, d_text, n, place == nullptr, nullptr)) return PBSIM_FAILED;
+  if (!prelaunched && !df_begin(c, sl, d_text, n, place == nullptr, nullptr, maf)) return PBSIM_FAILED;
   sl.pre_valid = false;
   if (sl.pre_elsewhere) {
     sl.stream = sl.lane_stream;
@@ -244,14 +254,14 @@
 }
 
 int deflate_to_host(pbsim_ctx *c, DfLane &sl, const uint8_t *d_text, int64_t n, char *host_dst, int64_t cap,
-                    int64_t *out_bytes) {
+                    int64_t *out_bytes, const DfMafLayout *maf = nullptr) {
   int64_t written = 0;
   const int ok = deflate_stream(c, sl, d_text, n, [&](const char *z, int64_t k) {
     if (written + k > cap) return fail("deflate: output buffer too small");
     memcpy(host_dst + written, z, (size_t)k);
     written += k;
     return PBSIM_SUCCEEDED;
-  });
+  }, nullptr, maf);
   *out_bytes = written;
   return ok;
 }
@@ -261,8 +271,8 @@
 
 extern "C++" int pbsim::deflate_pieces(pbsim_ctx *c, DfLane &lane, const uint8_t *d_text, int64_t n,
                                        const std::function<int(const char *, int64_t)> &consume,
-                                       const std::function<char *(int64_t)> *place) {
-  return deflate_stream(c, lane, d_text, n, consume, place);
+                                       const std::function<char *(int64_t)> *place, const DfMafLayout *maf) {
+  return deflate_stream(c, lane, d_text, n, consume, place, maf);
 }
 extern "C++" int pbsim::ensure_deflate_ready(pbsim_ctx *c) {
   for (auto &lane : c->df_streams)
@@ -273,9 +283,11 @@
 extern "C++" int pbsim::ensure_crc_tables(pbsim_ctx *c) { return ensure_deflate_tables(c); }
 extern "C++" int pbsim::deflate_prelaunch(pbsim_ctx *c, Slot &sl, bool want_read, bool want_maf) {
   const pbsim_batch_info &bi = sl.b_info;
-  if (want_read && bi.read_text_bytes > 0 && !df_begin(c, sl.df[0], sl.d_read_text.as<uint8_t>(), bi.read_text_bytes, true, sl.stream))
+  if (want_read && bi.read_text_bytes > 0 &&
+      !df_begin(c, sl.df[0], sl.d_read_text.as<uint8_t>(), bi.read_text_bytes, true, sl.stream, nullptr))
     return PBSIM_FAILED;
-  if (want_maf && bi.maf_text_bytes > 0 && !df_begin(c, sl.df[1], sl.d_maf_text.as<uint8_t>(), bi.maf_text_bytes, true, sl.stream))
+  const DfMafLayout maf = maf_layout_of(sl);
+  if (want_maf && bi.maf_text_bytes > 0 && !df_begin(c, sl.df[1], sl.d_maf_text.as<uint8_t>(), bi.maf_text_bytes, true, sl.stream, &maf))
     return PBSIM_FAILED;
   return PBSIM_SUCCEEDED;
 }
@@ -301,8 +313,9 @@
   if (read_gz && !deflate_to_host(c, c->s().df[0], c->s().d_read_text.as<uint8_t>(), c->s().b_info.read_text_bytes, read_gz,
                                   read_cap, &nr))
     return PBSIM_FAILED;
+  const DfMafLayout maf = maf_layout_of(c->s());
   if (maf_gz && !deflate_to_host(c, c->s().df[0], c->s().d_maf_text.as<uint8_t>(), c->s().b_info.maf_text_bytes, maf_gz,
-                                 maf_cap, &nm))
+                                 maf_cap, &nm, &maf))
     return PBSIM_FAILED;
   if (read_gz_bytes) *read_gz_bytes = nr;
   if (maf_gz_bytes) *maf_gz_bytes = nm;
@@ -353,9 +366,10 @@
       if (!zm)
         return sink->on_maf_text(sink->user, (const char *)sl.h_maf_text.p, bi.maf_text_bytes) ? PBSIM_SUCCEEDED
                                                                                               : fail("sink aborted (MAF text)");
+      const DfMafLayout maf = maf_layout_of(sl);
       return deflate_stream(c, sl.df[1], sl.d_maf_text.as<uint8_t>(), bi.maf_text_bytes, [&](const char *z, int64_t k) {
         return sink->on_maf_text(sink->user, z, k) ? PBSIM_SUCCEEDED : fail("sink aborted (MAF text)");
-      });
+      }, nullptr, &maf);
     };
     if (c->deflate_parallel && zr && zm && bi.read_text_bytes && bi.maf_text_bytes) {
       if (!ensure_deflate_tables(c)) return PBSIM_FAILED;
diff --git a/pbsim3_amd/csrc/engine.cpp b/pbsim3_amd/csrc/engine.cpp
--- a/pbsim3_amd/csrc/engine.cpp
+++ b/pbsim3_amd/csrc/engine.cpp
@@ -929,6 +929,8 @@
   t->maf_text_len = c->s().d_mt_len.as<int64_t>();
   t->read_text_off = t->read_text_len;
   t->maf_text_off = t->maf_text_len;
+  t->maf_row = c->s().d_maf_row.as<int32_t>();
+  t->maf_dist = c->s().d_maf_dist.as<int32_t>();
   t->id_prefix_len = (int)strlen(c->p.id_prefix);
   memcpy(t->id_prefix, c->p.id_prefix, sizeof t->id_prefix);
   t->rq_len = snprintf(t->rq_text, sizeof t->rq_text, "%f", c->p.accuracy_mean);
@@ -1025,6 +1027,8 @@
     HIP_OK(c->s().d_rt_len.ensure(n_tasks * 8));
     HIP_OK(c->s().d_mt_len.ensure(n_tasks * 8));
     HIP_OK(c->s().d_row_dst.ensure(n_tasks * 6 * 8));
+    HIP_OK(c->s().d_maf_row.ensure(n_tasks * 4));
+    HIP_OK(c->s().d_maf_dist.ensure(n_tasks * 4));
     c->s().stats_fetched = c->defer_text_sync;
     if (c->defer_text_sync && !fetch_stats(c, c->s(), n_tasks)) return PBSIM_FAILED;
     HIP_OK(hipMemsetAsync(&flags->sums[1], 0, 5 * sizeof(int64_t), c->s().stream));
@@ -1057,6 +1061,7 @@
     if (!c->defer_text_sync) HIP_OK(hipStreamSynchronize(c->s().stream));
   }
   c->s().b_info = bi;
+  c->s().maf_blocks = n_tasks > 0 ? n_tasks : 0;
   c->s().b_finalized = true;
   if (info) *info = bi;
   return PBSIM_SUCCEEDED;
diff --git a/pbsim3_amd/csrc/job.cpp b/pbsim3_amd/csrc/job.cpp
--- a/pbsim3_amd/csrc/job.cpp
+++ b/pbsim3_amd/csrc/job.cpp
@@ -417,11 +417,12 @@
       const int64_t base = is_read ? read_at : maf_at;
       const uint8_t *d = is_read ? sl.d_read_text.as<uint8_t>() : sl.d_maf_text.as<uint8_t>();
       if (!cb || n == 0) return PBSIM_SUCCEEDED;
+      const DfMafLayout maf = maf_layout_of(sl);
       return deflate_pieces(c, sl.df[which], d, n, [&](const char *z, int64_t k) {
         if (!call_sink(which, unit, z, k, base + *sent)) return fail(is_read ? "sink aborted (read text)" : "sink aborted (MAF text)");
         *sent += k;
         return PBSIM_SUCCEEDED;
-      });
+      }, nullptr, is_read ? nullptr : &maf);
     });
   }
   int arena_fill(Slot &sl, int64_t *read_gz, int64_t *maf_gz) {
@@ -440,7 +441,8 @@
         if (!p) oom = true;
         return p;
       };
-      if (!deflate_pieces(c, L, d, n, [](const char *, int64_t) { return PBSIM_SUCCEEDED; }, &place))
+      const DfMafLayout maf = maf_layout_of(sl);
+      if (!deflate_pieces(c, L, d, n, [](const char *, int64_t) { return PBSIM_SUCCEEDED; }, &place, which == 0 ? nullptr : &maf))
         return oom ? fail("out of pinned host memory for a compressed batch (PBSIM_PINNED_ARENA_MB bounds a lane's arena)") : PBSIM_FAILED;
       int64_t tot = 0;
       for (const auto &sg : L.arena_segs) tot += sg.second;
@@ -646,10 +648,11 @@
             if (!(which == 0 ? sink->on_read_text : sink->on_maf_text) || n == 0) return PBSIM_SUCCEEDED;
             std::string *z = which == 0 ? &zr : &zm;
             const uint8_t *d = which == 0 ? sl->d_read_text.as<uint8_t>() : sl->d_maf_text.as<uint8_t>();
+            const DfMafLayout maf = maf_layout_of(*sl);
             return deflate_pieces(c, sl->df[which], d, n, [z](const char *p, int64_t k) {
               z->append(p, (size_t)k);
               return PBSIM_SUCCEEDED;
-            });
+            }, nullptr, which == 0 ? nullptr : &maf);
           });
         } else if (wants_text()) {
           ok = fetch_plain(*sl);
diff --git a/pbsim3_amd/csrc/kernels.h b/pbsim3_amd/csrc/kernels.h
--- a/pbsim3_amd/csrc/kernels.h
+++ b/pbsim3_amd/csrc/kernels.h
@@ -167,6 +167,7 @@
   const uint8_t *scratch;
   const int64_t *read_text_off, *maf_text_off;
   int64_t *read_text_len, *maf_text_len;
+  int32_t *maf_row, *maf_dist;
   char *read_text, *maf_text;
   char id_prefix[64];
   int32_t id_prefix_len;
@@ -252,13 +253,25 @@
 #define DF_SAMPLE_CHUNKS 64
 #define DF_TABLE_HDR_DW 96
 #define DF_TABLE_BYTES 2048
+#define DF_CHUNK_ROWS_BYTES 64
+#define DF_HIST_WORDS 320
 void deflate_host_tables(uint32_t *crc_table , uint32_t *pow128 );
-void launch_deflate_table(const uint8_t *text, int64_t n_bytes, uint32_t *hist, void *table, hipStream_t s);
+struct DfMafLayout {
+  const int64_t *block_off = nullptr;
+  const int32_t *row = nullptr, *dist = nullptr;
+  void *chunk_rows = nullptr;
+  int64_t n_blocks = 0;
+  int64_t text_bytes = 0;
+  int64_t base = 0;
+};
+void launch_deflate_table(const uint8_t *text, int64_t n_bytes, uint32_t *hist, void *table, hipStream_t s,
+                          const DfMafLayout *maf = nullptr);
 #define DF_CTL_BYTES 16
 void launch_deflate(const uint8_t *text, int64_t n_bytes, uint64_t *status, void *ctl, uint32_t epoch, uint8_t *dense,
                     const uint32_t *d_crc_table, const uint32_t *d_pow128, const void *table, hipStream_t s,
                     unsigned long long *d_prof = nullptr ,
-                    hipEvent_t ev_begin = nullptr, hipEvent_t ev_chunks_done = nullptr );
+                    hipEvent_t ev_begin = nullptr, hipEvent_t ev_chunks_done = nullptr ,
+                    const DfMafLayout *maf = nullptr );
 
 struct InflateMember {
   int64_t in_off, out_off;
diff --git a/pbsim3_amd/csrc/kernels.hip b/pbsim3_amd/csrc/kernels.hip
--- a/pbsim3_amd/csrc/kernels.hip
+++ b/pbsim3_amd/csrc/kernels.hip
@@ -2531,7 +2531,8 @@
 
   TaskText x;
   task_text(a, r, pass, q, &x);
-  o = a.maf_text + a.maf_text_off[t];
+  char *const block = a.maf_text + a.maf_text_off[t];
+  o = block;
   *o++ = 'a';
   *o++ = '\n';
   *o++ = 's';
@@ -2576,6 +2577,8 @@
   o += put_dec(o, q);
   *o++ = ' ';
   rd[3] = o - a.maf_text;
+  a.maf_row[t] = (int32_t)(o - block);
+  a.maf_dist[t] = (int32_t)(rd[3] - rd[2]);
   o += m;
   *o++ = '\n';
   *o++ = '\n';
```
